# firelion9/raytracing-course-hw-public

Measured on AMD Instinct MI355X. Metric: Msamples/sec (whole node) on Sponza 1000x1000, higher is better.
Workload: dtype f32; 1 GPU; S-sponza synthetic (Sponza-sized): 262144+28 triangles, 16x3 1024^2 RGBA8 textures, 1000x1000, 64 SPP, ray_depth 8, device RNG; workload_id=sponza, width=1000, height=1000, spp=64, triangles=262172, launcher=single, ranks_formed=1, film=device (rt_render_rgb8), traversal=reference tree, reference order and pruning (parity mode), bvh=reference topology, host build

## Files before the change

### raytracing-course-hw-public_amd/csrc/rt_accum_host.cpp

```cpp
#include <algorithm>
#include <cmath>
#include <cstring>

#include "rt_scene_impl.h"

struct rt_accum {
    rt_scene *scene = nullptr;
    uint32_t width = 0, height = 0;
    WfView view{};
    WfView *d_view = nullptr;
    rt::AccumRound R{};
    std::vector<void *> owned;
    rt::PacketPolicy pkt;
    bool features = false;
    WfFeat F{};
    rt::DenoiseBufs D{};
    ~rt_accum() {
        (void)hipSetDevice(scene->device);
        (void)hipStreamSynchronize(scene->stream);
        for (void *p : owned)
            (void)hipFree(p);
        if (counted)
            --scene->live_accums;
    }
    bool counted = false;
};

template <class T> static int accum_alloc(rt_accum *a, size_t bytes, T **ptr, const char *fn) {
    void *q = nullptr;
    hipError_t e = hipMalloc(&q, bytes ? bytes : 16);
    if (e != hipSuccess)
        return rt::fail(e == hipErrorOutOfMemory ? RT_ERR_OOM : RT_ERR_HIP, std::string(fn) + ": " + hipGetErrorString(e));
    a->owned.push_back(q);
    *ptr = static_cast<T *>(q);
    return RT_OK;
}

extern "C" int rt_accum_create(rt_scene *s, uint32_t width, uint32_t height, const rt_camera *camera, uint64_t seed, rt_accum **out) {
    return rt_accum_create_ex(s, width, height, camera, seed, 0u, out);
}

extern "C" int rt_accum_create_ex(rt_scene *s, uint32_t width, uint32_t height, const rt_camera *camera, uint64_t seed, uint32_t accum_flags, rt_accum **out) {
    if (!s || !out)
        return rt::fail(RT_ERR_INVALID_ARG, "rt_accum_create: null argument");
    *out = nullptr;
    if (accum_flags & ~(uint32_t)RT_ACCUM_FEATURES)
        return rt::fail(RT_ERR_INVALID_ARG, "rt_accum_create_ex: unknown accum_flags bit");
    if (width == 0 || height == 0 || (uint64_t)width * height >= 0x7FFFFFFFull)
        return rt::fail(RT_ERR_INVALID_ARG, "rt_accum_create: image size " + std::to_string(width) + "x" + std::to_string(height));
    if (s->group)
        return rt::fail(RT_ERR_UNSUPPORTED, "rt_accum_create: accumulators run on single-GPU scenes only");
    HIP_TRY(hipSetDevice(s->device));
    auto a = std::make_unique<rt_accum>();
    a->scene = s;
    a->width = width;
    a->height = height;
    a->view = rt::make_view(camera ? *camera : s->cam, width, height, seed);
    const size_t n = (size_t)width * height;
    auto alloc = [&]<class T>(size_t bytes, T **ptr) -> int { return accum_alloc(a.get(), bytes, ptr, "rt_accum_create"); };
    rt::AccumRound &R = a->R;
    R.width = width;
    R.height = height;
    R.scan_temp_bytes = rt::accum_scan_temp_bytes((uint32_t)n);
    int rc;
    if ((rc = alloc(12 * n, &R.sum)) != RT_OK || (rc = alloc(12 * n, &R.even_sum)) != RT_OK || (rc = alloc(4 * n, &R.count)) != RT_OK ||
        (rc = alloc(4 * n, &R.err)) != RT_OK || (rc = alloc(4 * n, &R.target)) != RT_OK || (rc = alloc(8 * n, &R.scan_in)) != RT_OK ||
        (rc = alloc(8 * n, &R.scan)) != RT_OK || (rc = alloc(4 * n, &R.list_pix)) != RT_OK || (rc = alloc(4 * n, &R.list_base)) != RT_OK ||
        (rc = alloc(4 * (n + 1), &R.list_off)) != RT_OK || (rc = alloc(8, &R.totals)) != RT_OK || (rc = alloc(R.scan_temp_bytes, &R.scan_temp)) != RT_OK ||
        (rc = alloc(sizeof(WfView), &a->d_view)) != RT_OK)
        return rc;
    if (accum_flags & RT_ACCUM_FEATURES) {
        WfFeat &F = a->F;
        if ((rc = alloc(12 * n, &F.albedo_sum)) != RT_OK || (rc = alloc(12 * n, &F.normal_sum)) != RT_OK || (rc = alloc(4 * n, &F.depth_sum)) != RT_OK ||
            (rc = alloc(4 * n, &F.hits)) != RT_OK)
            return rc;
        HIP_TRY(hipMemsetAsync(F.albedo_sum, 0, 12 * n, s->stream));
        HIP_TRY(hipMemsetAsync(F.normal_sum, 0, 12 * n, s->stream));
        HIP_TRY(hipMemsetAsync(F.depth_sum, 0, 4 * n, s->stream));
        HIP_TRY(hipMemsetAsync(F.hits, 0, 4 * n, s->stream));
        a->features = true;
    }
    HIP_TRY(hipMemsetAsync(R.sum, 0, 12 * n, s->stream));
    HIP_TRY(hipMemsetAsync(R.even_sum, 0, 12 * n, s->stream));
    HIP_TRY(hipMemsetAsync(R.count, 0, 4 * n, s->stream));
    HIP_TRY(hipMemsetD32Async(R.err, 0x7F800000 , n, s->stream));
    HIP_TRY(hipMemcpyAsync(a->d_view, &a->view, sizeof(WfView), hipMemcpyHostToDevice, s->stream));
    HIP_TRY(hipStreamSynchronize(s->stream));
    a->counted = true;
    ++s->live_accums;
    *out = a.release();
    return RT_OK;
}

extern "C" void rt_accum_destroy(rt_accum *acc) { delete acc; }

static int accum_check(const rt_accum *a, const rt_params *p, const char *fn) {
    if (!a || !p)
        return rt::fail(RT_ERR_INVALID_ARG, std::string(fn) + ": null argument");
    if (p->width != a->width || p->height != a->height)
        return rt::fail(RT_ERR_INVALID_ARG, std::string(fn) + ": params size " + std::to_string(p->width) + "x" + std::to_string(p->height) +
                                                " differs from the accumulator's " + std::to_string(a->width) + "x" + std::to_string(a->height));
    if (p->shard_count > 1 || (p->flags & RT_FLAG_DEVICE_FB))
        return rt::fail(RT_ERR_INVALID_ARG, std::string(fn) + ": shard_count > 1 and RT_FLAG_DEVICE_FB do not apply to an accumulator");
    if (p->rng_mode == RT_RNG_REFERENCE)
        return rt::fail(RT_ERR_UNSUPPORTED, std::string(fn) + ": the reference RNG draws a 256-pixel span as one sequential stream; accumulators need RT_RNG_DEVICE");
    if (p->rng_mode != RT_RNG_DEVICE)
        return rt::fail(RT_ERR_INVALID_ARG, std::string(fn) + ": unknown rng_mode");
    if (p->flags & RT_FLAG_MEGAKERNEL)
        return rt::fail(RT_ERR_UNSUPPORTED, std::string(fn) + ": accumulators run on the wavefront pipeline, not the megakernel");
    return rt::check_pass_params(p, fn);
}

static int accum_run(rt_accum *a, const rt_params *p, const rt_adaptive *ad, uint32_t *rounds_out, rt_stats *stats) {
    rt_scene *s = a->scene;
    const auto wall0 = std::chrono::steady_clock::now();
    if (stats)
        std::memset(stats, 0, sizeof(*stats));
    if (rounds_out)
        *rounds_out = 0;
    if (s->dev.ray_depth == 0)
        return RT_OK;
    HIP_TRY(hipSetDevice(s->device));
    const uint32_t n_pix = a->width * a->height;
    const bool counters = stats && (p->flags & RT_FLAG_COUNTERS);
    const uint64_t max_paths = rt::wavefront_max_paths(s, p);
    const uint32_t chunk_cap = (uint32_t)std::max<uint64_t>(1, std::min<uint64_t>(max_paths, 0xFFFFFFFFull / n_pix));
    WfLaunch W{};
    W.width = a->width;
    W.height = a->height;
    W.shard_count = 1;
    W.shard_block = n_pix;
    W.ray_depth = s->dev.ray_depth;
    W.views = a->d_view;
    W.view_pixels = n_pix;
    W.global_best = (p->flags & RT_FLAG_GLOBAL_BEST) ? 1u : 0u;
    W.stats = counters ? s->d_stats : nullptr;
    s->ext_events.reset();
    uint32_t passes = 0, packet_passes = 0, rounds = 0;
    uint64_t added = 0;
    const uint32_t uni_chunk = std::min(ad ? 1u : p->samples, chunk_cap);
    const uint64_t uni_per_pass = std::max<uint64_t>(1, max_paths / uni_chunk);
    const uint32_t uni_passes = ad ? 0u : (uint32_t)(((uint64_t)p->samples + uni_chunk - 1) / uni_chunk * ((n_pix + uni_per_pass - 1) / uni_per_pass));

    auto fill = [&](uint32_t K, bool *any) -> int {
        const uint32_t C = std::min(K, chunk_cap);
        const uint32_t per_pass = (uint32_t)std::min<uint64_t>(n_pix, std::max<uint64_t>(1, max_paths / C));
        for (;;) {
            HIP_TRY(rt::launch_accum_plan(a->R, C, s->stream));
            uint32_t tot[2] = {0u, 0u};
            HIP_TRY(hipMemcpyAsync(tot, a->R.totals, sizeof(tot), hipMemcpyDeviceToHost, s->stream));
            HIP_TRY(hipStreamSynchronize(s->stream));
            if (tot[0] == 0)
                return RT_OK;
            *any = true;
            const uint64_t cap = std::min<uint64_t>((uint64_t)std::min(per_pass, tot[0]) * C, tot[1]);
            if (int rc = s->ensure_wavefront(cap, std::max<uint64_t>(s->wf_pixels_cap, 1), s->dev.ray_depth); rc != RT_OK)
                return rc;
            if (a->features) {
                if (int rc = s->ensure_features(); rc != RT_OK)
                    return rc;
                a->F.rec = s->wf_feat;
            }
            s->wf_bind(W);
            W.fb = nullptr;
            W.accum = nullptr;
            for (uint32_t e0 = 0; e0 < tot[0]; e0 += per_pass) {
                WfAccum A{a->R.sum, a->R.even_sum, a->R.count, a->R.list_pix, a->R.list_base, a->R.list_off, e0, std::min(per_pass, tot[0] - e0)};
                W.n_paths = (uint32_t)std::min<uint64_t>((uint64_t)A.n_entries * C, tot[1]);
                W.first_pixel = 0, W.pass_pixels = A.n_entries;
                W.first_sample = 0, W.pass_samples = C, W.samples = C;
                HIP_TRY(rt::launch_pass(s, p, a->pkt, W, 1, true, true, stats != nullptr, &A, a->features ? &a->F : nullptr));
                passes += 1;
                packet_passes += W.use_packet;
                if (p->progress && !ad) {
                    HIP_TRY(hipStreamSynchronize(s->stream));
                    p->progress(passes, std::max(passes, uni_passes), p->progress_user);
                }
            }
            added += tot[1];
        }
    };

    auto queue = [&]() -> int {
        if (counters)
            HIP_TRY(hipMemsetAsync(s->d_stats, 0, sizeof(DevStats), s->stream));
        HIP_TRY(hipEventRecord(s->ev0, s->stream));
        if (!ad) {
            HIP_TRY(rt::launch_accum_uniform(a->R, p->samples, s->stream));
            bool any = false;
            if (int rc = fill(p->samples, &any); rc != RT_OK)
                return rc;
        } else {
            const uint32_t mn = ad->min_samples ? ad->min_samples : 16u, st = ad->step ? ad->step : 32u, mx = ad->max_samples;
            const uint32_t bound = 1u + (mx - std::min(mn, mx) + st - 1u) / st;
            for (uint32_t r = 0;; ++r) {
                HIP_TRY(rt::launch_accum_judge(a->R, r == 0 ? 1 : 0, ad->threshold, mn, mx, st, s->stream));
                bool any = false;
                if (int rc = fill(r == 0 ? mn : st, &any); rc != RT_OK)
                    return rc;
                if (any) {
                    ++rounds;
                    if (p->progress)
                        p->progress(rounds, std::max(rounds, bound), p->progress_user);
                } else if (r > 0) {
                    break;
                }
            }
        }
        HIP_TRY(hipEventRecord(s->ev1, s->stream));
        return RT_OK;
    };
    if (int rc = rt::queue_and_wait(s, queue); rc != RT_OK)
        return rc;
    if (rounds_out)
        *rounds_out = rounds;
    if (stats) {
        float ms = 0;
        HIP_TRY(hipEventElapsedTime(&ms, s->ev0, s->ev1));
        if (int rc = rt::fill_stats(s, counters, added, ms, wall0, stats); rc != RT_OK)
            return rc;
        stats->packet_lanes_x100 = a->pkt.lanes_x100;
        stats->passes = passes;
        stats->packet_passes = packet_passes;
    }
    return RT_OK;
}

extern "C" int rt_accum_render(rt_accum *acc, const rt_params *params, rt_stats *stats) {
    if (int rc = accum_check(acc, params, "rt_accum_render"); rc != RT_OK)
        return rc;
    if (params->samples == 0)
        return rt::fail(RT_ERR_INVALID_ARG, "rt_accum_render: samples must be >= 1");
    return accum_run(acc, params, nullptr, nullptr, stats);
}

extern "C" int rt_accum_render_adaptive(rt_accum *acc, const rt_params *params, const rt_adaptive *ad, uint32_t *rounds, rt_stats *stats) {
    if (int rc = accum_check(acc, params, "rt_accum_render_adaptive"); rc != RT_OK)
        return rc;
    if (!ad)
        return rt::fail(RT_ERR_INVALID_ARG, "rt_accum_render_adaptive: null argument");
    if (!(ad->threshold >= 0.0f) || std::isinf(ad->threshold))
        return rt::fail(RT_ERR_INVALID_ARG, "rt_accum_render_adaptive: threshold must be finite and >= 0");
    const uint32_t mn = ad->min_samples ? ad->min_samples : 16u;
    if (mn == 1u || ad->max_samples < mn)
        return rt::fail(RT_ERR_INVALID_ARG, "rt_accum_render_adaptive: min_samples must be 0 or >= 2, and max_samples >= min_samples");
    for (uint32_t r : ad->reserved)
        if (r != 0)
            return rt::fail(RT_ERR_INVALID_ARG, "rt_accum_render_adaptive: reserved fields must be 0");
    return accum_run(acc, params, ad, rounds, stats);
}

extern "C" int rt_accum_resolve(rt_accum *acc, uint32_t flags, float *fb_rgb) {
    if (!acc || !fb_rgb || (flags & ~(uint32_t)RT_FLAG_DEVICE_FB))
        return rt::fail(RT_ERR_INVALID_ARG, "rt_accum_resolve: null argument or flags other than RT_FLAG_DEVICE_FB");
    rt_scene *s = acc->scene;
    HIP_TRY(hipSetDevice(s->device));
    const size_t n = (size_t)acc->width * acc->height;
    const bool device_fb = (flags & RT_FLAG_DEVICE_FB) != 0;
    if (!device_fb)
        if (int rc = s->ensure_fb(3 * n); rc != RT_OK)
            return rc;
    HIP_TRY(rt::launch_accum_image(acc->R, device_fb ? fb_rgb : s->d_fb, s->stream));
    if (!device_fb)
        HIP_TRY(hipMemcpyAsync(fb_rgb, s->d_fb, 3 * n * sizeof(float), hipMemcpyDeviceToHost, s->stream));
    HIP_TRY(hipStreamSynchronize(s->stream));
    return RT_OK;
}

extern "C" int rt_accum_resolve_rgb8(rt_accum *acc, uint32_t flags, uint8_t *rgb8) {
    if (!acc || !rgb8 || (flags & ~(uint32_t)RT_FLAG_DEVICE_FB))
        return rt::fail(RT_ERR_INVALID_ARG, "rt_accum_resolve_rgb8: null argument or flags other than RT_FLAG_DEVICE_FB");
    rt_scene *s = acc->scene;
    HIP_TRY(hipSetDevice(s->device));
    const uint32_t n = acc->width * acc->height;
    const bool device_fb = (flags & RT_FLAG_DEVICE_FB) != 0;
    int rc = s->ensure_fb(3ull * n);
    if (rc == RT_OK)
        rc = s->ensure_film(device_fb ? 0 : 3ull * n);
    if (rc != RT_OK)
        return rc;
    uint8_t *d_rgb8 = device_fb ? rgb8 : s->d_rgb8;
    HIP_TRY(rt::launch_accum_image(acc->R, s->d_fb, s->stream));
    HIP_TRY(rt::launch_film(s->d_fb, d_rgb8, n, 0, 1, n, s->d_film_table, s->stream));
    if (!device_fb)
        HIP_TRY(hipMemcpyAsync(rgb8, d_rgb8, 3ull * n, hipMemcpyDeviceToHost, s->stream));
    HIP_TRY(hipStreamSynchronize(s->stream));
    return RT_OK;
}

extern "C" int rt_accum_read(rt_accum *acc, float *sum_rgb, float *even_sum_rgb, uint32_t *samples, float *error) {
    if (!acc)
        return rt::fail(RT_ERR_INVALID_ARG, "rt_accum_read: null accumulator");
    rt_scene *s = acc->scene;
    HIP_TRY(hipSetDevice(s->device));
    const size_t n = (size_t)acc->width * acc->height;
    if (sum_rgb)
        HIP_TRY(hipMemcpyAsync(sum_rgb, acc->R.sum, 12 * n, hipMemcpyDeviceToHost, s->stream));
    if (even_sum_rgb)
        HIP_TRY(hipMemcpyAsync(even_sum_rgb, acc->R.even_sum, 12 * n, hipMemcpyDeviceToHost, s->stream));
    if (samples)
        HIP_TRY(hipMemcpyAsync(samples, acc->R.count, 4 * n, hipMemcpyDeviceToHost, s->stream));
    if (error)
        HIP_TRY(hipMemcpyAsync(error, acc->R.err, 4 * n, hipMemcpyDeviceToHost, s->stream));
    HIP_TRY(hipStreamSynchronize(s->stream));
    return RT_OK;
}

static int feature_check(const rt_accum *acc, const char *fn) {
    if (!acc)
        return rt::fail(RT_ERR_INVALID_ARG, std::string(fn) + ": null accumulator");
    if (!acc->features)
        return rt::fail(RT_ERR_INVALID_ARG, std::string(fn) + ": the accumulator was created without RT_ACCUM_FEATURES");
    return RT_OK;
}

extern "C" int rt_accum_read_features(rt_accum *acc, float *albedo_sum, float *normal_sum, float *depth_sum, uint32_t *hits) {
    if (int rc = feature_check(acc, "rt_accum_read_features"); rc != RT_OK)
        return rc;
    rt_scene *s = acc->scene;
    HIP_TRY(hipSetDevice(s->device));
    const size_t n = (size_t)acc->width * acc->height;
    if (albedo_sum)
        HIP_TRY(hipMemcpyAsync(albedo_sum, acc->F.albedo_sum, 12 * n, hipMemcpyDeviceToHost, s->stream));
    if (normal_sum)
        HIP_TRY(hipMemcpyAsync(normal_sum, acc->F.normal_sum, 12 * n, hipMemcpyDeviceToHost, s->stream));
    if (depth_sum)
        HIP_TRY(hipMemcpyAsync(depth_sum, acc->F.depth_sum, 4 * n, hipMemcpyDeviceToHost, s->stream));
    if (hits)
        HIP_TRY(hipMemcpyAsync(hits, acc->F.hits, 4 * n, hipMemcpyDeviceToHost, s->stream));
    HIP_TRY(hipStreamSynchronize(s->stream));
    return RT_OK;
}

extern "C" int rt_accum_resolve_features(rt_accum *acc, uint32_t flags, float *albedo, float *normal, float *depth) {
    if (int rc = feature_check(acc, "rt_accum_resolve_features"); rc != RT_OK)
        return rc;
    if (flags & ~(uint32_t)RT_FLAG_DEVICE_FB)
        return rt::fail(RT_ERR_INVALID_ARG, "rt_accum_resolve_features: flags other than RT_FLAG_DEVICE_FB");
    rt_scene *s = acc->scene;
    HIP_TRY(hipSetDevice(s->device));
    const size_t n = (size_t)acc->width * acc->height;
    if (flags & RT_FLAG_DEVICE_FB) {
        HIP_TRY(rt::launch_accum_feature_means(acc->R, acc->F, albedo, normal, depth, s->stream));
        HIP_TRY(hipStreamSynchronize(s->stream));
        return RT_OK;
    }
    if (int rc = s->ensure_fb(7 * n); rc != RT_OK)
        return rc;
    float *d_a = s->d_fb, *d_n = s->d_fb + 3 * n, *d_z = s->d_fb + 6 * n;
    HIP_TRY(rt::launch_accum_feature_means(acc->R, acc->F, d_a, d_n, d_z, s->stream));
    if (albedo)
        HIP_TRY(hipMemcpyAsync(albedo, d_a, 12 * n, hipMemcpyDeviceToHost, s->stream));
    if (normal)
        HIP_TRY(hipMemcpyAsync(normal, d_n, 12 * n, hipMemcpyDeviceToHost, s->stream));
    if (depth)
        HIP_TRY(hipMemcpyAsync(depth, d_z, 4 * n, hipMemcpyDeviceToHost, s->stream));
    HIP_TRY(hipStreamSynchronize(s->stream));
    return RT_OK;
}

static int denoise_options(const rt_accum *acc, const rt_denoise *opt, uint32_t flags, const void *out, const char *fn, rt::DenoiseOpt *O) {
    if (int rc = feature_check(acc, fn); rc != RT_OK)
        return rc;
    if (!out || (flags & ~(uint32_t)RT_FLAG_DEVICE_FB))
        return rt::fail(RT_ERR_INVALID_ARG, std::string(fn) + ": null buffer or flags other than RT_FLAG_DEVICE_FB");
    const rt_denoise zero{};
    const rt_denoise &o = opt ? *opt : zero;
    for (uint32_t r : o.reserved)
        if (r != 0)
            return rt::fail(RT_ERR_INVALID_ARG, std::string(fn) + ": reserved fields must be 0");
    if (o.iterations > 8u || o.normal_sharpness > 8u || (o.flags & ~(uint32_t)RT_DENOISE_NO_DEMODULATE))
        return rt::fail(RT_ERR_INVALID_ARG, std::string(fn) + ": iterations and normal_sharpness are at most 8; unknown rt_denoise.flags bit");
    if (!(o.sigma_color >= 0.0f) || std::isinf(o.sigma_color) || !(o.sigma_depth >= 0.0f) || std::isinf(o.sigma_depth))
        return rt::fail(RT_ERR_INVALID_ARG, std::string(fn) + ": sigma_color and sigma_depth must be finite and >= 0");
    O->iterations = o.iterations ? o.iterations : 5u;
    O->sigma_color = o.sigma_color != 0.0f ? o.sigma_color : 8.0f;
    O->sigma_depth = o.sigma_depth != 0.0f ? o.sigma_depth : 0.5f;
    O->sharpness = o.normal_sharpness ? o.normal_sharpness : 3u;
    O->demodulate = (o.flags & RT_DENOISE_NO_DEMODULATE) ? 0u : 1u;
    return RT_OK;
}

static int denoise_buffers(rt_accum *acc, const char *fn) {
    if (acc->D.guide)
        return RT_OK;
    const size_t n = (size_t)acc->width * acc->height;
    int rc;
    if ((rc = accum_alloc(acc, 16 * n, &acc->D.sig[0], fn)) != RT_OK || (rc = accum_alloc(acc, 16 * n, &acc->D.sig[1], fn)) != RT_OK ||
        (rc = accum_alloc(acc, 16 * n, &acc->D.den, fn)) != RT_OK)
        return rc;
    return accum_alloc(acc, 32 * n, &acc->D.guide, fn);
}

extern "C" int rt_accum_denoise(rt_accum *acc, const rt_denoise *opt, uint32_t flags, float *fb_rgb) {
    rt::DenoiseOpt O{};
    if (int rc = denoise_options(acc, opt, flags, fb_rgb, "rt_accum_denoise", &O); rc != RT_OK)
        return rc;
    rt_scene *s = acc->scene;
    HIP_TRY(hipSetDevice(s->device));
    const size_t n = (size_t)acc->width * acc->height;
    const bool device_fb = (flags & RT_FLAG_DEVICE_FB) != 0;
    if (int rc = denoise_buffers(acc, "rt_accum_denoise"); rc != RT_OK)
        return rc;
    if (!device_fb)
        if (int rc = s->ensure_fb(3 * n); rc != RT_OK)
            return rc;
    HIP_TRY(rt::launch_denoise(acc->R, acc->F, acc->D, O, device_fb ? fb_rgb : s->d_fb, s->stream));
    if (!device_fb)
        HIP_TRY(hipMemcpyAsync(fb_rgb, s->d_fb, 3 * n * sizeof(float), hipMemcpyDeviceToHost, s->stream));
    HIP_TRY(hipStreamSynchronize(s->stream));
    return RT_OK;
}

extern "C" int rt_accum_denoise_rgb8(rt_accum *acc, const rt_denoise *opt, uint32_t flags, uint8_t *rgb8) {
    rt::DenoiseOpt O{};
    if (int rc = denoise_options(acc, opt, flags, rgb8, "rt_accum_denoise_rgb8", &O); rc != RT_OK)
        return rc;
    rt_scene *s = acc->scene;
    HIP_TRY(hipSetDevice(s->device));
    const uint32_t n = acc->width * acc->height;
    const bool device_fb = (flags & RT_FLAG_DEVICE_FB) != 0;
    int rc = denoise_buffers(acc, "rt_accum_denoise_rgb8");
    if (rc == RT_OK)
        rc = s->ensure_fb(3ull * n);
    if (rc == RT_OK)
        rc = s->ensure_film(device_fb ? 0 : 3ull * n);
    if (rc != RT_OK)
        return rc;
    uint8_t *d_rgb8 = device_fb ? rgb8 : s->d_rgb8;
    HIP_TRY(rt::launch_denoise(acc->R, acc->F, acc->D, O, s->d_fb, s->stream));
    HIP_TRY(rt::launch_film(s->d_fb, d_rgb8, n, 0, 1, n, s->d_film_table, s->stream));
    if (!device_fb)
        HIP_TRY(hipMemcpyAsync(rgb8, d_rgb8, 3ull * n, hipMemcpyDeviceToHost, s->stream));
    HIP_TRY(hipStreamSynchronize(s->stream));
    return RT_OK;
}
```

### raytracing-course-hw-public_amd/csrc/rt_dev_queue.h

```cpp
#pragma once
#include "rt_dev_math.h"

namespace {

struct TicketState {
    uint32_t part, tried;
};
DEV TicketState ticket_init() { return TicketState{blockIdx.x & 7u, 0u}; }
DEV bool ticket_take(uint32_t *counters, uint32_t n_in, uint32_t chunk, TicketState &ts, uint32_t &q_lo, uint32_t &q_hi) {
    const uint32_t n_chunks = (n_in + chunk - 1u) / chunk;
    for (;;) {
        if (ts.tried >= 8u)
            return false;
        const uint32_t c0 = (uint32_t)(((unsigned long long)n_chunks * ts.part) >> 3), c1 = (uint32_t)(((unsigned long long)n_chunks * (ts.part + 1u)) >> 3);
        uint32_t t = 0;
        if ((threadIdx.x & 63u) == 0u)
            t = atomicAdd(counters + WF_CNT_XCD + ts.part * WF_CNT_XCD_STRIDE, 1u);
        t = (uint32_t)__builtin_amdgcn_readfirstlane((int)t);
        if (c0 + t < c1) {
            q_lo = (c0 + t) * chunk;
            q_hi = q_lo + chunk < n_in ? q_lo + chunk : n_in;
            return true;
        }
        ts.part = (ts.part + 1u) & 7u;
        ++ts.tried;
    }
}
template <class START>
DEV void ticket_refill(uint32_t *counters, uint32_t n_in, uint32_t chunk, int refill_min, bool idle, bool &exhausted, uint32_t &q_lo, uint32_t &q_hi, TicketState &tks, START start) {
    const unsigned long long im = __ballot(idle);
    const int n_idle = __popcll(im);
    if (!exhausted && (n_idle >= refill_min || n_idle == (int)__popcll(__ballot(1)))) {
        if (q_lo == q_hi)
            exhausted = !ticket_take(counters, n_in, chunk, tks, q_lo, q_hi);
        const uint32_t rank = lane_rank(im);
        const uint32_t avail = q_hi - q_lo;
        if (idle && rank < avail)
            start(q_lo + rank);
        q_lo += (uint32_t)n_idle < avail ? (uint32_t)n_idle : avail;
    }
}
DEV void census_flush(unsigned long long *census, unsigned long long n_trips, unsigned long long n_lanes) {
    if ((threadIdx.x & 63u) == 0u && census && n_trips != 0ull) {
        atomicAdd(census, n_trips);
        atomicAdd(census + 1, n_lanes);
    }
}

}
```

### raytracing-course-hw-public_amd/csrc/rt_dev_trav.h

```cpp
#pragma once
#include "../../include/rt_primspec.h"
#include "rt_dev_math.h"

namespace {

DEV float div_exact_fast(float a, float d, float r) {
    const float q0 = a * r;
    const float e0 = __builtin_fmaf(-d, q0, a);
    return __builtin_fmaf(e0, r, q0);
}
constexpr float RANGE_LO = 9.094947017729282e-13f;
constexpr float RANGE_HI = 1099511627776.0f;
constexpr float ORIGIN_LO = 7.275957614183426e-12f;
DEV bool coord_in_fast_range(float c) {
    const float m = __builtin_fabsf(c);
    return (c == 0.0f) | ((m >= ORIGIN_LO) & (m <= RANGE_HI));
}

DEV bool box_hit_exact(V3 bmin, V3 bmax, V3 o, V3 d, float min_dst, float &dist) {
    V3 i1 = (bmin - o) / d;
    V3 i2 = (bmax - o) / d;
    V3 mn = {rmin(i1.x, i2.x), rmin(i1.y, i2.y), rmin(i1.z, i2.z)};
    V3 mx = {rmax(i1.x, i2.x), rmax(i1.y, i2.y), rmax(i1.z, i2.z)};
    float t_min = mn.x;
    if (t_min < mn.y)
        t_min = mn.y;
    if (t_min < mn.z)
        t_min = mn.z;
    float t_max = mx.x;
    if (mx.y < t_max)
        t_max = mx.y;
    if (mx.z < t_max)
        t_max = mx.z;
    if (t_min <= t_max && t_max >= min_dst) {
        dist = rmax(t_min, min_dst);
        return true;
    }
    return false;
}

DEV bool box_hit_fast(V3 bmin, V3 bmax, V3 o, V3 d, V3 r, float min_dst, float &dist) {
    V3 a1 = bmin - o, a2 = bmax - o;
    float q1x = div_exact_fast(a1.x, d.x, r.x), q1y = div_exact_fast(a1.y, d.y, r.y), q1z = div_exact_fast(a1.z, d.z, r.z);
    float q2x = div_exact_fast(a2.x, d.x, r.x), q2y = div_exact_fast(a2.y, d.y, r.y), q2z = div_exact_fast(a2.z, d.z, r.z);
    float t_min = fmaxf(fmaxf(fminf(q1x, q2x), fminf(q1y, q2y)), fminf(q1z, q2z));
    float t_max = fminf(fminf(fmaxf(q1x, q2x), fmaxf(q1y, q2y)), fmaxf(q1z, q2z));
    dist = fmaxf(t_min, min_dst);
    return (t_min <= t_max) & (t_max >= min_dst);
}

struct NodeRec {
    V3 lmin, lmax, rmn, rmx;
    uint32_t left, right;
};
template <class P, class P3> DEV NodeRec node_rec(const P &r0, const P &r1, const P &r2, const P3 &r3) {
    return NodeRec{mk(r0.x, r0.y, r0.z), mk(r0.w, r1.x, r1.y), mk(r1.z, r1.w, r2.x), mk(r2.y, r2.z, r2.w), __float_as_uint(r3.x), __float_as_uint(r3.y)};
}
struct TriRec {
    V3 a, v, u;
    uint32_t flags, index;
};
template <class P> DEV TriRec tri_rec(const P &r0, const P &r1, const P &r2) {
    return TriRec{mk(r0.x, r0.y, r0.z), mk(r0.w, r1.x, r1.y), mk(r1.z, r1.w, r2.x), __float_as_uint(r2.z), __float_as_uint(r2.w)};
}

DEV bool tri_hit(const TriRec &tri, V3 o, V3 d, float min_dst, V3 &xs_out) {
    const V3 av = tri.v, au = tri.u;
    V3 at = -d;
    V3 y = o - tri.a;
    V3 c_ut = crs(au, at);
    float den = dot(av, c_ut);
    float nx = dot(y, c_ut), ny = dot(av, crs(y, at)), nz = dot(av, crs(au, y));
    const uint32_t sgn = __float_as_uint(den) & 0x80000000u;
    const float D = __builtin_fabsf(den);
    const float nxs = __uint_as_float(__float_as_uint(nx) ^ sgn), nys = __uint_as_float(__float_as_uint(ny) ^ sgn),
                nzs = __uint_as_float(__float_as_uint(nz) ^ sgn);
    const bool d_ok = (D >= 8.673617379884035e-19f) & (D <= 1.152921504606847e18f);
    const bool miss = (nxs < -8.673617379884035e-19f) | (nys < -8.673617379884035e-19f) | (nxs + nys > D * 1.00000095367431640625f) |
                      (nzs < D * (min_dst * 0.99999904632568359375f));
    if (d_ok & miss)
        return false;
    V3 xs = V3{nx, ny, nz} / den;
    if (xs.x >= 0 && xs.y >= 0 && xs.x + xs.y <= 1 && xs.z >= min_dst) {
        xs_out = xs;
        return true;
    }
    return false;
}

struct Hit {
    uint32_t k;
    float b, c, t;
};
DEV void hit_take(Hit &best, uint32_t k, float b, float c, float t) {
    if (best.k == RT_NONE || best.t > t) {
        best.k = k;
        best.b = b;
        best.c = c;
        best.t = t;
    }
}

DEV rt_primitive_desc load_prim(const rt_primitive_desc *prims, uint32_t i) {
    rt_primitive_desc p;
    const uint4 *src = reinterpret_cast<const uint4 *>(prims + i);
    uint4 *dst = reinterpret_cast<uint4 *>(&p);
    dst[0] = src[0];
    dst[1] = src[1];
    dst[2] = src[2];
    return p;
}
DEV void prims_closest(const DevScene &S, V3 o, V3 d, Hit &best) {
    const float oo[3] = {o.x, o.y, o.z}, dd[3] = {d.x, d.y, d.z};
    for (uint32_t i = 0; i < S.n_prims; ++i) {
        const rt_primitive_desc p = load_prim(S.prims, i);
        float t, n[3];
        if (rt_prim_intersect(&p, oo, dd, 1e-4f , &t, n))
            hit_take(best, RT_PRIM_FLAG | i, 0.0f, 0.0f, t);
    }
}

constexpr uint32_t T_DONE = 0xFFFFFFFEu, T_POP = 0xFFFFFFFDu;
struct Trav {
    V3 o, d, r;
    uint32_t cur;
    int sp;
    float t_loc;
    Hit best;
    bool fast;
    uint32_t top_ref;
    float top_d, top_loc;
};
DEV bool ray_fast_ok_ray(V3 o, V3 d) {
    const float lo = fminf(fminf(__builtin_fabsf(d.x), __builtin_fabsf(d.y)), __builtin_fabsf(d.z));
    const float hi = fmaxf(fmaxf(__builtin_fabsf(d.x), __builtin_fabsf(d.y)), __builtin_fabsf(d.z));
    return (d.x == d.x) & (d.y == d.y) & (d.z == d.z) & (lo >= RANGE_LO) & (hi <= RANGE_HI) & (int)coord_in_fast_range(o.x) & (int)coord_in_fast_range(o.y) &
           (int)coord_in_fast_range(o.z);
}
DEV bool ray_fast_ok(const DevBvh &bvh, V3 o, V3 d) {
    const bool ray_ok = ray_fast_ok_ray(o, d);
    return ray_ok & (bvh.fast_ok != 0u);
}
template <bool GB = false> DEV void trav_init_stored(Trav &T, const DevBvh &bvh, V3 o, V3 d, V3 r, bool ray_ok) {
    T.o = o;
    T.d = d;
    T.r = r;
    T.fast = ray_ok & (bvh.fast_ok != 0u);
    T.cur = (bvh.root == RT_NONE || bvh.n_tris == 0) ? T_DONE : bvh.root;
    T.sp = 0;
    T.t_loc = GB ? RT_INF : RT_NAN;
    if constexpr (GB)
        T.top_loc = 0.0f;
    T.best = Hit{RT_NONE, 0.f, 0.f, 0.f};
}
DEV void trav_init(Trav &T, const DevBvh &bvh, V3 o, V3 d) { trav_init_stored<false>(T, bvh, o, d, mk(1.0f / d.x, 1.0f / d.y, 1.0f / d.z), ray_fast_ok_ray(o, d)); }
template <bool GB = false> DEV Trav trav_idle() {
    Trav T;
    T.o = T.d = T.r = mk(0.f, 0.f, 0.f);
    T.cur = T_DONE;
    T.sp = 0;
    T.t_loc = GB ? RT_INF : RT_NAN;
    T.best = Hit{RT_NONE, 0.f, 0.f, 0.f};
    T.fast = false;
    T.top_ref = 0u;
    T.top_d = T.top_loc = 0.f;
    return T;
}

template <class STK> DEV void trav_pop(Trav &T, STK &stk) {
    while (T.cur == T_POP) {
        if (T.sp == 0) {
            T.cur = T_DONE;
            break;
        }
        --T.sp;
        const uint32_t ref = T.top_ref;
        const float dfar = T.top_d, saved = T.top_loc;
        if (T.sp > 0)
            stk.pop(T.sp - 1, T.top_ref, T.top_d, T.top_loc);
        const float t_near = T.t_loc;
        T.t_loc = fminf(saved, t_near);
        if (!(t_near <= dfar))
            T.cur = ref;
    }
}

struct TwoBox {
    bool hl, hr;
    float dl, dr;
};
template <bool KNOWN_FAST = false> DEV TwoBox two_box(const NodeRec &n, V3 o, V3 d, V3 r, bool fast, float min_dst) {
    TwoBox b;
    if (KNOWN_FAST || fast) {
        b.hl = box_hit_fast(n.lmin, n.lmax, o, d, r, min_dst, b.dl);
        b.hr = box_hit_fast(n.rmn, n.rmx, o, d, r, min_dst, b.dr);
    } else {
        b.hl = box_hit_exact(n.lmin, n.lmax, o, d, min_dst, b.dl);
        b.hr = box_hit_exact(n.rmn, n.rmx, o, d, min_dst, b.dr);
    }
    return b;
}
template <bool STATS, bool GB = false, bool KNOWN_FAST = false, class STK>
DEV void trav_inner_apply(Trav &T, STK &stk, const NodeRec &n, float min_dst, LaneStats<STATS> &st) {
    st.node();
    st.box(2);
    const TwoBox bx = two_box<KNOWN_FAST>(n, T.o, T.d, T.r, T.fast, min_dst);
    bool hl = bx.hl, hr = bx.hr;
    const float dl = bx.dl, dr = bx.dr;
    if constexpr (GB) {
        hl = hl && dl < T.t_loc;
        hr = hr && dr < T.t_loc;
    }
    const bool both = hl & hr;
    const bool swap = dl > dr;
    if (both & (T.sp > 0))
        stk.push(T.sp - 1, T.top_ref, T.top_d, T.top_loc);
    T.top_ref = both ? (swap ? n.left : n.right) : T.top_ref;
    T.top_d = both ? (swap ? dl : dr) : T.top_d;
    if constexpr (!GB) {
        T.top_loc = both ? T.t_loc : T.top_loc;
        T.t_loc = both ? RT_NAN : T.t_loc;
    }
    T.sp += both ? 1 : 0;
    T.cur = both ? (swap ? n.right : n.left) : (hl ? n.left : (hr ? n.right : T_POP));
}
template <bool STATS, bool GB = false, class STK> DEV void trav_step_core(Trav &T, const DevBvh &bvh, STK &stk, float min_dst, LaneStats<STATS> &st) {
    const bool leaf = (T.cur & RT_LEAF_FLAG) != 0;
    const float4 *p = leaf ? reinterpret_cast<const float4 *>(bvh.tris + (T.cur & RT_LEAF_BEGIN_MASK)) : reinterpret_cast<const float4 *>(bvh.nodes + T.cur);
    const float4 r0 = p[0], r1 = p[1], r2 = p[2];
    if (!leaf) {
        trav_inner_apply<STATS, GB>(T, stk, node_rec(r0, r1, r2, p[3]), min_dst, st);
    } else {
        const TriRec tri = tri_rec(r0, r1, r2);
        if (tri.flags & 2u)
            st.node();
        st.tri();
        V3 xs;
        if (tri_hit(tri, T.o, T.d, min_dst, xs)) {
            hit_take(T.best, T.cur & RT_LEAF_BEGIN_MASK, xs.x, xs.y, xs.z);
            T.t_loc = fminf(T.t_loc, xs.z);
        }
        T.cur = (tri.flags & 1u) ? T_POP : T.cur + 1;
    }
}
template <bool STATS, class STK> DEV void trav_step(Trav &T, const DevBvh &bvh, STK &stk, float min_dst, LaneStats<STATS> &st) {
    trav_step_core<STATS, false>(T, bvh, stk, min_dst, st);
    trav_pop(T, stk);
}
template <bool STATS, bool GB = false, class STK> DEV void trav_step_inner_fast(Trav &T, const DevBvh &bvh, STK &stk, float min_dst, LaneStats<STATS> &st) {
    const float4 *p = reinterpret_cast<const float4 *>(bvh.nodes + T.cur);
    const float4 r0 = p[0], r1 = p[1], r2 = p[2];
    const float2 r3 = *reinterpret_cast<const float2 *>(p + 3);
    trav_inner_apply<STATS, GB, true>(T, stk, node_rec(r0, r1, r2, r3), min_dst, st);
}
template <bool GB = false, class STK> DEV void trav_pop_once(Trav &T, STK &stk) {
    const bool pop = T.cur == T_POP;
    const bool go = pop & (T.sp != 0);
    const int nsp = T.sp - 1;
    const bool refill = go & (nsp > 0);
    uint32_t n_ref;
    float n_d, n_loc = 0.0f;
    stk.pop_masked(nsp - 1, refill, n_ref, n_d, n_loc);
    const float t_near = T.t_loc;
    const bool visit = !(t_near <= T.top_d);
    T.cur = pop ? (go ? (visit ? T.top_ref : T_POP) : T_DONE) : T.cur;
    if constexpr (!GB)
        T.t_loc = go ? fminf(T.top_loc, t_near) : t_near;
    T.sp = go ? nsp : T.sp;
    T.top_ref = refill ? n_ref : T.top_ref;
    T.top_d = refill ? n_d : T.top_d;
    if constexpr (!GB)
        T.top_loc = refill ? n_loc : T.top_loc;
}
template <bool GB = false, class STK> DEV void trav_pop_wave(Trav &T, STK &stk) {
    while (__ballot(T.cur == T_POP) != 0ull)
        trav_pop_once<GB>(T, stk);
}
template <class PAYLOAD> struct CoopLds {
    uint16_t *owner;
    unsigned long long *min;
    PAYLOAD *pay;
};
template <class PAYLOAD> DEV PAYLOAD coop_payload(V3 xs, uint32_t index) {
    if constexpr (sizeof(PAYLOAD) == sizeof(float2))
        return make_float2(xs.x, xs.y);
    else
        return make_float4(xs.x, xs.y, __uint_as_float(index), 0.0f);
}
template <int N_ENT, bool STATS, class PAYLOAD, class REC, class ENTRY, class ADDR>
DEV void coop_tri_batch(bool waiting, uint32_t n, uint32_t base, V3 ro, V3 rd, const REC *recs, const CoopLds<PAYLOAD> &lds, ENTRY entry, ADDR addr, LaneStats<STATS> &st) {
    const uint32_t lane = threadIdx.x & 63u;
    uint32_t total;
    const uint32_t off = wave_prefix_sum4(n, total);
    if (waiting) {
        uint16_t ent[N_ENT];
#pragma unroll
        for (int t = 0; t < N_ENT; ++t)
            ent[t] = (uint16_t)(lane | (entry(t) << 8));
#pragma unroll
        for (int t = N_ENT - 1; t >= 0; --t) {
            lds.owner[off + t] = ent[t];
            asm volatile("" ::: "memory");
        }
        lds.min[lane] = ~0ull;
    }
    __threadfence_block();
    for (uint32_t q0 = 0; q0 < total; q0 += 64u) {
        const uint32_t q = q0 + lane;
        const bool valid = q < total;
        const uint32_t ow = valid ? (uint32_t)lds.owner[q] : 0u;
        const int src = (int)(ow & 63u);
        const uint32_t kk = addr((uint32_t)__shfl((int)base, src), ow >> 8);
        const V3 o = mk(__shfl(ro.x, src), __shfl(ro.y, src), __shfl(ro.z, src));
        const V3 d = mk(__shfl(rd.x, src), __shfl(rd.y, src), __shfl(rd.z, src));
        if (valid) {
            const float4 *p = reinterpret_cast<const float4 *>(recs + kk);
            const float4 r0 = p[0], r1 = p[1], r2 = p[2];
            const TriRec tri = tri_rec(r0, r1, r2);
            st.tri();
            V3 xs;
            if (tri_hit(tri, o, d, EPS, xs)) {
                const unsigned long long key = ((unsigned long long)__float_as_uint(xs.z) << 32) | (unsigned long long)kk;
                atomicMin(&lds.min[src], key);
                __threadfence_block();
                if (lds.min[src] == key)
                    lds.pay[src] = coop_payload<PAYLOAD>(xs, tri.index);
            }
        }
    }
    __threadfence_block();
}
template <class PAYLOAD> DEV bool coop_result(const CoopLds<PAYLOAD> &lds, float &t, uint32_t &rec, PAYLOAD &pay) {
    const uint32_t lane = threadIdx.x & 63u;
    const unsigned long long key = lds.min[lane];
    if (key == ~0ull)
        return false;
    t = __uint_as_float((uint32_t)(key >> 32));
    rec = (uint32_t)key;
    pay = lds.pay[lane];
    return true;
}

struct LightTabs {
    const float4 *nodes, *tris, *aux;
};
DEV LightTabs light_tabs_global(const DevScene &S) {
    return LightTabs{reinterpret_cast<const float4 *>(S.lights.nodes), reinterpret_cast<const float4 *>(S.lights.tris), reinterpret_cast<const float4 *>(S.light_aux)};
}
template <bool STATS, class STK> DEV float lights_pdf(const DevScene &S, const LightTabs &LT, V3 x, V3 d, STK &stk, LaneStats<STATS> &st) {
    const DevBvh &bvh = S.lights;
    st.lq();
    float res = 0;
    if (bvh.root != RT_NONE && bvh.n_tris != 0) {
        uint32_t cur = bvh.root;
        int sp = 0;
        const bool fast = ray_fast_ok(bvh, x, d);
        const V3 r = mk(1.0f / d.x, 1.0f / d.y, 1.0f / d.z);
        while (cur != T_DONE) {
            const bool leaf = (cur & RT_LEAF_FLAG) != 0;
            const float4 *p = leaf ? LT.tris + 3u * (cur & RT_LEAF_BEGIN_MASK) : LT.nodes + 4u * cur;
            const float4 r0 = p[0], r1 = p[1], r2 = p[2];
            if (!leaf) {
                const NodeRec n = node_rec(r0, r1, r2, p[3]);
                st.lnode();
                st.lbox(2);
                const TwoBox bx = two_box(n, x, d, r, fast, EPS);
                if (bx.hl & bx.hr) {
                    stk.push_ref(sp++, n.right);
                    cur = n.left;
                } else if (bx.hl) {
                    cur = n.left;
                } else if (bx.hr) {
                    cur = n.right;
                } else {
                    cur = T_POP;
                }
            } else {
                const uint32_t k = cur & RT_LEAF_BEGIN_MASK;
                const TriRec tri = tri_rec(r0, r1, r2);
                const uint32_t flags = tri.flags;
                if (flags & 2u)
                    st.lnode();
                st.ltri();
                V3 xs;
                if (tri_hit(tri, x, d, EPS, xs)) {
                    st.lhit();
                    const float4 aux = LT.aux[k];
                    V3 y = x + d * xs.z;
                    V3 dir = norm(y - x);
                    float mult = len2(x - y) / __builtin_fabsf(dot(dir, mk(aux.x, aux.y, aux.z)));
                    res += mult / aux.w;
                }
                cur = (flags & 1u) ? T_POP : cur + 1;
            }
            if (cur == T_POP)
                cur = sp ? stk.pop_ref(--sp) : T_DONE;
        }
    }
    return res / (float)bvh.n_tris;
}

}
```

### raytracing-course-hw-public_amd/csrc/rt_device_types.h

```cpp
#pragma once
#include <stdint.h>

#include "../../include/rt_abi.h"

#define RT_NONE 0xFFFFFFFFu
#define RT_PRIM_FLAG 0x40000000u
#define RT_LEAF_FLAG 0x80000000u
#define RT_LEAF_BEGIN_MASK 0x07FFFFFFu
#define RT_LEAF_CNT(ref) (((ref) >> 27) & 15u)
#define RT_LEAF_COOP_MAX 8u
#define RT_MAX_STACK 64
#define RT_MAX_RAY_DEPTH 32u
#define RT_SPAN 256u

struct alignas(16) DevNode {
    float lmin[3], lmax[3];
    float rmin[3], rmax[3];
    uint32_t left, right;
    uint32_t pad[2];
};
static_assert(sizeof(DevNode) == 64, "DevNode must be 64 bytes");

struct alignas(16) DevTri {
    float a[3];
    float v[3];
    float u[3];
    uint32_t prim;
    uint32_t flags;
    uint32_t pad;
};
static_assert(sizeof(DevTri) == 48, "DevTri must be 48 bytes");

struct alignas(16) DevAttr {
    float n[9];
    float tg[9];
    float uv[6];
    float gn[3];
    uint32_t material;
    uint32_t pad[4];
};
static_assert(sizeof(DevAttr) == 128, "DevAttr must be 128 bytes");

struct alignas(16) uint4_pod {
    uint32_t x, y, z, w;
};

struct alignas(16) DevLightAux {
    float normal[3];
    float area;
};

struct alignas(16) DevMaterial {
    float color[4];
    float emission[3];
    float roughness;
    float metallic;
    float ior;
    int32_t color_tex, emissive_tex, mr_tex, normal_tex;
    int32_t tex_set;
    uint32_t tex_set_info;
};
static_assert(sizeof(DevMaterial) == 64, "DevMaterial must be 64 bytes");

struct alignas(16) DevTexture {
    uint32_t width, height;
    uint32_t offset;
    uint32_t count;
    uint32_t stride;
    uint32_t tiles_x;
    uint32_t tw_log, th_log;
};
static_assert(sizeof(DevTexture) == 32, "DevTexture must be 32 bytes");

struct alignas(16) WideNode {
    float p[3];
    uint8_t e[3];
    uint8_t imask;
    uint32_t child_base;
    uint32_t tri_base;
    uint32_t tri_mask;
    uint32_t pad;
    uint8_t qlo[3][8];
    uint8_t qhi[3][8];
};
static_assert(sizeof(WideNode) == 80, "WideNode must be 80 bytes");
#define RT_WIDE_MAX_LEAF_TRIS 3u

struct WideGrid {
    float base[3];
    float g;
    int32_t e_base;
    uint32_t pad_;
};
#define RT_WIDE_ORIGIN_BITS 20u
#define RT_WIDE_NODE_UNITS 4u
#define RT_WIDE_TRI_UNITS 3u

struct DevBvh {
    const DevNode *nodes;
    const DevTri *tris;
    uint32_t root;
    uint32_t n_tris;
    uint32_t fast_ok;
    uint32_t lds_inner;
    const uint4_pod *wide;
    uint32_t n_wide;
    uint32_t n_units;
    WideGrid grid;
};
#define RT_SHADE_LIGHTS_F4 384

struct DevScene {
    DevBvh scene;
    DevBvh lights;
    const DevAttr *attrs;
    const DevLightAux *light_aux;
    const DevMaterial *materials;
    const DevTexture *textures;
    const uint32_t *texels;
    const float *lut_linear;
    const float *lut_gamma;
    float cam_pos[3], cam_right[3], cam_up[3], cam_fwd[3];
    float bg[3];
    uint32_t ray_depth;
    float bounds_lo[3], bounds_inv[3];
    const rt_primitive_desc *prims;
    uint32_t n_prims;
    uint32_t n_triangles;
    int32_t bg_tex;
    uint32_t pad_bg;
};

struct DevStats {
    unsigned long long samples, casts, nodes, box_tests, tri_tests, shaded, lq, lnodes, lbox, ltri, lhits, texels;
};

struct alignas(64) WfPath {
    float o[3];
    float dx;
    float dy, dz;
    uint32_t path;
    uint32_t depth;
    float r[3];
    uint32_t fast;
    uint32_t s[4];
};
static_assert(sizeof(WfPath) == 64, "WfPath must be 64 bytes");
#define WF_ORDER_SLOT_MASK 0x3FFFFFFFu
#define WF_ORDER_CLASS_SHIFT 30
struct alignas(16) WfHit {
    uint32_t k;
    float b, c, t;
};
struct alignas(16) RtF4 {
    float x, y, z, w;
};
struct alignas(16) WfFold {
    float e[3], pad0;
    float s[3], pad1;
};
enum {
    WF_CNT_IN = 0, WF_CNT_TICKET = 2, WF_CNT_SLOTS = 3,
    WF_CNT_XCD = 32 , WF_CNT_XCD_STRIDE = 32,
    WF_CNT_WORDS = WF_CNT_XCD + 8 * WF_CNT_XCD_STRIDE,
    WF_CNT_CENSUS = WF_CNT_WORDS,
    WF_CNT_ALLOC_WORDS = WF_CNT_CENSUS + 4
};
static_assert(WF_CNT_XCD + 7 * WF_CNT_XCD_STRIDE < WF_CNT_WORDS && WF_CNT_CENSUS >= WF_CNT_WORDS && (WF_CNT_CENSUS % 2) == 0,
              "census words must not overlap the ticket lines and must be 8-byte aligned");
#define WF_STRIPES 64u
#define WF_STRIPE_WORDS 32u
#define WF_STRIPE_BUF_WORDS (WF_STRIPES * WF_STRIPE_WORDS + WF_STRIPES + 1u)
#ifdef __HIPCC__
__host__ __device__
#endif
inline uint32_t wf_stripe_base(uint32_t k, uint32_t n_slots) {
    const uint32_t q = n_slots / WF_STRIPES, r = n_slots % WF_STRIPES;
    return 64u * (k * q + (k < r ? k : r));
}

struct alignas(64) WfView {
    float pos[3], right[3], up[3], fwd[3];
    float tan_x, tan_y;
    uint64_t seed;
};
static_assert(sizeof(WfView) == 64, "WfView must be 64 bytes");

struct WfLaunch {
    uint32_t width, height, samples;
    uint32_t first_sample, pass_samples;
    uint32_t first_pixel, pass_pixels;
    uint32_t n_paths;
    uint32_t shard_index, shard_count, shard_block;
    uint32_t ray_depth;
    const WfView *views;
    uint32_t view_pixels;
    WfPath *paths_in, *paths_out;
    WfHit *hits;
    WfFold *fold;
    RtF4 *sample_out;
    RtF4 *accum;
    float *fb;
    void *stack_overflow;
    uint32_t stack_stride;
    uint32_t *counters;
    uint32_t *stripes;
    const uint32_t *order;
    uint32_t *sort_keys[2];
    uint32_t *sort_vals[2];
    void *sort_temp;
    uint32_t use_packet;
    unsigned long long *packet_census;
    uint32_t global_best;
    uint32_t order_classed;
    uint32_t sort_mode;
    size_t sort_temp_bytes;
    DevStats *stats;
};

struct WfAccum {
    float *sum, *even_sum;
    uint32_t *count;
    const uint32_t *list_pix;
    const uint32_t *list_base;
    const uint32_t *list_off;
    uint32_t first_entry, n_entries;
};

struct WfFeat {
    RtF4 *rec;
    float *albedo_sum, *normal_sum;
    float *depth_sum;
    uint32_t *hits;
};

struct WfRays {
    const uint4_pod *rays;
    uint32_t group;
    uint32_t samples;
    uint64_t seed;
};

struct RenderLaunch {
    uint32_t width, height, samples, rng_mode;
    uint64_t seed;
    uint32_t shard_index, shard_count, shard_block;
    uint32_t n_items;
    uint32_t items_per_block;
    float tan_x, tan_y;
    uint32_t item_base;
    uint32_t pix_base;
    float *fb;
    uint32_t *counter;
    DevStats *stats;
};
```

### raytracing-course-hw-public_amd/csrc/rt_kernels.h

```cpp
#pragma once
#include <hip/hip_runtime_api.h>

#include <type_traits>
#include <vector>

#include "rt_device_types.h"

#define RT_LAUNCH_CHECKED(...)               \
    ({                                       \
        (void)hipGetLastError();             \
        hipLaunchKernelGGL(__VA_ARGS__);     \
        hipGetLastError();                   \
    })

template <class F> auto with_bools(F &&f) { return f(); }
template <class F, class... Rest> auto with_bools(F &&f, bool b, Rest... rest) {
    return b ? with_bools([&](auto... c) { return f(std::true_type{}, c...); }, rest...) : with_bools([&](auto... c) { return f(std::false_type{}, c...); }, rest...);
}

namespace rt {
struct EventPool {
    std::vector<hipEvent_t> ev;
    size_t used = 0;
    hipEvent_t next() {
        if (used == ev.size()) {
            hipEvent_t e = nullptr;
            if (hipEventCreate(&e) != hipSuccess)
                return nullptr;
            ev.push_back(e);
        }
        return ev[used++];
    }
    void reset() { used = 0; }
    void destroy() {
        for (hipEvent_t e : ev)
            (void)hipEventDestroy(e);
        ev.clear();
        used = 0;
    }
};
hipError_t launch_render(const DevScene &S, const RenderLaunch &L, bool stats, int blocks, hipStream_t stream);
hipError_t launch_cast(const DevScene &S, const float *rays, uint32_t n, uint32_t *prim, float *bct, hipStream_t stream);
hipError_t launch_surface_normals(const DevScene &S, const float *rays, uint32_t n, uint32_t *prim, float *t, float *normal, float *shading, hipStream_t stream);
hipError_t launch_light_pdf(const DevScene &S, const float *rays, uint32_t n, float *pdf, hipStream_t stream);
hipError_t launch_bg_at(const DevScene &S, const float *dirs, uint32_t n, float *rgb, hipStream_t stream);
struct WfHostSync {
    uint32_t *counts;
    hipEvent_t *events;
    int n_events;
};
#define WF_HOST_CENSUS_WORD 40
hipError_t launch_wavefront_pass(const DevScene &S, WfLaunch L, bool stats, int num_cus, bool first_pass, bool last_pass, hipStream_t stream,
                                 EventPool *extend_events, unsigned long long *packet_census_out, const WfHostSync *host_sync,
                                 const WfAccum *acc = nullptr, const WfFeat *feat = nullptr, const WfRays *rays = nullptr);
hipError_t launch_wavefront_cast(const DevScene &S, WfLaunch L, const float *rays, uint32_t n, bool packet, bool stats, uint32_t *prim, float *bct,
                                 hipStream_t stream);
hipError_t launch_extend_wide(const DevScene &S, const WfLaunch &L, bool packet, bool stats, int blocks, hipStream_t stream);
size_t wavefront_sort_temp_bytes(size_t n);
struct AccumRound {
    float *sum, *even_sum;
    uint32_t *count;
    float *err;
    uint32_t *target;
    unsigned long long *scan_in, *scan;
    uint32_t *list_pix, *list_base, *list_off;
    uint32_t *totals;
    void *scan_temp;
    size_t scan_temp_bytes;
    uint32_t width, height;
};
size_t accum_scan_temp_bytes(uint32_t pixels);
hipError_t launch_accum_judge(const AccumRound &R, int round0, float threshold, uint32_t min_samples, uint32_t max_samples, uint32_t step,
                              hipStream_t stream);
hipError_t launch_accum_uniform(const AccumRound &R, uint32_t samples, hipStream_t stream);
hipError_t launch_accum_plan(const AccumRound &R, uint32_t chunk, hipStream_t stream);
hipError_t launch_accum_image(const AccumRound &R, float *fb, hipStream_t stream);
hipError_t launch_accum_feature_means(const AccumRound &R, const WfFeat &F, float *albedo, float *normal, float *depth, hipStream_t stream);
struct DenoiseBufs {
    RtF4 *sig[2];
    RtF4 *den;
    RtF4 *guide;
};
struct DenoiseOpt {
    uint32_t iterations, sharpness, demodulate;
    float sigma_color, sigma_depth;
};
hipError_t launch_denoise(const AccumRound &R, const WfFeat &F, const DenoiseBufs &D, const DenoiseOpt &O, float *fb, hipStream_t stream);
}
```

### raytracing-course-hw-public_amd/csrc/rt_render.cpp

```cpp
#include <algorithm>
#include <cmath>
#include <cstring>

#include "rt_scene_impl.h"

#ifndef RT_WIDE_PACKET_MIN_LANES
#define RT_WIDE_PACKET_MIN_LANES 20.0
#endif
static_assert(WF_STRIPES == 64u && (WF_STRIPES & (WF_STRIPES - 1u)) == 0u, "WF_STRIPES must equal the wave size (64)");

WfView rt::make_view(const rt_camera &cam, uint32_t width, uint32_t height, uint64_t seed) {
    WfView v{};
    std::memcpy(v.pos, cam.position, 12);
    std::memcpy(v.right, cam.right, 12);
    std::memcpy(v.up, cam.up, 12);
    std::memcpy(v.fwd, cam.forward, 12);
    v.tan_x = std::tan(cam.fov_x / 2);
    const float fov_y = std::atan(std::tan(cam.fov_x / 2) * height / width) * 2;
    v.tan_y = std::tan(fov_y / 2);
    v.seed = seed;
    return v;
}
void rt::set_camera(DevScene &D, const float *pos, const float *right, const float *up, const float *fwd) {
    std::memcpy(D.cam_pos, pos, 12);
    std::memcpy(D.cam_right, right, 12);
    std::memcpy(D.cam_up, up, 12);
    std::memcpy(D.cam_fwd, fwd, 12);
}

int rt::check_views(const rt_params *p, const rt_view *views, uint32_t n_views) {
    if (!p || !views || n_views == 0)
        return rt::fail(RT_ERR_INVALID_ARG, "rt_render_views: null argument or no view");
    for (uint32_t v = 0; v < n_views; ++v)
        if (views[v].reserved != 0)
            return rt::fail(RT_ERR_INVALID_ARG, "rt_render_views: reserved field of view " + std::to_string(v) + " is not 0");
    if ((uint64_t)n_views * p->width * p->height >= 0x7FFFFFFFull)
        return rt::fail(RT_ERR_INVALID_ARG, "rt_render_views: n_views x width x height must stay below 2^31");
    if (p->rng_mode == RT_RNG_REFERENCE && n_views > 1 && p->shard_count > 1)
        return rt::fail(RT_ERR_INVALID_ARG, "rt_render_views: reference RNG mode shards one view at a time (shard_count > 1 needs n_views == 1)");
    return RT_OK;
}

uint64_t rt::wavefront_max_paths(rt_scene *s, const rt_params *p) {
    uint64_t max_paths = 128ull << 20;
    {
        size_t free_b = 0, total_b = 0;
        if (hipMemGetInfo(&free_b, &total_b) == hipSuccess) {
            const uint64_t per_path = 2 * sizeof(WfPath) + sizeof(WfHit) + s->dev.ray_depth * sizeof(WfFold) + sizeof(RtF4) + 16 ;
            const uint64_t have = free_b + s->wf_paths_cap * per_path;
            const uint64_t fit = (uint64_t)(0.6 * (double)have) / per_path;
            max_paths = std::max<uint64_t>(1u << 16, std::min(max_paths, fit));
        }
    }
    if (p->max_paths)
        max_paths = std::max<uint64_t>(1024, p->max_paths);
    return std::min<uint64_t>(max_paths, 1ull << 29);
}

static rt::WfHostSync wavefront_host_sync(rt_scene *s) {
    if (!s->wf_host_count && hipHostMalloc((void **)&s->wf_host_count, 48 * sizeof(uint32_t)) != hipSuccess)
        s->wf_host_count = nullptr;
    while (s->wf_count_events.size() < RT_MAX_RAY_DEPTH + 1) {
        hipEvent_t ev = nullptr;
        if (hipEventCreateWithFlags(&ev, hipEventDisableTiming) != hipSuccess)
            break;
        s->wf_count_events.push_back(ev);
    }
    return rt::WfHostSync{s->wf_host_count, s->wf_count_events.data(), (int)s->wf_count_events.size()};
}

static uint32_t wavefront_sort_mode(const rt_scene *s, const rt_params *p) {
    const size_t bvh_bytes = (size_t)s->dev.scene.n_units * 16u;
    const bool sort_default = !(s->wide_built && bvh_bytes < ((size_t)128 << 20));
    return (p->sort_mode == RT_SORT_AUTO ? sort_default : p->sort_mode == RT_SORT_OCTANT_CELL_CONE) ? 1u : 0u;
}

static double packet_min_lanes(const rt_scene *s, const rt_params *p) {
    return p->packet_min_lanes > 0.0f ? (double)p->packet_min_lanes : (s->wide_built ? RT_WIDE_PACKET_MIN_LANES : 33.0);
}

int rt::check_pass_params(const rt_params *p, const char *fn) {
    if ((p->sort_mode != RT_SORT_AUTO && p->sort_mode != RT_SORT_OFF && p->sort_mode != RT_SORT_OCTANT_CELL_CONE) || p->packet_mode > RT_PACKET_ON || !(p->packet_min_lanes >= 0.0f && p->packet_min_lanes <= 64.0f))
        return rt::fail(RT_ERR_INVALID_ARG, std::string(fn) + ": unknown sort_mode / packet_mode, or packet_min_lanes outside [0, 64]");
    return RT_OK;
}

hipError_t rt::launch_pass(rt_scene *s, const rt_params *p, PacketPolicy &pol, WfLaunch &W, uint32_t n_views, bool first_pass, bool last_pass, bool time_extends,
                           const WfAccum *acc, const WfFeat *feat, const WfRays *rays) {
    W.sort_mode = (p->sort_mode == RT_SORT_AUTO && W.n_paths < (1u << 20)) ? 0u : wavefront_sort_mode(s, p);
    const double min_lanes = packet_min_lanes(s, p);
    uint32_t min_lanes_bits;
    { const float ml = (float)min_lanes; std::memcpy(&min_lanes_bits, &ml, 4); }
    const uint64_t key = ((uint64_t)W.width << 44) ^ ((uint64_t)W.height << 24) ^ ((uint64_t)W.pass_samples << 8) ^ (uint64_t)W.shard_count ^
                         ((uint64_t)min_lanes_bits * 0x9E3779B97F4A7C15ull) ^ ((uint64_t)(n_views - 1) * 0xC2B2AE3D27D4EB4Full);
    if (key != pol.key) {
        pol.key = key;
        pol.off = false;
    }
    const uint32_t pkt_min_spp = s->wide_built ? 4u : 16u;
    W.use_packet = p->packet_mode == RT_PACKET_OFF ? 0u : p->packet_mode == RT_PACKET_ON ? 1u : (W.pass_samples >= pkt_min_spp && !pol.off) ? 1u : 0u;
    const rt::WfHostSync hsync = wavefront_host_sync(s);
    unsigned long long census[2] = {0ull, 0ull};
    const hipError_t e = rt::launch_wavefront_pass(s->dev, W, W.stats != nullptr, s->num_cus, first_pass, last_pass, s->stream, time_extends ? &s->ext_events : nullptr, census,
                                                   s->wf_host_count ? &hsync : nullptr, acc, feat, rays);
    if (e == hipSuccess && census[0] != 0ull) {
        pol.lanes_x100 = (uint32_t)(100.0 * (double)census[1] / (double)census[0]);
        if ((double)census[1] < min_lanes * (double)census[0])
            pol.off = true;
    }
    return e;
}

int rt::fill_stats(rt_scene *s, bool counters, uint64_t samples, float kernel_ms, std::chrono::steady_clock::time_point wall0, rt_stats *stats) {
    DevStats h{};
    if (counters)
        HIP_TRY(hipMemcpy(&h, s->d_stats, sizeof(h), hipMemcpyDeviceToHost));
    stats->samples = counters ? h.samples : samples;
    stats->casts = h.casts;
    stats->nodes_visited = h.nodes;
    stats->box_tests = h.box_tests;
    stats->tri_tests = h.tri_tests;
    stats->shaded_hits = h.shaded;
    stats->light_queries = h.lq;
    stats->light_nodes = h.lnodes;
    stats->light_box_tests = h.lbox;
    stats->light_tri_tests = h.ltri;
    stats->light_hits = h.lhits;
    stats->texel_fetches = h.texels;
    stats->kernel_ms = kernel_ms;
    const std::vector<hipEvent_t> &xe = s->ext_events.ev;
    const size_t n_xe = s->ext_events.used & ~size_t(1);
    stats->dominant_launches = (uint32_t)(n_xe / 2);
    for (size_t i = 0; i + 1 < n_xe; i += 2) {
        float t = 0;
        if (hipEventElapsedTime(&t, xe[i], xe[i + 1]) == hipSuccess)
            stats->dominant_ms += t;
    }
    stats->total_ms = std::chrono::duration<double, std::milli>(std::chrono::steady_clock::now() - wall0).count();
    return RT_OK;
}

static int render_impl(rt_scene *s, const rt_params *p, const rt_view *views, uint32_t n_views, float *fb_rgb, uint8_t *rgb8_out, rt_stats *stats) {
    if (!s || !p || (!fb_rgb && !rgb8_out))
        return rt::fail(RT_ERR_INVALID_ARG, "rt_render: null argument");
    if (views)
        if (int rc = rt::check_views(p, views, n_views); rc != RT_OK)
            return rc;
    if (s->group)
        return rt::group_render(s->group, p, views, n_views, fb_rgb, rgb8_out, stats);
    if (!views)
        n_views = 1;
    if (p->width == 0 || p->height == 0 || (uint64_t)p->width * p->height >= 0x7FFFFFFFull)
        return rt::fail(RT_ERR_INVALID_ARG, "Illegal image size" + std::to_string(p->width) + "x" + std::to_string(p->height));
    if (p->rng_mode != RT_RNG_DEVICE && p->rng_mode != RT_RNG_REFERENCE)
        return rt::fail(RT_ERR_INVALID_ARG, "rt_render: unknown rng_mode");
    if (p->samples == 0)
        return rt::fail(RT_ERR_INVALID_ARG, "rt_render: samples must be >= 1");
    if (int rc = rt::check_pass_params(p, "rt_render"); rc != RT_OK)
        return rc;
    auto wall0 = std::chrono::steady_clock::now();
    if (stats)
        std::memset(stats, 0, sizeof(*stats));
    if (s->dev.ray_depth == 0)
        return RT_OK;
    HIP_TRY(hipSetDevice(s->device));

    const uint32_t view_pixels = p->width * p->height;
    const uint32_t n_pix = n_views * view_pixels;
    RenderLaunch L{};
    L.width = p->width;
    L.height = p->height;
    L.samples = p->samples;
    L.rng_mode = p->rng_mode;
    L.seed = p->seed;
    L.shard_count = p->shard_count ? p->shard_count : 1;
    L.shard_index = p->shard_index;
    if (L.shard_index >= L.shard_count)
        return rt::fail(RT_ERR_INVALID_ARG, "rt_render: shard_index >= shard_count");
    const uint32_t unit = p->rng_mode == RT_RNG_REFERENCE ? RT_SPAN : 1u;
    uint32_t block = p->shard_block ? p->shard_block : (L.shard_count > 1 ? RT_SPAN * 8u : n_pix);
    if (L.shard_count == 1)
        block = ((n_pix + unit - 1) / unit) * unit;
    if (block % unit != 0)
        return rt::fail(RT_ERR_INVALID_ARG, "rt_render: shard_block must be a multiple of 256 in reference RNG mode");
    L.shard_block = block;
    L.items_per_block = block / unit;
    const uint64_t n_blocks = ((uint64_t)n_pix + block - 1) / block;
    uint64_t items = 0, local_pixels = 0;
    for (uint64_t b = L.shard_index; b < n_blocks; b += L.shard_count) {
        uint64_t first = b * block, last = std::min<uint64_t>(first + block, n_pix);
        items += (last - first + unit - 1) / unit;
        local_pixels += last - first;
    }
    L.n_items = (uint32_t)items;
    std::vector<WfView> vt(n_views);
    for (uint32_t v = 0; v < n_views; ++v)
        vt[v] = views ? rt::make_view(views[v].camera, p->width, p->height, views[v].seed) : rt::make_view(s->cam, p->width, p->height, p->seed);
    L.tan_x = vt[0].tan_x;
    L.tan_y = vt[0].tan_y;

    const bool device_fb = (p->flags & RT_FLAG_DEVICE_FB) != 0;
    const size_t fb_floats = (size_t)n_pix * 3;
    float *d_fb = fb_rgb;
    if (!device_fb || rgb8_out) {
        int rc = s->ensure_fb(fb_floats);
        if (rc != RT_OK)
            return rc;
        d_fb = s->d_fb;
    }
    uint8_t *d_rgb8 = nullptr;
    if (rgb8_out) {
        int rc = s->ensure_film(device_fb ? 0 : fb_floats);
        if (rc != RT_OK)
            return rc;
        d_rgb8 = device_fb ? rgb8_out : s->d_rgb8;
    }
    L.fb = d_fb;
    L.counter = s->d_counter;
    const bool counters = stats && (p->flags & RT_FLAG_COUNTERS);
    L.stats = counters ? s->d_stats : nullptr;
    HIP_TRY(hipMemsetAsync(s->d_counter, 0, sizeof(uint32_t), s->stream));
    if (counters)
        HIP_TRY(hipMemsetAsync(s->d_stats, 0, sizeof(DevStats), s->stream));

    const bool wavefront = p->rng_mode == RT_RNG_DEVICE && !(p->flags & RT_FLAG_MEGAKERNEL);
    if (s->wide_built && !wavefront)
        return rt::fail(RT_ERR_UNSUPPORTED, "rt_render: a scene built with RT_BUILD_WIDE renders through the wavefront pipeline only (the megakernel and "
                                            "the reference-RNG parity mode walk the reference's binary tree: create the scene without RT_BUILD_WIDE)");
    s->ext_events.reset();
    uint32_t passes = 0, packet_passes = 0;
    auto queue_render = [&]() -> int {
    HIP_TRY(hipEventRecord(s->ev0, s->stream));
    if (L.n_items > 0 && wavefront) {
        const uint64_t max_paths = rt::wavefront_max_paths(s, p);
        const uint64_t tile_pixels = std::min<uint64_t>(local_pixels, max_paths);
        const uint32_t pass_spp = (uint32_t)std::clamp<uint64_t>(max_paths / tile_pixels, 1, p->samples);
        int rc = s->ensure_wavefront(tile_pixels * pass_spp, tile_pixels, s->dev.ray_depth);
        if (rc == RT_OK)
            rc = s->ensure_views(n_views);
        if (rc != RT_OK)
            return rc;
        HIP_TRY(hipMemcpyAsync(s->d_views, vt.data(), n_views * sizeof(WfView), hipMemcpyHostToDevice, s->stream));
        WfLaunch W{};
        W.width = p->width;
        W.height = p->height;
        W.samples = p->samples;
        W.shard_index = L.shard_index;
        W.shard_count = L.shard_count;
        W.shard_block = L.shard_block;
        W.ray_depth = s->dev.ray_depth;
        W.views = s->d_views;
        W.view_pixels = view_pixels;
        s->wf_bind(W);
        W.fb = d_fb;
        W.global_best = (p->flags & RT_FLAG_GLOBAL_BEST) ? 1u : 0u;
        W.stats = L.stats;
        uint32_t n_passes = 0, reported = 0;
        for (uint64_t p0 = 0; p0 < local_pixels; p0 += tile_pixels)
            n_passes += (p->samples + pass_spp - 1) / pass_spp;
        if (p->progress)
            while (s->pass_events.size() < n_passes) {
                hipEvent_t ev = nullptr;
                if (hipEventCreateWithFlags(&ev, hipEventDisableTiming) != hipSuccess)
                    return rt::fail(RT_ERR_HIP, "rt_render: progress event");
                s->pass_events.push_back(ev);
            }
        uint32_t pass_no = 0;
        for (uint64_t p0 = 0; p0 < local_pixels; p0 += tile_pixels) {
            W.first_pixel = (uint32_t)p0;
            W.pass_pixels = (uint32_t)std::min<uint64_t>(tile_pixels, local_pixels - p0);
            for (uint32_t s0 = 0; s0 < p->samples; s0 += pass_spp) {
                W.first_sample = s0;
                W.pass_samples = std::min<uint32_t>(pass_spp, p->samples - s0);
                W.n_paths = W.pass_pixels * W.pass_samples;
                HIP_TRY(rt::launch_pass(s, p, s->pkt, W, n_views, s0 == 0, s0 + W.pass_samples >= p->samples, stats != nullptr, nullptr));
                passes += 1;
                packet_passes += W.use_packet;
                if (p->progress) {
                    HIP_TRY(hipEventRecord(s->pass_events[pass_no], s->stream));
                    if (pass_no > 0) {
                        HIP_TRY(hipEventSynchronize(s->pass_events[pass_no - 1]));
                        p->progress(++reported, n_passes, p->progress_user);
                    }
                }
                ++pass_no;
            }
        }
        if (p->progress && pass_no > 0) {
            HIP_TRY(hipEventSynchronize(s->pass_events[pass_no - 1]));
            p->progress(++reported, n_passes, p->progress_user);
        }
    } else if (L.n_items > 0) {
        const uint64_t blk = L.shard_block;
        auto items_below = [&](uint64_t x) {
            const uint64_t full = x / blk, r = x % blk;
            return (full / L.shard_count) * blk + ((full % L.shard_count) > L.shard_index ? blk : 0) + ((full % L.shard_count) == L.shard_index ? r : 0);
        };
        uint32_t launched = 0;
        for (uint32_t v = 0; v < n_views; ++v) {
            RenderLaunch Lv = L;
            DevScene Sv = s->dev;
            rt::set_camera(Sv, vt[v].pos, vt[v].right, vt[v].up, vt[v].fwd);
            Lv.tan_x = vt[v].tan_x;
            Lv.tan_y = vt[v].tan_y;
            Lv.seed = vt[v].seed;
            Lv.fb = d_fb + (size_t)v * view_pixels * 3;
            if (n_views > 1 && p->rng_mode == RT_RNG_REFERENCE) {
                const uint32_t spans = (view_pixels + RT_SPAN - 1) / RT_SPAN;
                Lv.shard_block = spans * RT_SPAN;
                Lv.items_per_block = spans;
                Lv.n_items = spans;
            } else if (n_views > 1) {
                const uint64_t lo = items_below((uint64_t)v * view_pixels), hi = items_below((uint64_t)(v + 1) * view_pixels);
                Lv.item_base = (uint32_t)lo;
                Lv.n_items = (uint32_t)(hi - lo);
                Lv.pix_base = v * view_pixels;
            }
            if (Lv.n_items == 0)
                continue;
            if (launched > 0)
                HIP_TRY(hipMemsetAsync(s->d_counter, 0, sizeof(uint32_t), s->stream));
            const int vblocks = (int)std::max<uint64_t>(1, std::min<uint64_t>((Lv.n_items + 255) / 256, (uint64_t)s->num_cus * s->blocks_per_cu));
            HIP_TRY(rt::launch_render(Sv, Lv, counters, vblocks, s->stream));
            ++launched;
        }
        passes = launched;
        if (p->progress) {
            HIP_TRY(hipStreamSynchronize(s->stream));
            p->progress(launched, launched, p->progress_user);
        }
    }
    if (rgb8_out && L.n_items > 0)
        HIP_TRY(rt::launch_film(d_fb, d_rgb8, n_pix, L.shard_index, L.shard_count, block, s->d_film_table, s->stream));
    HIP_TRY(hipEventRecord(s->ev1, s->stream));
    return RT_OK;
    };
    if (int rc = rt::queue_and_wait(s, queue_render); rc != RT_OK)
        return rc;
    float ms = 0;
    HIP_TRY(hipEventElapsedTime(&ms, s->ev0, s->ev1));

    if (!device_fb && L.n_items > 0) {
        const size_t elem = rgb8_out ? 1 : sizeof(float);
        char *dst = rgb8_out ? reinterpret_cast<char *>(rgb8_out) : reinterpret_cast<char *>(fb_rgb);
        const char *src = rgb8_out ? reinterpret_cast<const char *>(d_rgb8) : reinterpret_cast<const char *>(d_fb);
        if (L.shard_count == 1) {
            HIP_TRY(hipMemcpy(dst, src, fb_floats * elem, hipMemcpyDeviceToHost));
        } else {
            for (uint64_t b = L.shard_index; b < n_blocks; b += L.shard_count) {
                uint64_t first = b * block, last = std::min<uint64_t>(first + block, n_pix);
                HIP_TRY(hipMemcpy(dst + 3 * first * elem, src + 3 * first * elem, (last - first) * 3 * elem, hipMemcpyDeviceToHost));
            }
        }
    }
    if (stats) {
        if (int rc = rt::fill_stats(s, counters, local_pixels * p->samples, ms, wall0, stats); rc != RT_OK)
            return rc;
        if (!wavefront) {
            stats->dominant_launches = passes;
            stats->dominant_ms = ms;
        }
        stats->packet_lanes_x100 = wavefront ? s->pkt.lanes_x100 : 0u;
        stats->passes = passes;
        stats->packet_passes = packet_passes;
    }
    return RT_OK;
}

extern "C" int rt_render(rt_scene *s, const rt_params *p, float *fb_rgb, rt_stats *stats) {
    if (!fb_rgb)
        return rt::fail(RT_ERR_INVALID_ARG, "rt_render: null argument");
    return render_impl(s, p, nullptr, 0, fb_rgb, nullptr, stats);
}

extern "C" int rt_render_rgb8(rt_scene *s, const rt_params *p, uint8_t *rgb8, rt_stats *stats) {
    if (!rgb8)
        return rt::fail(RT_ERR_INVALID_ARG, "rt_render_rgb8: null argument");
    return render_impl(s, p, nullptr, 0, nullptr, rgb8, stats);
}

extern "C" int rt_render_views(rt_scene *s, const rt_params *p, const rt_view *views, uint32_t n_views, float *fb_rgb, rt_stats *stats) {
    if (!fb_rgb || !views || n_views == 0)
        return rt::fail(RT_ERR_INVALID_ARG, "rt_render_views: null argument or no view");
    return render_impl(s, p, views, n_views, fb_rgb, nullptr, stats);
}

extern "C" int rt_render_views_rgb8(rt_scene *s, const rt_params *p, const rt_view *views, uint32_t n_views, uint8_t *rgb8, rt_stats *stats) {
    if (!rgb8 || !views || n_views == 0)
        return rt::fail(RT_ERR_INVALID_ARG, "rt_render_views_rgb8: null argument or no view");
    return render_impl(s, p, views, n_views, nullptr, rgb8, stats);
}

extern "C" int rt_film_rgb8(rt_scene *s, const float *rgb, size_t n_pixels, uint8_t *out_rgb8) {
    if (s && s->group)
        return rt_film_rgb8(rt::group_primary(s->group), rgb, n_pixels, out_rgb8);
    if (!s || (n_pixels && (!rgb || !out_rgb8)) || n_pixels >= 0x7FFFFFFFull)
        return rt::fail(RT_ERR_INVALID_ARG, "rt_film_rgb8: bad argument");
    if (n_pixels == 0)
        return RT_OK;
    HIP_TRY(hipSetDevice(s->device));
    int rc = s->ensure_fb(n_pixels * 3);
    if (rc == RT_OK)
        rc = s->ensure_film(n_pixels * 3);
    if (rc != RT_OK)
        return rc;
    HIP_TRY(hipMemcpyAsync(s->d_fb, rgb, n_pixels * 3 * sizeof(float), hipMemcpyHostToDevice, s->stream));
    HIP_TRY(rt::launch_film(s->d_fb, s->d_rgb8, (uint32_t)n_pixels, 0, 1, (uint32_t)n_pixels, s->d_film_table, s->stream));
    HIP_TRY(hipMemcpyAsync(out_rgb8, s->d_rgb8, n_pixels * 3, hipMemcpyDeviceToHost, s->stream));
    HIP_TRY(hipStreamSynchronize(s->stream));
    return RT_OK;
}
```

### raytracing-course-hw-public_amd/csrc/rt_scene.cpp

```cpp
#include <array>
#include <cmath>
#include <cstring>
#include <future>

#include "rt_bvh_device.h"
#include "rt_scene_impl.h"
#include "rt_wide_pack.h"
#include "wide_build.h"
#include "rt_build_stamp.h"

namespace {

template <class T> int upload(const std::vector<T> &v, const T **out, std::vector<void *> &owned) {
    *out = nullptr;
    if (v.empty())
        return RT_OK;
    void *p = nullptr;
    HIP_TRY(hipMalloc(&p, v.size() * sizeof(T)));
    owned.push_back(p);
    HIP_TRY(hipMemcpy(p, v.data(), v.size() * sizeof(T), hipMemcpyHostToDevice));
    *out = static_cast<const T *>(p);
    return RT_OK;
}

struct V3h {
    float x, y, z;
};
inline V3h cross_h(V3h a, V3h b) { return {a.y * b.z - a.z * b.y, a.z * b.x - a.x * b.z, a.x * b.y - a.y * b.x}; }
inline float len_h(V3h a) { return std::sqrt(a.x * a.x + a.y * a.y + a.z * a.z); }

}

extern "C" const char *rt_source_stamp(void) { return RT_SOURCE_STAMP; }

extern "C" int rt_device_count(void) {
    int n = 0;
    if (hipGetDeviceCount(&n) != hipSuccess)
        return 0;
    return n;
}

uint32_t rt::light_lds_inner(const rt::FlatBvh &f) {
    if (f.root == RT_NONE || f.tris.empty() || 4u * f.nodes.size() + 4u * f.tris.size() > (size_t)RT_SHADE_LIGHTS_F4)
        return 0u;
    return (uint32_t)f.nodes.size() + 1u;
}


static void make_attrs(const rt_scene_desc *d, const std::vector<DevTri> &tris, std::vector<DevAttr> &attrs) {
    attrs.resize(tris.size());
    for (size_t k = 0; k < attrs.size(); ++k) {
        const uint32_t t = tris[k].prim;
        DevAttr &a = attrs[k];
        std::memset(&a, 0, sizeof(a));
        std::memcpy(a.n, d->normals + 9 * (size_t)t, 36);
        std::memcpy(a.tg, d->tangents + 9 * (size_t)t, 36);
        std::memcpy(a.uv, d->texcoords + 6 * (size_t)t, 24);
        const DevTri &tr = tris[k];
        V3h c = cross_h({tr.v[0], tr.v[1], tr.v[2]}, {tr.u[0], tr.u[1], tr.u[2]});
        float l = len_h(c);
        a.gn[0] = c.x / l;
        a.gn[1] = c.y / l;
        a.gn[2] = c.z / l;
        a.material = d->material_ids[t];
    }
}
static void make_wide_tris(const rt_scene_desc *d, const rt::WideBvh &wide, std::vector<DevTri> &tris) {
    tris.resize(wide.order.size());
    for (size_t k = 0; k < tris.size(); ++k) {
        const float *p = d->positions + 9 * (size_t)wide.order[k];
        DevTri &t = tris[k];
        for (int c = 0; c < 3; ++c) {
            t.a[c] = p[c];
            t.v[c] = p[3 + c] - p[c];
            t.u[c] = p[6 + c] - p[c];
        }
        t.prim = wide.order[k];
        t.flags = 0;
        t.pad = 0;
    }
}

void rt::prepare_geometry(const rt_scene_desc *d, const std::vector<uint8_t> &emissive, float wide_cost_node, float wide_cost_tri, rt::PreparedGeometry &P,
                          bool lights_only) {
    const uint32_t n = d->n_triangles;
    std::vector<uint32_t> all(n), lights;
    for (uint32_t i = 0; i < n; ++i) {
        all[i] = i;
        if (emissive[d->material_ids[i]])
            lights.push_back(i);
    }
    P.dev_build = n > 0 && (d->build_flags & RT_BUILD_DEVICE_LBVH);
    P.wide_build = n > 0 && (d->build_flags & RT_BUILD_WIDE);
    const auto tb0 = std::chrono::steady_clock::now();
    if (!P.dev_build && !lights_only) {
        P.host_bvh[0] = rt::build_bvh(d->positions, n, all);
        if (!P.wide_build) {
            P.flat[0] = rt::flatten_bvh(P.host_bvh[0], d->positions);
            make_attrs(d, P.flat[0].tris, P.attrs);
        }
        P.build_ms = std::chrono::duration<double, std::milli>(std::chrono::steady_clock::now() - tb0).count();
        if (P.wide_build) {
            const auto tw0 = std::chrono::steady_clock::now();
            P.wide = rt::build_wide(rt::bin_from_host(P.host_bvh[0]), d->positions, wide_cost_node, wide_cost_tri);
            make_wide_tris(d, P.wide, P.wide_tris);
            make_attrs(d, P.wide_tris, P.attrs);
            P.wide_ms = std::chrono::duration<double, std::milli>(std::chrono::steady_clock::now() - tw0).count();
        }
    }
    rt::prepare_lights(d->positions, n, lights, nullptr, P);
}

void rt::prepare_lights(const float *positions, uint32_t n_total, const std::vector<uint32_t> &lights, const uint32_t *original, rt::PreparedGeometry &P) {
    P.host_bvh[1] = rt::build_bvh(positions, n_total, lights);
    P.flat[1] = rt::flatten_bvh(P.host_bvh[1], positions);
    if (original) {
        for (uint32_t &t : P.host_bvh[1].order)
            t = original[t];
        for (DevTri &tr : P.flat[1].tris)
            tr.prim = original[tr.prim];
    }
    P.laux.resize(P.flat[1].tris.size());
    for (size_t k = 0; k < P.laux.size(); ++k) {
        const DevTri &tr = P.flat[1].tris[k];
        V3h c = cross_h({tr.v[0], tr.v[1], tr.v[2]}, {tr.u[0], tr.u[1], tr.u[2]});
        float l = len_h(c);
        P.laux[k].normal[0] = c.x / l;
        P.laux[k].normal[1] = c.y / l;
        P.laux[k].normal[2] = c.z / l;
        P.laux[k].area = l / 2;
    }
}

static int prepare_scene(const rt_scene_desc *d, rt::PreparedScene &P) {
    const uint32_t n = d->n_triangles;
    for (uint32_t i = 0; i < n; ++i)
        if (d->material_ids[i] >= d->n_materials)
            return rt::fail(RT_ERR_INVALID_ARG, "rt_create: material id out of range");
    for (size_t i = 0; i < (size_t)n * 9; ++i)
        if (!std::isfinite(d->positions[i]))
            return rt::fail(RT_ERR_INVALID_ARG, "rt_create: non-finite vertex position (triangle " + std::to_string(i / 9) + ")");
    auto tex_ok = [&](int32_t t) { return t < 0 || (uint32_t)t < d->n_textures; };
    for (uint32_t i = 0; i < d->n_materials; ++i) {
        const rt_material_desc &m = d->materials[i];
        if (!tex_ok(m.color_tex) || !tex_ok(m.emissive_tex) || !tex_ok(m.metallic_roughness_tex) || !tex_ok(m.normal_tex))
            return rt::fail(RT_ERR_INVALID_ARG, "rt_create: texture index out of range");
    }
    if (!tex_ok(d->bg_texture))
        return rt::fail(RT_ERR_INVALID_ARG, "rt_create: bg_texture out of range");
    for (uint32_t i = 0; i < d->n_textures; ++i)
        if (d->textures[i].width == 0 || d->textures[i].height == 0 || !d->textures[i].rgba8)
            return rt::fail(RT_ERR_INVALID_ARG, "rt_create: empty texture");

    if (d->build.wide_cost_node > 0.0f)
        P.wide_cost_node = d->build.wide_cost_node;
    if (d->build.wide_cost_tri > 0.0f)
        P.wide_cost_tri = d->build.wide_cost_tri;
    P.build_flags = d->build_flags;
    P.build = d->build;
    std::vector<uint8_t> emissive(d->n_materials);
    for (uint32_t i = 0; i < d->n_materials; ++i) {
        const float *e = d->materials[i].emission;
        emissive[i] = !((e[0] == 0) & (e[1] == 0) & (e[2] == 0));
    }
    auto G = std::make_shared<rt::PreparedGeometry>();
    auto geometry_task = std::async(std::launch::async, [&]() { rt::prepare_geometry(d, emissive, P.wide_cost_node, P.wide_cost_tri, *G); });
    struct JoinGeometry {
        std::future<void> &f;
        ~JoinGeometry() {
            if (f.valid())
                f.wait();
        }
    } join_geometry{geometry_task};

    std::vector<DevMaterial> &mats = P.mats;
    mats.resize(d->n_materials);
    for (uint32_t i = 0; i < d->n_materials; ++i) {
        const rt_material_desc &m = d->materials[i];
        DevMaterial &o = mats[i];
        std::memset(&o, 0, sizeof(o));
        std::memcpy(o.color, m.color, 16);
        std::memcpy(o.emission, m.emission, 12);
        o.roughness = m.roughness;
        o.metallic = m.metallic;
        o.ior = m.ior;
        o.color_tex = m.color_tex;
        o.emissive_tex = m.emissive_tex;
        o.mr_tex = m.metallic_roughness_tex;
        o.normal_tex = m.normal_tex;
    }
    std::vector<DevTexture> &texs = P.texs;
    std::vector<uint32_t> &pool = P.pool;
    {
        auto store = [&](const std::vector<int32_t> &members, uint32_t stride, std::vector<int32_t> &view_of_member) {
            const rt_texture_desc *first = nullptr;
            for (int32_t t : members)
                if (t >= 0)
                    first = &d->textures[t];
            const uint32_t w = first->width, h = first->height;
            const uint32_t tw_log = stride == 1 ? 3u : 2u, th_log = stride == 1 ? 2u : 1u;
            const uint32_t tiles_x = (w + (1u << tw_log) - 1) >> tw_log, tiles_y = (h + (1u << th_log) - 1) >> th_log;
            const size_t base = (pool.size() + 31) & ~size_t(31);
            const size_t records = (size_t)tiles_x * tiles_y << (tw_log + th_log);
            pool.resize(base + records * stride, 0u);
            view_of_member.assign(members.size(), -1);
            for (size_t k = 0; k < members.size(); ++k) {
                if (members[k] < 0)
                    continue;
                const uint32_t *src = reinterpret_cast<const uint32_t *>(d->textures[members[k]].rgba8);
                for (uint32_t y = 0; y < h; ++y)
                    for (uint32_t x = 0; x < w; ++x) {
                        const size_t tile = (size_t)(y >> th_log) * tiles_x + (x >> tw_log);
                        const size_t within = ((y & ((1u << th_log) - 1)) << tw_log) | (x & ((1u << tw_log) - 1));
                        pool[base + ((tile << (tw_log + th_log)) + within) * stride + k] = src[(size_t)y * w + x];
                    }
                view_of_member[k] = (int32_t)texs.size();
                texs.push_back(DevTexture{w, h, (uint32_t)(base + k), w * h, stride, tiles_x, tw_log, th_log});
            }
        };
        std::vector<int32_t> alone(d->n_textures, -1);
        auto alone_view = [&](int32_t t) {
            if (alone[t] < 0) {
                std::vector<int32_t> v;
                store({t}, 1, v);
                alone[t] = v[0];
            }
            return alone[t];
        };
        std::vector<std::pair<std::array<int32_t, 4>, std::array<int32_t, 4>>> sets;
        const size_t budget = (size_t)1 << 30;
        for (uint32_t i = 0; i < d->n_materials; ++i) {
            DevMaterial &o = mats[i];
            std::array<int32_t, 4> ids = {o.color_tex, o.emissive_tex, o.mr_tex, o.normal_tex}, views = {-1, -1, -1, -1};
            bool found = false;
            for (const auto &e : sets)
                if (e.first == ids) {
                    views = e.second;
                    found = true;
                }
            if (!found) {
                std::array<int32_t, 4> group = {-1, -1, -1, -1};
                int best_n = 0;
                for (int a = 0; a < 4; ++a) {
                    if (ids[a] < 0 || d->textures[ids[a]].width * d->textures[ids[a]].height == 1)
                        continue;
                    std::array<int32_t, 4> g = {-1, -1, -1, -1};
                    int n = 0;
                    for (int b = 0; b < 4; ++b)
                        if (ids[b] >= 0 && d->textures[ids[b]].width == d->textures[ids[a]].width && d->textures[ids[b]].height == d->textures[ids[a]].height) {
                            g[b] = ids[b];
                            ++n;
                        }
                    if (n > best_n) {
                        best_n = n;
                        group = g;
                    }
                }
                if (best_n >= 2 && pool.size() < budget) {
                    std::vector<int32_t> v;
                    store({group[0], group[1], group[2], group[3]}, 4, v);
                    for (int a = 0; a < 4; ++a)
                        views[a] = v[a];
                }
                for (int a = 0; a < 4; ++a)
                    if (ids[a] >= 0 && views[a] < 0)
                        views[a] = alone_view(ids[a]);
                sets.push_back({ids, views});
            }
            o.color_tex = views[0];
            o.emissive_tex = views[1];
            o.mr_tex = views[2];
            o.normal_tex = views[3];
            o.tex_set = -1;
            o.tex_set_info = 0;
            uint32_t present = 0;
            int first = -1;
            bool one_set = true;
            for (int a = 0; a < 4; ++a) {
                if (views[a] < 0)
                    continue;
                present |= 1u << a;
                const DevTexture &t = texs[views[a]];
                if (t.stride != 4u)
                    one_set = false;
                else if (first < 0)
                    first = a;
                else if (t.offset - (uint32_t)a != texs[views[first]].offset - (uint32_t)first)
                    one_set = false;
            }
            if (one_set && first >= 0) {
                o.tex_set = views[first];
                o.tex_set_info = present | ((uint32_t)first << 4);
            }
        }
        if (d->bg_texture >= 0)
            P.bg_view = alone_view(d->bg_texture);
        if (pool.size() >= ((size_t)1 << 32))
            return rt::fail(RT_ERR_OOM, "rt_create: texture pool exceeds 2^32 texels");
    }
    if (d->n_primitives) {
        if (!d->primitives || d->n_primitives > RT_MAX_PRIMITIVES)
            return rt::fail(RT_ERR_INVALID_ARG, "rt_create: bad primitive list (limit " + std::to_string(RT_MAX_PRIMITIVES) + ")");
        P.prims.assign(d->primitives, d->primitives + d->n_primitives);
        for (const rt_primitive_desc &pr : P.prims)
            if ((pr.kind != RT_PRIM_ELLIPSOID && pr.kind != RT_PRIM_PLANE) || pr.material_id >= d->n_materials)
                return rt::fail(RT_ERR_INVALID_ARG, "rt_create: primitive with unknown kind or material id out of range");
    }
    P.lut_lin.resize(256);
    P.lut_gam.resize(256);
    for (int k = 0; k < 256; ++k) {
        P.lut_lin[k] = k / 255.0f;
        P.lut_gam[k] = std::pow(P.lut_lin[k], 2.2f);
    }
    geometry_task.get();
    P.geo = G;
    return RT_OK;
}

int rt::upload_geometry(rt_scene *s, const rt_scene_desc *d, const rt::PreparedScene &PS, const rt::PreparedGeometry &P, rt::GeometryOnDevice &out,
                        const rt::DeviceArrays *arrays) {
    const bool dev_build = P.dev_build, wide_build = P.wide_build;
    rt::DeviceBvh dbvh{};
    rt::WideBvh wide_local;
    std::vector<DevTri> wide_tris_local;
    std::vector<DevAttr> attrs_local;
    const rt::WideBvh *wide = &P.wide;
    const std::vector<DevTri> *wide_tris = &P.wide_tris;
    const std::vector<DevAttr> *attrs = &P.attrs;
    out.build_ms = P.build_ms;
    out.wide_ms = P.wide_ms;
    if (dev_build) {
        const char *what = "";
        const bool device_collapse = wide_build && !(d->build_flags & RT_BUILD_WIDE_HOST_COLLAPSE);
        if (arrays && wide_build && (!device_collapse || d->n_triangles <= 8u))
            return rt::fail(RT_ERR_INVALID_ARG, "upload_geometry: the host collapse reads the arrays on the host");
        hipError_t be = arrays ? rt::build_bvh_device_arrays(*arrays, d->build, s->stream, &dbvh, &what, device_collapse, PS.wide_cost_node, PS.wide_cost_tri)
                               : rt::build_bvh_device(d, s->stream, &dbvh, &what, device_collapse, PS.wide_cost_node, PS.wide_cost_tri);
        if (be != hipSuccess)
            return rt::fail(be == hipErrorOutOfMemory ? RT_ERR_OOM : RT_ERR_HIP, std::string("device BVH build: ") + what + ": " + hipGetErrorString(be));
        out.device_built = true;
        out.build_ms = dbvh.build_ms;
        out.build_upload_ms = dbvh.upload_ms;
        if (!wide_build) {
            out.owned.push_back(dbvh.nodes);
            out.owned.push_back(dbvh.tris);
            out.owned.push_back(dbvh.attrs);
        } else if (dbvh.wide) {
            out.owned.push_back(dbvh.tris);
            out.owned.push_back(dbvh.attrs);
            out.wide_ms = dbvh.wide_ms;
        } else {
            const auto tw0 = std::chrono::steady_clock::now();
            std::vector<DevNode> hn(dbvh.n_inner);
            std::vector<DevTri> ht(dbvh.n_tris);
            hipError_t ce = hipSuccess;
            if (dbvh.n_inner)
                ce = hipMemcpy(hn.data(), dbvh.nodes, sizeof(DevNode) * hn.size(), hipMemcpyDeviceToHost);
            if (ce == hipSuccess && dbvh.n_tris)
                ce = hipMemcpy(ht.data(), dbvh.tris, sizeof(DevTri) * ht.size(), hipMemcpyDeviceToHost);
            (void)hipFree(dbvh.nodes);
            (void)hipFree(dbvh.tris);
            (void)hipFree(dbvh.attrs);
            dbvh.nodes = nullptr, dbvh.tris = nullptr, dbvh.attrs = nullptr;
            if (ce != hipSuccess)
                return rt::fail(RT_ERR_HIP, std::string("wide build: reading the device BVH back: ") + hipGetErrorString(ce));
            wide_local = rt::build_wide(rt::bin_from_device(hn, ht, dbvh.root), d->positions, PS.wide_cost_node, PS.wide_cost_tri);
            make_wide_tris(d, wide_local, wide_tris_local);
            make_attrs(d, wide_tris_local, attrs_local);
            wide = &wide_local, wide_tris = &wide_tris_local, attrs = &attrs_local;
            out.wide_ms = std::chrono::duration<double, std::milli>(std::chrono::steady_clock::now() - tw0).count();
        }
    }
    const bool wide_on_device = wide_build && dbvh.wide != nullptr;
    if (wide_on_device)
        out.owned.push_back(dbvh.wide);
    if (wide_build) {
        out.wide_built = true;
        out.wide_depth = wide_on_device ? dbvh.wide_depth : wide->depth;
        out.wide_cost = wide_on_device ? 0.0 : wide->sah_cost;
        if (out.wide_depth > (uint32_t)RT_MAX_STACK)
            return rt::fail(RT_ERR_UNSUPPORTED, "rt_create: the 8-wide tree is " + std::to_string(out.wide_depth) + " levels deep, the traversal stacks hold " +
                                                    std::to_string(RT_MAX_STACK) + ": build the scene without RT_BUILD_WIDE");
    }
    int rc;
    for (int w = 0; w < 2; ++w) {
        DevBvh &b = w == 0 ? out.scene : out.lights;
        std::vector<void *> &owned = w == 0 ? out.owned : out.light_owned;
        if (w == 0 && wide_build) {
            const WideNode *d_wide80 = nullptr;
            std::vector<void *> wide80_owned;
            struct FreeWide80 {
                std::vector<void *> &v;
                ~FreeWide80() {
                    for (void *q : v)
                        (void)hipFree(q);
                }
            } free_wide80{wide80_owned};
            WideGrid grid{};
            if (wide_on_device) {
                d_wide80 = dbvh.wide;
                out.owned.pop_back();
                wide80_owned.push_back(dbvh.wide);
                b.tris = dbvh.tris;
                b.n_tris = dbvh.n_tris;
                b.n_wide = dbvh.n_wide;
                grid = dbvh.wide_grid;
            } else {
                if ((rc = upload(wide->nodes, &d_wide80, wide80_owned)) != RT_OK)
                    return rc;
                if ((rc = upload(*wide_tris, &b.tris, owned)) != RT_OK)
                    return rc;
                b.n_tris = (uint32_t)wide_tris->size();
                b.n_wide = (uint32_t)wide->nodes.size();
                grid = wide->grid;
                HIP_TRY(hipDeviceSynchronize());
            }
            if (b.n_wide != 0u && !rt::wide_grid_in_range(grid))
                return rt::fail(RT_ERR_UNSUPPORTED, "rt_create: the scene's extent is outside the 8-wide tree's exponent range (2^-52 .. 2^52): build without RT_BUILD_WIDE");
            uint4_pod *blob = nullptr;
            uint32_t n_units = 0;
            const char *what = "";
            if (hipError_t pe = rt::pack_wide_device(d_wide80, b.n_wide, b.tris, grid, s->stream, &blob, &n_units, &what); pe != hipSuccess)
                return rt::fail(pe == hipErrorOutOfMemory ? RT_ERR_OOM : RT_ERR_HIP, std::string("wide pack: ") + what + ": " + hipGetErrorString(pe));
            if (blob)
                owned.push_back(blob);
            b.wide = blob;
            b.n_units = n_units;
            b.grid = grid;
            b.nodes = nullptr;
            b.root = b.n_wide == 0u ? RT_NONE : 0u;
            b.fast_ok = 0u;
            out.dev_n_inner[0] = 0;
            continue;
        }
        if (w == 0 && dev_build) {
            b.nodes = dbvh.nodes;
            b.tris = dbvh.tris;
            b.root = dbvh.root;
            b.n_tris = dbvh.n_tris;
            b.fast_ok = dbvh.fast_ok ? 1u : 0u;
            out.dev_n_inner[0] = dbvh.n_inner;
            continue;
        }
        if ((rc = upload(P.flat[w].nodes, &b.nodes, owned)) != RT_OK)
            return rc;
        if ((rc = upload(P.flat[w].tris, &b.tris, owned)) != RT_OK)
            return rc;
        b.root = P.flat[w].root;
        b.n_tris = (uint32_t)P.flat[w].tris.size();
        b.fast_ok = P.flat[w].fast_ok ? 1u : 0u;
        b.lds_inner = w == 1 ? rt::light_lds_inner(P.flat[w]) : 0u;
        out.dev_n_inner[w] = (uint32_t)P.flat[w].nodes.size();
    }
    if (dev_build && (!wide_build || wide_on_device))
        out.attrs = dbvh.attrs;
    else if ((rc = upload(*attrs, &out.attrs, out.owned)) != RT_OK)
        return rc;
    if ((rc = upload(P.laux, &out.light_aux, out.light_owned)) != RT_OK)
        return rc;
    for (int k = 0; k < 3; ++k) {
        float lo = 0.f, hi = 1.f;
        if (dev_build) {
            lo = dbvh.lo[k];
            hi = dbvh.hi[k];
        } else if (P.host_bvh[0].root != RT_NONE && !P.host_bvh[0].nodes.empty()) {
            lo = P.host_bvh[0].nodes[P.host_bvh[0].root].lo[k];
            hi = P.host_bvh[0].nodes[P.host_bvh[0].root].hi[k];
        }
        rt::sort_bounds_axis(lo, hi, out.bounds_lo[k], out.bounds_inv[k]);
    }
    return RT_OK;
}

void rt::install_geometry(rt_scene *s, rt::GeometryOnDevice &g) {
    DevScene &D = s->dev;
    D.scene = g.scene;
    D.lights = g.lights;
    D.attrs = g.attrs;
    D.light_aux = g.light_aux;
    std::memcpy(D.bounds_lo, g.bounds_lo, 12);
    std::memcpy(D.bounds_inv, g.bounds_inv, 12);
    s->geo_owned = std::move(g.owned);
    s->light_owned = std::move(g.light_owned);
    g.owned.clear();
    g.light_owned.clear();
    s->device_built = g.device_built;
    s->wide_built = g.wide_built;
    s->wide_depth = g.wide_depth;
    s->wide_ms = g.wide_ms;
    s->wide_cost = g.wide_cost;
    s->build_ms = g.build_ms;
    s->build_upload_ms = g.build_upload_ms;
    s->dev_n_inner[0] = g.dev_n_inner[0];
    s->dev_n_inner[1] = g.dev_n_inner[1];
}

static int create_impl(const rt_scene_desc *d, const std::shared_ptr<const rt::PreparedScene> &prep, int device, rt_scene *s) {
    const rt::PreparedScene &P = *prep;
    int ndev = 0;
    if (hipGetDeviceCount(&ndev) != hipSuccess || ndev == 0)
        return rt::fail(RT_ERR_NO_DEVICE, "rt_create: no HIP device available (this library has no CPU fallback)");
    if (device < 0 || device >= ndev)
        return rt::fail(RT_ERR_INVALID_ARG, "rt_create: device ordinal out of range");
    s->device = device;
    s->prep = prep;
    s->geo = prep->geo;
    HIP_TRY(hipSetDevice(device));
    hipDeviceProp_t prop;
    HIP_TRY(hipGetDeviceProperties(&prop, device));
    s->num_cus = prop.multiProcessorCount;
    HIP_TRY(hipStreamCreateWithFlags(&s->stream, hipStreamNonBlocking));
    HIP_TRY(hipEventCreate(&s->ev0));
    HIP_TRY(hipEventCreate(&s->ev1));

    DevScene &D = s->dev;
    int rc;
    {
        rt::GeometryOnDevice g;
        rc = rt::upload_geometry(s, d, P, *prep->geo, g);
        if (rc == RT_OK)
            rt::install_geometry(s, g);
        else
            g.free_all();
        if (rc != RT_OK)
            return rc;
    }
    if ((rc = upload(P.mats, &D.materials, s->owned)) != RT_OK)
        return rc;
    if ((rc = upload(P.texs, &D.textures, s->owned)) != RT_OK)
        return rc;
    if ((rc = upload(P.pool, &D.texels, s->owned)) != RT_OK)
        return rc;
    if ((rc = upload(P.lut_lin, &D.lut_linear, s->owned)) != RT_OK)
        return rc;
    if ((rc = upload(P.lut_gam, &D.lut_gamma, s->owned)) != RT_OK)
        return rc;
    if ((rc = upload(P.prims, &D.prims, s->owned)) != RT_OK)
        return rc;
    D.n_prims = (uint32_t)P.prims.size();
    D.n_triangles = d->n_triangles;
    rt::set_camera(D, d->camera.position, d->camera.right, d->camera.up, d->camera.forward);
    std::memcpy(D.bg, d->bg_color, 12);
    D.bg_tex = P.bg_view;
    D.ray_depth = d->ray_depth;
    s->cam = d->camera;

    void *p = nullptr;
    HIP_TRY(hipMalloc(&p, sizeof(uint32_t) * 64));
    s->owned.push_back(p);
    s->d_counter = static_cast<uint32_t *>(p);
    HIP_TRY(hipMalloc(&p, sizeof(DevStats)));
    s->owned.push_back(p);
    s->d_stats = static_cast<DevStats *>(p);
    HIP_TRY(hipDeviceSynchronize());
    return RT_OK;
}

static int check_desc(const rt_scene_desc *desc, const void *out) {
    if (!desc || !out)
        return rt::fail(RT_ERR_INVALID_ARG, "rt_create: null argument");
    if (desc->abi_version != RT_ABI_VERSION)
        return rt::fail(RT_ERR_INVALID_ARG, "rt_create: ABI version mismatch");
    if (desc->ray_depth > RT_MAX_RAY_DEPTH)
        return rt::fail(RT_ERR_INVALID_ARG, "rt_create: ray_depth above RT_MAX_RAY_DEPTH (32)");
    if (desc->n_triangles && (!desc->positions || !desc->normals || !desc->texcoords || !desc->tangents || !desc->material_ids || !desc->materials))
        return rt::fail(RT_ERR_INVALID_ARG, "rt_create: null geometry array");
    if (desc->n_triangles > RT_LEAF_BEGIN_MASK)
        return rt::fail(RT_ERR_INVALID_ARG, "rt_create: too many triangles (limit 2^27 - 1)");
    if (desc->build_flags & ~(uint32_t)(RT_BUILD_DEVICE_LBVH | RT_BUILD_WIDE | RT_BUILD_WIDE_HOST_COLLAPSE | RT_BUILD_GROUP_COPY | RT_BUILD_GROUP_SELF_EXCHANGE))
        return rt::fail(RT_ERR_INVALID_ARG, "rt_create: unknown build_flags bit");
    if (desc->build.reserved0 || desc->build.reserved1 || desc->build.reserved)
        return rt::fail(RT_ERR_INVALID_ARG, "rt_create: reserved field of rt_build_options is not 0");
    return RT_OK;
}

int rt::create_replica(const rt_scene_desc *desc, const std::shared_ptr<const rt::PreparedScene> &prep, int device, rt_scene **out) {
    rt_scene *s = new rt_scene();
    int rc = create_impl(desc, prep, device, s);
    if (rc != RT_OK) {
        delete s;
        return rc;
    }
    *out = s;
    return RT_OK;
}
int rt::prepare(const rt_scene_desc *desc, std::shared_ptr<const rt::PreparedScene> *out) {
    auto P = std::make_shared<rt::PreparedScene>();
    if (int rc = prepare_scene(desc, *P); rc != RT_OK)
        return rc;
    *out = P;
    return RT_OK;
}
const rt::HostBvh &rt::prepared_host_bvh(const rt_scene *s, int which) { return s->geo->host_bvh[which]; }

extern "C" int rt_create_on(const rt_scene_desc *desc, const int *devices, int n_devices, rt_scene **out) {
    if (int rc = check_desc(desc, out); rc != RT_OK)
        return rc;
    if (!devices || n_devices < 1)
        return rt::fail(RT_ERR_INVALID_ARG, "rt_create_on: empty device list");
    rt::Group *g = nullptr;
    if (int rc = rt::group_create(desc, devices, n_devices, &g); rc != RT_OK)
        return rc;
    rt_scene *s = new rt_scene();
    s->group = g;
    s->device = devices[0];
    *out = s;
    return RT_OK;
}

extern "C" int rt_create(const rt_scene_desc *desc, int device, rt_scene **out) {
    if (int rc = check_desc(desc, out); rc != RT_OK)
        return rc;
    if (device == RT_ALL_DEVICES) {
        int ndev = 0;
        if (hipGetDeviceCount(&ndev) != hipSuccess || ndev == 0)
            return rt::fail(RT_ERR_NO_DEVICE, "rt_create: no HIP device available (this library has no CPU fallback)");
        std::vector<int> all(ndev);
        for (int i = 0; i < ndev; ++i)
            all[i] = i;
        return rt_create_on(desc, all.data(), ndev, out);
    }
    int ndev = 0;
    if (hipGetDeviceCount(&ndev) != hipSuccess || ndev == 0)
        return rt::fail(RT_ERR_NO_DEVICE, "rt_create: no HIP device available (this library has no CPU fallback)");
    std::shared_ptr<const rt::PreparedScene> prep;
    if (int rc = rt::prepare(desc, &prep); rc != RT_OK)
        return rc;
    return rt::create_replica(desc, prep, device, out);
}

extern "C" int rt_scene_device_count(const rt_scene *scene) { return !scene ? 0 : (scene->group ? rt::group_size(scene->group) : 1); }

extern "C" void rt_destroy(rt_scene *scene) { delete scene; }

extern "C" int rt_build_times(const rt_scene *s, double *build_ms, double *upload_ms) {
    if (!s)
        return rt::fail(RT_ERR_INVALID_ARG, "rt_build_times: null argument");
    if (s->group)
        return rt_build_times(rt::group_primary(s->group), build_ms, upload_ms);
    if (build_ms)
        *build_ms = s->build_ms;
    if (upload_ms)
        *upload_ms = s->build_upload_ms;
    return RT_OK;
}

extern "C" int rt_build_times_ex(const rt_scene *s, double *build_ms, double *upload_ms, double *wide_ms) {
    if (!s)
        return rt::fail(RT_ERR_INVALID_ARG, "rt_build_times_ex: null argument");
    if (s->group)
        return rt_build_times_ex(rt::group_primary(s->group), build_ms, upload_ms, wide_ms);
    if (wide_ms)
        *wide_ms = s->wide_ms;
    return rt_build_times(s, build_ms, upload_ms);
}
```

### raytracing-course-hw-public_amd/csrc/rt_scene_impl.h

```cpp
#pragma once
#include <hip/hip_runtime_api.h>

#include <chrono>
#include <memory>
#include <string>
#include <vector>

#include "../../include/rt_abi.h"
#include "bvh_build.h"
#include "rt_bvh_device.h"
#include "rt_device_types.h"
#include "rt_error.h"
#include "rt_film.h"
#include "rt_group.h"
#include "rt_kernels.h"
#include "wide_build.h"

#define HIP_TRY(expr)                                                                                     \
    do {                                                                                                  \
        hipError_t e_ = (expr);                                                                           \
        if (e_ != hipSuccess)                                                                             \
            return rt::fail(e_ == hipErrorOutOfMemory ? RT_ERR_OOM : (e_ == hipErrorNoDevice ? RT_ERR_NO_DEVICE : RT_ERR_HIP), \
                            std::string(#expr) + ": " + hipGetErrorString(e_));                           \
    } while (0)

namespace rt {
struct PacketPolicy {
    uint64_t key = 0;
    bool off = false;
    uint32_t lanes_x100 = 0;
};

struct PreparedGeometry {
    bool dev_build = false, wide_build = false;
    HostBvh host_bvh[2];
    FlatBvh flat[2];
    WideBvh wide;
    std::vector<DevTri> wide_tris;
    std::vector<DevAttr> attrs;
    std::vector<DevLightAux> laux;
    double build_ms = 0, wide_ms = 0;
};
struct PreparedScene {
    std::shared_ptr<const PreparedGeometry> geo;
    std::vector<DevMaterial> mats;
    std::vector<DevTexture> texs;
    std::vector<uint32_t> pool;
    std::vector<rt_primitive_desc> prims;
    std::vector<float> lut_lin, lut_gam;
    int32_t bg_view = -1;
    float wide_cost_node = 1.0f, wide_cost_tri = 0.3f;
    uint32_t build_flags = 0;
    rt_build_options build{};
};

struct GeometryOnDevice {
    std::vector<void *> owned;
    std::vector<void *> light_owned;
    DevBvh scene{}, lights{};
    const DevAttr *attrs = nullptr;
    const DevLightAux *light_aux = nullptr;
    float bounds_lo[3] = {0, 0, 0}, bounds_inv[3] = {0, 0, 0};
    bool device_built = false, wide_built = false;
    uint32_t wide_depth = 0;
    double wide_ms = 0, wide_cost = 0, build_ms = 0, build_upload_ms = 0;
    uint32_t dev_n_inner[2] = {0, 0};
    void free_all() {
        for (void *p : owned)
            (void)hipFree(p);
        for (void *p : light_owned)
            (void)hipFree(p);
        owned.clear();
        light_owned.clear();
    }
};

inline bool wide_grid_in_range(const WideGrid &grid) { return !(grid.e_base + 15 < -60 || grid.e_base + 15 > 44); }
inline void sort_bounds_axis(float lo, float hi, float &bounds_lo, float &bounds_inv) {
    bounds_lo = lo;
    bounds_inv = (hi > lo) ? 1.0f / (hi - lo) : 0.0f;
}
}

struct rt_scene {
    rt::Group *group = nullptr;
    int device = 0;
    hipStream_t stream = nullptr;
    hipEvent_t ev0 = nullptr, ev1 = nullptr;
    rt::EventPool ext_events;
    DevScene dev{};
    rt_camera cam{};
    std::vector<void *> owned;
    std::vector<void *> geo_owned;
    std::vector<void *> light_owned;
    std::shared_ptr<const rt::PreparedScene> prep;
    std::shared_ptr<const rt::PreparedGeometry> geo;
    uint32_t live_accums = 0;
    bool refitted = false;
    rt::HostBvh rebuilt_bvh;
    bool device_built = false;
    bool wide_built = false;
    uint32_t wide_depth = 0;
    double wide_ms = 0, wide_cost = 0;
    uint32_t dev_n_inner[2] = {0, 0};
    double build_ms = 0, build_upload_ms = 0;
    double refit_ms = 0, refit_levels_ms = 0;
    uint32_t *d_counter = nullptr;
    DevStats *d_stats = nullptr;
    float *d_fb = nullptr;
    size_t fb_capacity = 0;
    uint8_t *d_rgb8 = nullptr;
    size_t rgb8_capacity = 0;
    WfView *d_views = nullptr;
    uint32_t views_capacity = 0;
    rt::FilmTable *d_film_table = nullptr;

    int ensure_fb(size_t fb_floats) {
        if (fb_capacity >= fb_floats)
            return RT_OK;
        if (d_fb)
            (void)hipFree(d_fb);
        d_fb = nullptr;
        fb_capacity = 0;
        void *q = nullptr;
        HIP_TRY(hipMalloc(&q, fb_floats * sizeof(float)));
        d_fb = static_cast<float *>(q);
        fb_capacity = fb_floats;
        return RT_OK;
    }
    int ensure_film(size_t rgb8_bytes) {
        if (!d_film_table) {
            rt::FilmTable t{};
            if (!rt::film_table(t.thr, t.special))
                return rt::fail(RT_ERR_UNSUPPORTED, "device film: the host libm's powf failed the monotonicity check; use rt_render + rt_tonemap_rgb8");
            void *q = nullptr;
            HIP_TRY(hipMalloc(&q, sizeof(t)));
            d_film_table = static_cast<rt::FilmTable *>(q);
            HIP_TRY(hipMemcpyAsync(d_film_table, &t, sizeof(t), hipMemcpyHostToDevice, stream));
            HIP_TRY(hipStreamSynchronize(stream));
        }
        if (rgb8_capacity < rgb8_bytes) {
            if (d_rgb8)
                (void)hipFree(d_rgb8);
            d_rgb8 = nullptr;
            rgb8_capacity = 0;
            void *q = nullptr;
            HIP_TRY(hipMalloc(&q, rgb8_bytes));
            d_rgb8 = static_cast<uint8_t *>(q);
            rgb8_capacity = rgb8_bytes;
        }
        return RT_OK;
    }
    int ensure_views(uint32_t n) {
        if (views_capacity >= n)
            return RT_OK;
        if (d_views)
            (void)hipFree(d_views);
        d_views = nullptr;
        views_capacity = 0;
        void *q = nullptr;
        HIP_TRY(hipMalloc(&q, (size_t)n * sizeof(WfView)));
        d_views = static_cast<WfView *>(q);
        views_capacity = n;
        return RT_OK;
    }
    void *d_rays = nullptr;
    size_t rays_capacity = 0;
    int ensure_rays(size_t bytes) {
        if (rays_capacity >= bytes)
            return RT_OK;
        if (d_rays)
            (void)hipFree(d_rays);
        d_rays = nullptr;
        rays_capacity = 0;
        HIP_TRY(hipMalloc(&d_rays, bytes));
        rays_capacity = bytes;
        return RT_OK;
    }
    int num_cus = 0;
    int blocks_per_cu = 8;
    uint64_t wf_paths_cap = 0, wf_pixels_cap = 0;
    uint32_t wf_depth_cap = 0;
    std::vector<void *> wf_owned;
    WfPath *wf_paths[2] = {nullptr, nullptr};
    uint32_t *wf_stripes = nullptr;
    WfHit *wf_hits = nullptr;
    WfFold *wf_fold = nullptr;
    RtF4 *wf_samples = nullptr, *wf_accum = nullptr;
    uint32_t *wf_counters = nullptr;
    void *wf_stack_overflow = nullptr;
    uint32_t wf_stack_stride = 0;
    uint32_t *wf_sort_keys[2] = {nullptr, nullptr}, *wf_sort_vals[2] = {nullptr, nullptr};
    void *wf_sort_temp = nullptr;
    size_t wf_sort_temp_bytes = 0;
    uint32_t *wf_host_count = nullptr;
    std::vector<hipEvent_t> wf_count_events;
    rt::PacketPolicy pkt;
    std::vector<hipEvent_t> pass_events;

    int ensure_wavefront(uint64_t paths, uint64_t pixels, uint32_t depth) {
        if (paths <= wf_paths_cap && pixels <= wf_pixels_cap && depth <= wf_depth_cap)
            return RT_OK;
        for (void *p : wf_owned)
            (void)hipFree(p);
        wf_owned.clear();
        wf_paths_cap = wf_pixels_cap = 0;
        wf_depth_cap = 0;
        auto alloc = [&](size_t bytes, void **out) -> int {
            *out = nullptr;
            hipError_t e = hipMalloc(out, bytes ? bytes : 16);
            if (e != hipSuccess)
                return rt::fail(e == hipErrorOutOfMemory ? RT_ERR_OOM : RT_ERR_HIP, std::string("wavefront workspace: ") + hipGetErrorString(e));
            wf_owned.push_back(*out);
            return RT_OK;
        };
        int rc;
        if ((rc = alloc((paths + 64) * sizeof(WfPath), (void **)&wf_paths[0])) != RT_OK || (rc = alloc((paths + 64) * sizeof(WfPath), (void **)&wf_paths[1])) != RT_OK ||
            (rc = alloc(WF_STRIPE_BUF_WORDS * sizeof(uint32_t), (void **)&wf_stripes)) != RT_OK ||
            (rc = alloc(paths * sizeof(WfHit), (void **)&wf_hits)) != RT_OK || (rc = alloc(paths * depth * sizeof(WfFold), (void **)&wf_fold)) != RT_OK ||
            (rc = alloc(paths * sizeof(RtF4), (void **)&wf_samples)) != RT_OK || (rc = alloc(pixels * sizeof(RtF4), (void **)&wf_accum)) != RT_OK ||
            (rc = alloc(WF_CNT_ALLOC_WORDS * sizeof(uint32_t), (void **)&wf_counters)) != RT_OK)
            return rc;
        wf_stack_stride = (uint32_t)num_cus * 8u * 256u;
        if ((rc = alloc((size_t)RT_MAX_STACK * wf_stack_stride * 16, &wf_stack_overflow)) != RT_OK)
            return rc;
        wf_sort_temp_bytes = rt::wavefront_sort_temp_bytes(paths);
        if ((rc = alloc(paths * 4, (void **)&wf_sort_keys[0])) != RT_OK || (rc = alloc(paths * 4, (void **)&wf_sort_keys[1])) != RT_OK ||
            (rc = alloc(paths * 4, (void **)&wf_sort_vals[0])) != RT_OK || (rc = alloc(paths * 4, (void **)&wf_sort_vals[1])) != RT_OK ||
            (rc = alloc(wf_sort_temp_bytes, &wf_sort_temp)) != RT_OK)
            return rc;
        HIP_TRY(hipMemsetAsync(wf_counters, 0, WF_CNT_ALLOC_WORDS * sizeof(uint32_t), stream));
        wf_paths_cap = paths;
        wf_pixels_cap = pixels;
        wf_depth_cap = depth;
        return RT_OK;
    }

    RtF4 *wf_feat = nullptr;
    uint64_t wf_feat_cap = 0;
    int ensure_features() {
        if (wf_feat_cap >= wf_paths_cap)
            return RT_OK;
        if (wf_feat)
            (void)hipFree(wf_feat);
        wf_feat = nullptr;
        wf_feat_cap = 0;
        void *q = nullptr;
        hipError_t e = hipMalloc(&q, wf_paths_cap * 2 * sizeof(RtF4));
        if (e != hipSuccess)
            return rt::fail(e == hipErrorOutOfMemory ? RT_ERR_OOM : RT_ERR_HIP, std::string("feature records: ") + hipGetErrorString(e));
        wf_feat = static_cast<RtF4 *>(q);
        wf_feat_cap = wf_paths_cap;
        return RT_OK;
    }

    void wf_bind(WfLaunch &W) {
        W.paths_in = wf_paths[0];
        W.paths_out = wf_paths[1];
        W.hits = wf_hits;
        W.fold = wf_fold;
        W.sample_out = wf_samples;
        W.accum = wf_accum;
        W.counters = wf_counters;
        W.stripes = wf_stripes;
        W.stack_overflow = wf_stack_overflow;
        W.stack_stride = wf_stack_stride;
        for (int k = 0; k < 2; ++k) {
            W.sort_keys[k] = wf_sort_keys[k];
            W.sort_vals[k] = wf_sort_vals[k];
        }
        W.sort_temp = wf_sort_temp;
        W.sort_temp_bytes = wf_sort_temp_bytes;
        W.packet_census = reinterpret_cast<unsigned long long *>(wf_counters + WF_CNT_CENSUS);
    }

    ~rt_scene() {
        if (group) {
            rt::group_destroy(group);
            return;
        }
        (void)hipSetDevice(device);
        if (wf_host_count)
            (void)hipHostFree(wf_host_count);
        for (hipEvent_t ev : wf_count_events)
            (void)hipEventDestroy(ev);
        for (hipEvent_t ev : pass_events)
            (void)hipEventDestroy(ev);
        for (void *p : wf_owned)
            (void)hipFree(p);
        for (void *p : owned)
            (void)hipFree(p);
        for (void *p : geo_owned)
            (void)hipFree(p);
        for (void *p : light_owned)
            (void)hipFree(p);
        if (wf_feat)
            (void)hipFree(wf_feat);
        if (d_fb)
            (void)hipFree(d_fb);
        if (d_rgb8)
            (void)hipFree(d_rgb8);
        if (d_views)
            (void)hipFree(d_views);
        if (d_rays)
            (void)hipFree(d_rays);
        if (d_film_table)
            (void)hipFree(d_film_table);
        ext_events.destroy();
        if (ev0)
            (void)hipEventDestroy(ev0);
        if (ev1)
            (void)hipEventDestroy(ev1);
        if (stream)
            (void)hipStreamDestroy(stream);
    }
};

namespace rt {
const HostBvh &prepared_host_bvh(const rt_scene *s, int which);
void prepare_geometry(const rt_scene_desc *d, const std::vector<uint8_t> &emissive, float wide_cost_node, float wide_cost_tri, PreparedGeometry &P,
                      bool lights_only = false);
void prepare_lights(const float *positions, uint32_t n_total, const std::vector<uint32_t> &lights, const uint32_t *original, PreparedGeometry &P);
int upload_geometry(rt_scene *s, const rt_scene_desc *d, const PreparedScene &PS, const PreparedGeometry &P, GeometryOnDevice &out,
                    const DeviceArrays *arrays = nullptr);
void install_geometry(rt_scene *s, GeometryOnDevice &g);
uint32_t light_lds_inner(const FlatBvh &f);
WfView make_view(const rt_camera &cam, uint32_t width, uint32_t height, uint64_t seed);
void set_camera(DevScene &D, const float *pos, const float *right, const float *up, const float *fwd);
int check_pass_params(const rt_params *p, const char *fn);
uint64_t wavefront_max_paths(rt_scene *s, const rt_params *p);
hipError_t launch_pass(rt_scene *s, const rt_params *p, PacketPolicy &pol, WfLaunch &W, uint32_t n_views, bool first_pass, bool last_pass, bool time_extends,
                       const WfAccum *acc, const WfFeat *feat = nullptr, const WfRays *rays = nullptr);
int fill_stats(rt_scene *s, bool counters, uint64_t samples, float kernel_ms, std::chrono::steady_clock::time_point wall0, rt_stats *stats);

template <class Queue> int queue_and_wait(rt_scene *s, Queue queue) {
    if (int rc = queue(); rc != RT_OK) {
        (void)hipStreamSynchronize(s->stream);
        return rc;
    }
    HIP_TRY(hipStreamSynchronize(s->stream));
    return RT_OK;
}
}
```

### raytracing-course-hw-public_amd/csrc/rt_update.cpp

```cpp
#include <cmath>
#include <cstring>

#include "rt_scene_impl.h"
#include "rt_update_dev.h"
#include "rt_wide_refit.h"
#include "wide_grid.h"

namespace {

int check_struct(const rt_geometry_update *u, const std::string &fn, bool device) {
    if (!u)
        return rt::fail(RT_ERR_INVALID_ARG, fn + ": null argument");
    if (u->mode != RT_UPDATE_REBUILD && u->mode != RT_UPDATE_REFIT)
        return rt::fail(RT_ERR_INVALID_ARG, fn + ": unknown mode");
    for (uint32_t r : u->reserved)
        if (r)
            return rt::fail(RT_ERR_INVALID_ARG, fn + ": reserved field is not 0");
    if (u->n_triangles && (!u->positions || !u->normals || !u->texcoords || !u->tangents || !u->material_ids))
        return rt::fail(RT_ERR_INVALID_ARG, fn + ": null geometry array");
    if (device)
        for (const void *p : {(const void *)u->positions, (const void *)u->normals, (const void *)u->texcoords, (const void *)u->tangents, (const void *)u->material_ids})
            if ((uintptr_t)p & 3u)
                return rt::fail(RT_ERR_INVALID_ARG, fn + ": misaligned geometry array (device pointers must be 4-byte aligned)");
    return RT_OK;
}
int check_scene(const rt_scene *s, const rt_geometry_update *u, const std::string &fn) {
    if (!s)
        return rt::fail(RT_ERR_INVALID_ARG, fn + ": null scene");
    if (s->group)
        return rt::fail(RT_ERR_UNSUPPORTED, fn + ": multi-GPU scenes cannot be updated");
    if (u->n_triangles != s->dev.n_triangles)
        return rt::fail(RT_ERR_INVALID_ARG, fn + ": n_triangles is " + std::to_string(u->n_triangles) + ", the scene has " + std::to_string(s->dev.n_triangles));
    if (s->live_accums)
        return rt::fail(RT_ERR_INVALID_ARG, fn + ": the scene has " + std::to_string(s->live_accums) +
                                                " live accumulator(s), whose sums are of the old geometry: destroy them first");
    return RT_OK;
}
int refuse_material(const std::string &fn) { return rt::fail(RT_ERR_INVALID_ARG, fn + ": material id out of range"); }
int refuse_non_finite(const std::string &fn, size_t triangle) {
    return rt::fail(RT_ERR_INVALID_ARG, fn + ": non-finite vertex position (triangle " + std::to_string(triangle) + ")");
}
int check_data(const rt_scene *s, const rt_geometry_update *u, const std::string &fn) {
    const size_t n_mats = s->prep->mats.size();
    for (uint32_t i = 0; i < u->n_triangles; ++i)
        if (u->material_ids[i] >= n_mats)
            return refuse_material(fn);
    for (size_t i = 0; i < (size_t)u->n_triangles * 9; ++i)
        if (!std::isfinite(u->positions[i]))
            return refuse_non_finite(fn, i / 9);
    return RT_OK;
}
bool check_mode_ok(const rt_scene *s, const rt_geometry_update *u) { return !(u->mode == RT_UPDATE_REFIT && !(s->prep->build_flags & RT_BUILD_WIDE)); }
int check_mode(const rt_scene *s, const rt_geometry_update *u, const std::string &fn) {
    if (!check_mode_ok(s, u))
        return rt::fail(RT_ERR_UNSUPPORTED, fn + ": RT_UPDATE_REFIT needs a scene built with RT_BUILD_WIDE (a refitted binary tree is "
                                                 "not the reference's topology): use RT_UPDATE_REBUILD");
    return RT_OK;
}

const std::string FN_HOST = "rt_update_geometry", FN_DEVICE = "rt_update_geometry_device";

rt_scene_desc geometry_desc(const rt_scene *s, const rt_geometry_update *u) {
    rt_scene_desc d{};
    d.abi_version = RT_ABI_VERSION;
    d.n_triangles = u->n_triangles;
    d.positions = u->positions;
    d.normals = u->normals;
    d.texcoords = u->texcoords;
    d.tangents = u->tangents;
    d.material_ids = u->material_ids;
    d.n_materials = (uint32_t)s->prep->mats.size();
    d.build_flags = s->prep->build_flags;
    d.build = s->prep->build;
    return d;
}

std::vector<uint8_t> emissive_materials(const rt::PreparedScene &P) {
    std::vector<uint8_t> em(P.mats.size());
    for (size_t i = 0; i < em.size(); ++i) {
        const float *e = P.mats[i].emission;
        em[i] = !((e[0] == 0) & (e[1] == 0) & (e[2] == 0));
    }
    return em;
}

void free_list(std::vector<void *> &v) {
    for (void *p : v)
        (void)hipFree(p);
    v.clear();
}

int rebuild_from(rt_scene *s, const rt_scene_desc &d, const std::shared_ptr<rt::PreparedGeometry> &G, const rt::DeviceArrays *arrays, const std::string &fn) {
    const rt::PreparedScene &P = *s->prep;
    rt::GeometryOnDevice g;
    int rc = rt::upload_geometry(s, &d, P, *G, g, arrays);
    hipError_t se = rc == RT_OK ? hipDeviceSynchronize() : hipSuccess;
    if (rc == RT_OK && se != hipSuccess)
        rc = rt::fail(RT_ERR_HIP, fn + ": " + hipGetErrorString(se));
    if (rc != RT_OK) {
        g.free_all();
        return rc;
    }
    std::vector<void *> old_geo = std::move(s->geo_owned), old_light = std::move(s->light_owned);
    rt::install_geometry(s, g);
    free_list(old_geo);
    free_list(old_light);
    s->geo = G;
    s->refitted = false;
    return RT_OK;
}

int rebuild(rt_scene *s, const rt_scene_desc &d, const std::string &fn) {
    const rt::PreparedScene &P = *s->prep;
    auto G = std::make_shared<rt::PreparedGeometry>();
    rt::prepare_geometry(&d, emissive_materials(P), P.wide_cost_node, P.wide_cost_tri, *G);
    return rebuild_from(s, d, G, nullptr, fn);
}

int refit_from(rt_scene *s, const std::shared_ptr<rt::PreparedGeometry> &G, const rt::RefitInput &in, const std::string &fn);

int refit(rt_scene *s, const rt_geometry_update *u, const rt_scene_desc &d) {
    const rt::PreparedScene &P = *s->prep;
    if (u->n_triangles == 0)
        return RT_OK;
    auto G = std::make_shared<rt::PreparedGeometry>();
    rt::prepare_geometry(&d, emissive_materials(P), P.wide_cost_node, P.wide_cost_tri, *G, true);
    rt::RefitInput in;
    const char *what = "";
    if (hipError_t e = rt::refit_upload(u, s->stream, &in, &what); e != hipSuccess)
        return rt::fail(e == hipErrorOutOfMemory ? RT_ERR_OOM : RT_ERR_HIP, std::string("rt_update_geometry: ") + what + ": " + hipGetErrorString(e));
    struct FreeInput {
        rt::RefitInput &in;
        ~FreeInput() { in.free_all(); }
    } free_input{in};
    return refit_from(s, G, in, FN_HOST);
}

int refit_from(rt_scene *s, const std::shared_ptr<rt::PreparedGeometry> &G, const rt::RefitInput &in, const std::string &fn) {
    DevScene &D = s->dev;
    const char *what = "";
    const WideGrid grid = rt::make_wide_grid(in.lo, in.hi);
    if (D.scene.n_wide != 0u && !rt::wide_grid_in_range(grid))
        return rt::fail(RT_ERR_UNSUPPORTED, fn + ": the new extent is outside the 8-wide tree's exponent range (2^-52 .. 2^52)");
    rt::GeometryOnDevice lg;
    auto upload_lights = [&]() -> int {
        auto up = [&](const void *src, size_t bytes, const void **dst) -> int {
            *dst = nullptr;
            if (!bytes)
                return RT_OK;
            void *p = nullptr;
            HIP_TRY(hipMalloc(&p, bytes));
            lg.light_owned.push_back(p);
            HIP_TRY(hipMemcpyAsync(p, src, bytes, hipMemcpyHostToDevice, s->stream));
            *dst = p;
            return RT_OK;
        };
        const rt::FlatBvh &f = G->flat[1];
        int rc;
        if ((rc = up(f.nodes.data(), f.nodes.size() * sizeof(DevNode), (const void **)&lg.lights.nodes)) != RT_OK ||
            (rc = up(f.tris.data(), f.tris.size() * sizeof(DevTri), (const void **)&lg.lights.tris)) != RT_OK ||
            (rc = up(G->laux.data(), G->laux.size() * sizeof(DevLightAux), (const void **)&lg.light_aux)) != RT_OK)
            return rc;
        HIP_TRY(hipStreamSynchronize(s->stream));
        return RT_OK;
    };
    if (int rc = upload_lights(); rc != RT_OK) {
        (void)hipStreamSynchronize(s->stream);
        lg.free_all();
        return rc;
    }
    double levels_ms = 0;
    const auto t_refit = std::chrono::steady_clock::now();
    if (hipError_t e = rt::refit_wide_device(in, const_cast<DevTri *>(D.scene.tris), const_cast<DevAttr *>(D.attrs), D.scene.n_tris, const_cast<uint4_pod *>(D.scene.wide),
                                             D.scene.n_units, D.scene.n_wide, grid, s->stream, &what, &levels_ms);
        e != hipSuccess) {
        (void)hipStreamSynchronize(s->stream);
        lg.free_all();
        return rt::fail(e == hipErrorOutOfMemory ? RT_ERR_OOM : RT_ERR_HIP, fn + ": " + what + ": " + hipGetErrorString(e));
    }
    const rt::FlatBvh &f = G->flat[1];
    DevBvh &L = D.lights;
    const DevNode *ln = lg.lights.nodes;
    const DevTri *lt = lg.lights.tris;
    L = DevBvh{};
    L.nodes = ln;
    L.tris = lt;
    L.root = f.root;
    L.n_tris = (uint32_t)f.tris.size();
    L.fast_ok = f.fast_ok ? 1u : 0u;
    L.lds_inner = rt::light_lds_inner(f);
    D.light_aux = lg.light_aux;
    s->dev_n_inner[1] = (uint32_t)f.nodes.size();
    free_list(s->light_owned);
    s->light_owned = std::move(lg.light_owned);
    D.scene.grid = grid;
    for (int k = 0; k < 3; ++k)
        rt::sort_bounds_axis(in.lo[k], in.hi[k], D.bounds_lo[k], D.bounds_inv[k]);
    s->refit_ms = std::chrono::duration<double, std::milli>(std::chrono::steady_clock::now() - t_refit).count();
    s->refit_levels_ms = levels_ms;
    s->geo = G;
    s->refitted = true;
    return RT_OK;
}

int check_device_pointers(const rt_scene *s, const rt_geometry_update *u) {
    const size_t n = u->n_triangles;
    const struct {
        const void *p;
        size_t bytes;
    } arrays[5] = {{u->positions, 36 * n}, {u->normals, 36 * n}, {u->texcoords, 24 * n}, {u->tangents, 36 * n}, {u->material_ids, 4 * n}};
    for (const auto &a : arrays)
        for (const char *q : {(const char *)a.p, (const char *)a.p + a.bytes - 1}) {
            hipPointerAttribute_t at{};
            const hipError_t e = hipPointerGetAttributes(&at, q);
            if (e != hipSuccess)
                (void)hipGetLastError();
            if (e != hipSuccess || at.type != hipMemoryTypeDevice || at.device != s->device)
                return rt::fail(RT_ERR_INVALID_ARG, FN_DEVICE + ": a geometry array is not device memory of the scene's GPU (device " + std::to_string(s->device) + ")");
        }
    return RT_OK;
}

int lights_from_scan(const rt::UpdateScan &scan, uint32_t n, rt::PreparedGeometry &G) {
    const size_t nl = scan.light_prims.size();
    for (size_t k = 0; k < nl; ++k)
        if (scan.light_prims[k] >= n || (k && scan.light_prims[k] <= scan.light_prims[k - 1]))
            return rt::fail(RT_ERR_INVALID_ARG, FN_DEVICE + ": the arrays changed during the call (they must be idle on entry)");
    std::vector<uint32_t> all(nl);
    for (size_t k = 0; k < nl; ++k)
        all[k] = (uint32_t)k;
    rt::prepare_lights(scan.light_pos.data(), n == 0 ? 0u : (uint32_t)std::max<size_t>(nl, 1), all, scan.light_prims.data(), G);
    return RT_OK;
}

int rebuild_staged(rt_scene *s, const rt_geometry_update *u) {
    const size_t n = u->n_triangles;
    std::vector<float> pos(9 * n), nrm(9 * n), uv(6 * n), tan(9 * n);
    std::vector<uint32_t> mat(n);
    if (n) {
        HIP_TRY(hipMemcpyAsync(pos.data(), u->positions, 36 * n, hipMemcpyDeviceToHost, s->stream));
        HIP_TRY(hipMemcpyAsync(nrm.data(), u->normals, 36 * n, hipMemcpyDeviceToHost, s->stream));
        HIP_TRY(hipMemcpyAsync(uv.data(), u->texcoords, 24 * n, hipMemcpyDeviceToHost, s->stream));
        HIP_TRY(hipMemcpyAsync(tan.data(), u->tangents, 36 * n, hipMemcpyDeviceToHost, s->stream));
        HIP_TRY(hipMemcpyAsync(mat.data(), u->material_ids, 4 * n, hipMemcpyDeviceToHost, s->stream));
        HIP_TRY(hipStreamSynchronize(s->stream));
    }
    rt_geometry_update h = *u;
    h.positions = pos.data(), h.normals = nrm.data(), h.texcoords = uv.data(), h.tangents = tan.data(), h.material_ids = mat.data();
    return rebuild(s, geometry_desc(s, &h), FN_DEVICE);
}

}

extern "C" int rt_update_geometry(rt_scene *s, const rt_geometry_update *u) {
    int rc;
    if ((rc = check_struct(u, FN_HOST, false)) != RT_OK || (rc = check_scene(s, u, FN_HOST)) != RT_OK || (rc = check_data(s, u, FN_HOST)) != RT_OK ||
        (rc = check_mode(s, u, FN_HOST)) != RT_OK)
        return rc;
    HIP_TRY(hipSetDevice(s->device));
    HIP_TRY(hipStreamSynchronize(s->stream));
    const rt_scene_desc d = geometry_desc(s, u);
    rc = u->mode == RT_UPDATE_REFIT ? refit(s, u, d) : rebuild(s, d, FN_HOST);
    if (rc == RT_OK) {
        s->pkt = rt::PacketPolicy{};
        s->rebuilt_bvh = rt::HostBvh{};
    }
    return rc;
}

extern "C" int rt_refit_times(const rt_scene *s, double *refit_ms, double *levels_ms) {
    if (!s || !refit_ms || !levels_ms)
        return rt::fail(RT_ERR_INVALID_ARG, "rt_refit_times: null argument");
    if (s->group)
        return rt::fail(RT_ERR_UNSUPPORTED, "rt_refit_times: multi-GPU scenes cannot be updated");
    *refit_ms = s->refit_ms;
    *levels_ms = s->refit_levels_ms;
    return RT_OK;
}

extern "C" int rt_update_geometry_device(rt_scene *s, const rt_geometry_update *u) {
    int rc;
    if ((rc = check_struct(u, FN_DEVICE, true)) != RT_OK || (rc = check_scene(s, u, FN_DEVICE)) != RT_OK)
        return rc;
    HIP_TRY(hipSetDevice(s->device));
    const uint32_t n = u->n_triangles;
    if (n && (rc = check_device_pointers(s, u)) != RT_OK)
        return rc;
    HIP_TRY(hipStreamSynchronize(s->stream));
    const rt::PreparedScene &P = *s->prep;
    const bool dev_build = n > 0 && (P.build_flags & RT_BUILD_DEVICE_LBVH), wide_build = n > 0 && (P.build_flags & RT_BUILD_WIDE);
    const bool refit = u->mode == RT_UPDATE_REFIT;
    const bool staged = !refit && (!dev_build || (wide_build && ((P.build_flags & RT_BUILD_WIDE_HOST_COLLAPSE) || n <= 8u)));
    rt::DeviceArrays arrays;
    arrays.pos = u->positions, arrays.nrm = u->normals, arrays.uv = u->texcoords, arrays.tan = u->tangents, arrays.mat = u->material_ids, arrays.n = n;
    rt::UpdateScan scan;
    const char *what = "";
    const bool want_lights = !staged && check_mode_ok(s, u);
    if (hipError_t e = rt::scan_update_device(arrays, emissive_materials(P), want_lights, s->stream, &scan, &what); e != hipSuccess)
        return rt::fail(e == hipErrorOutOfMemory ? RT_ERR_OOM : RT_ERR_HIP, FN_DEVICE + ": " + what + ": " + hipGetErrorString(e));
    if (scan.bad_material)
        return refuse_material(FN_DEVICE);
    if (scan.first_non_finite != RT_NONE)
        return refuse_non_finite(FN_DEVICE, scan.first_non_finite);
    if ((rc = check_mode(s, u, FN_DEVICE)) != RT_OK)
        return rc;
    if (staged)
        rc = rebuild_staged(s, u);
    else if (refit && n == 0)
        rc = RT_OK;
    else {
        auto G = std::make_shared<rt::PreparedGeometry>();
        G->dev_build = dev_build, G->wide_build = wide_build;
        if ((rc = lights_from_scan(scan, n, *G)) != RT_OK)
            return rc;
        if (refit) {
            rt::RefitInput in;
            in.pos = const_cast<float *>(u->positions), in.nrm = const_cast<float *>(u->normals), in.uv = const_cast<float *>(u->texcoords);
            in.tan = const_cast<float *>(u->tangents), in.mat = const_cast<uint32_t *>(u->material_ids), in.n = n;
            std::memcpy(in.lo, scan.lo, 12);
            std::memcpy(in.hi, scan.hi, 12);
            rc = refit_from(s, G, in, FN_DEVICE);
        } else {
            rt_geometry_update none = *u;
            none.positions = none.normals = none.texcoords = none.tangents = nullptr;
            none.material_ids = nullptr;
            rc = rebuild_from(s, geometry_desc(s, &none), G, &arrays, FN_DEVICE);
        }
    }
    if (rc == RT_OK) {
        s->pkt = rt::PacketPolicy{};
        s->rebuilt_bvh = rt::HostBvh{};
    }
    return rc;
}
```

### raytracing-course-hw-public_amd/csrc/rt_wavefront.hip

```cpp
#include <cstring>
#include <vector>

#include <rocprim/rocprim.hpp>

#include "rt_dev_queue.h"
#include "rt_dev_shade.h"
#include "rt_dev_stack.h"
#include "rt_kernels.h"
#include "rt_wf_records.h"

namespace {

#ifndef RT_EXT_WAVES_PER_SIMD
#define RT_EXT_WAVES_PER_SIMD 6
#endif
#ifndef RT_EXT_LDS_DEPTH
#define RT_EXT_LDS_DEPTH 6
#endif
#ifndef RT_EXT_GB_LDS_DEPTH
#define RT_EXT_GB_LDS_DEPTH 9
#endif
#ifndef RT_SHADE_WAVES_PER_SIMD
#define RT_SHADE_WAVES_PER_SIMD 4
#endif
#ifndef RT_SHADE_BLOCKS_PER_CU
#define RT_SHADE_BLOCKS_PER_CU 8
#endif
#ifndef RT_SHADE_LDS_DEPTH
#define RT_SHADE_LDS_DEPTH 4
#endif
using ShadeStack = StackMemT<RT_SHADE_LDS_DEPTH>;
#ifndef RT_EXT_CHUNK
#define RT_EXT_CHUNK 64u
#endif
#ifndef RT_EXT_REFILL_MIN
#define RT_EXT_REFILL_MIN 16
#endif

DEV uint32_t wf_global_pixel(const WfLaunch &L, uint32_t local_pixel) {
    const uint32_t local_block = local_pixel / L.shard_block;
    const uint32_t within = local_pixel - local_block * L.shard_block;
    return (local_block * L.shard_count + L.shard_index) * L.shard_block + within;
}

DEV void wf_store_first(const DevScene &S, const WfLaunch &L, uint32_t i, V3 o, V3 d, const Rng<RT_RNG_DEVICE> &rng) {
    wf_store_path(L.paths_in + i, wf_pack(o, d, i, next_shade_class(rng, S.lights.n_tris != 0), L.ray_depth, 0u, rng.g));
}

DEV void wf_primary_ray(const DevScene &S, const WfLaunch &L, uint32_t i, uint32_t v, uint32_t pix, uint32_t s) {
    const uint32_t v0 = __builtin_amdgcn_readfirstlane(v);
    WfView view;
    if (__ballot(v != v0) == 0ull)
        view = L.views[v0];
    else
        view = L.views[v];
    const V3 cam_pos = ld3(view.pos), cam_right = ld3(view.right), cam_up = ld3(view.up), cam_fwd = ld3(view.fwd);
    Rng<RT_RNG_DEVICE> rng;
    rt_xoshiro_seed(&rng.g, view.seed, pix, s);
    const V3 rd = gen_ray_dir(rng, pix, L.width, L.height, view.tan_x, view.tan_y, cam_right, cam_up, cam_fwd);
    wf_store_first(S, L, i, cam_pos, rd, rng);
}

template <bool STATS> __global__ __launch_bounds__(256) void wf_generate(const DevScene S, const WfLaunch L) {
    LaneStats<STATS> st;
    if (blockIdx.x == 0 && threadIdx.x == 0)
        L.counters[WF_CNT_IN] = L.n_paths;
    for (uint32_t i = blockIdx.x * blockDim.x + threadIdx.x; i < L.n_paths; i += gridDim.x * blockDim.x) {
        const uint32_t lp = i / L.pass_samples;
        const uint32_t ds = i - lp * L.pass_samples;
        const uint32_t vpix = wf_global_pixel(L, L.first_pixel + lp);
        const uint32_t v = vpix / L.view_pixels;
        const uint32_t pix = vpix - v * L.view_pixels;
        const uint32_t s = L.first_sample + ds;
        wf_primary_ray(S, L, i, v, pix, s);
        st.cast();
    }
    st.flush(L.stats);
}

template <bool STATS> __global__ __launch_bounds__(256) void wf_generate_list(const DevScene S, const WfLaunch L, const WfAccum A) {
    LaneStats<STATS> st;
    const uint32_t *off = A.list_off + A.first_entry;
    const uint32_t base = off[0], n_exact = off[A.n_entries] - base;
    if (blockIdx.x == 0 && threadIdx.x == 0)
        L.counters[WF_CNT_IN] = n_exact;
    for (uint32_t i = blockIdx.x * blockDim.x + threadIdx.x; i < L.n_paths; i += gridDim.x * blockDim.x) {
        if (i >= n_exact) {
            L.sample_out[i] = RtF4{0.f, 0.f, 0.f, __uint_as_float(0u)};
            continue;
        }
        const uint32_t g = base + i;
        uint32_t lo = 0, hi = A.n_entries - 1;
        while (lo < hi) {
            const uint32_t mid = (lo + hi + 1u) >> 1;
            if (off[mid] <= g)
                lo = mid;
            else
                hi = mid - 1u;
        }
        const uint32_t e = A.first_entry + lo;
        wf_primary_ray(S, L, i, 0u, A.list_pix[e], A.list_base[e] + (g - off[lo]));
        st.cast();
    }
    st.flush(L.stats);
}

template <bool STATS> __global__ __launch_bounds__(256) void wf_generate_rays(const DevScene S, const WfLaunch L, const WfRays R) {
    LaneStats<STATS> st;
    if (blockIdx.x == 0 && threadIdx.x == 0)
        L.counters[WF_CNT_IN] = L.n_paths;
    const uint4 *recs = reinterpret_cast<const uint4 *>(R.rays);
    for (uint32_t i = blockIdx.x * blockDim.x + threadIdx.x; i < L.n_paths; i += gridDim.x * blockDim.x) {
        const uint32_t lp = i / L.pass_samples;
        const uint32_t ds = L.first_sample + (i - lp * L.pass_samples);
        const uint32_t sub = ds / R.samples;
        const size_t ray = (size_t)(L.first_pixel + lp) * R.group + sub;
        const uint4 p0 = recs[2 * ray], p1 = recs[2 * ray + 1];
        Rng<RT_RNG_DEVICE> rng;
        rt_xoshiro_seed(&rng.g, R.seed, p1.z, p1.w + (ds - sub * R.samples));
        (void)uniform_real(rng, 0.0f, 1.0f);
        (void)uniform_real(rng, 0.0f, 1.0f);
        wf_store_first(S, L, i, mk(__uint_as_float(p0.x), __uint_as_float(p0.y), __uint_as_float(p0.z)),
                       mk(__uint_as_float(p0.w), __uint_as_float(p1.x), __uint_as_float(p1.y)), rng);
        st.cast();
    }
    st.flush(L.stats);
}

template <bool STATS> DEV void leaf_batch(Trav &T, const DevBvh &bvh, bool at_leaf, const CoopLds<float2> &lds, LaneStats<STATS> &st) {
    coop_tri_batch<RT_LEAF_COOP_MAX>(
        at_leaf, at_leaf ? RT_LEAF_CNT(T.cur) : 0u, T.cur & RT_LEAF_BEGIN_MASK, T.o, T.d, bvh.tris, lds, [](int t) { return (uint32_t)t; },
        [](uint32_t k0, uint32_t e) { return k0 + e; }, st);
    if (at_leaf) {
        st.node();
        float t;
        uint32_t k;
        float2 bc;
        if (coop_result(lds, t, k, bc)) {
            hit_take(T.best, k, bc.x, bc.y, t);
            T.t_loc = fminf(T.t_loc, t);
        }
        T.cur = T_POP;
    }
}

#ifndef RT_EXT_LEAF_MIN
#define RT_EXT_LEAF_MIN 20
#endif

template <bool STATS, bool GB> __global__ __launch_bounds__(256, RT_EXT_WAVES_PER_SIMD) void wf_extend(const DevScene S, const WfLaunch L) {
    constexpr int DEPTH = GB ? RT_EXT_GB_LDS_DEPTH : RT_EXT_LDS_DEPTH, WORDS = GB ? 2 : 3;
    __shared__ uint32_t s_stack[STACK_LDS_DWORDS(DEPTH, WORDS)];
    __shared__ uint16_t s_owner_all[4][64 * RT_LEAF_COOP_MAX + RT_LEAF_COOP_MAX];
    __shared__ unsigned long long s_min_all[4][64];
    __shared__ float2 s_bc_all[4][64];
    const uint32_t wave = threadIdx.x >> 6;
    const CoopLds<float2> s_coop{s_owner_all[wave], s_min_all[wave], s_bc_all[wave]};
    LaneStats<STATS> st;
    RT_DECLARE_RING_STACK_W(stk, DEPTH, WORDS, s_stack, L.stack_overflow, L.stack_stride);
    const uint32_t n_in = L.counters[WF_CNT_IN];
    Trav T;
    T.cur = T_DONE;
    T.sp = 0;
    uint32_t slot = RT_NONE;
    bool exhausted = n_in == 0;
    uint32_t q_lo = 0, q_hi = 0;
    TicketState tks = ticket_init();
    for (;;) {
        ticket_refill(L.counters, n_in, (uint32_t)RT_EXT_CHUNK, RT_EXT_REFILL_MIN, T.cur == T_DONE, exhausted, q_lo, q_hi, tks, [&](uint32_t jq) {
            const WfRay ray = wf_load_ray(L.paths_in + wf_order_slot(L, jq));
            slot = jq;
            trav_init_stored<GB>(T, S.scene, ray.o, ray.d, ray.r, ray.fast);
            stk.reset();
            if (T.cur == T_DONE)
                wf_store_hit(L.hits + jq, wf_miss());
        });
        const bool was_live = T.cur != T_DONE;
        trav_pop_once<GB>(T, stk);
        if (was_live && T.cur == T_DONE)
            wf_store_hit(L.hits + slot, T.best);
        const bool active = T.cur != T_DONE;
        const bool popping = T.cur == T_POP;
        const bool at_leaf = active && !popping && (T.cur & RT_LEAF_FLAG) != 0 && RT_LEAF_CNT(T.cur) != 0;
        const bool stepper = active && !popping && !at_leaf;
        const unsigned long long lm = __ballot(at_leaf), sm = __ballot(stepper);
        if ((lm | sm) == 0ull) {
            if (__ballot(popping) != 0ull)
                continue;
            if (exhausted)
                break;
            continue;
        }
        if (sm == 0ull || __popcll(lm) >= RT_EXT_LEAF_MIN) {
            leaf_batch<STATS>(T, S.scene, at_leaf, s_coop, st);
        } else {
            const bool plain = (T.cur & RT_LEAF_FLAG) == 0 && T.fast;
            if (__ballot(stepper && !plain) == 0ull) {
                if (stepper) {
                    trav_step_inner_fast<STATS, GB>(T, S.scene, stk, EPS, st);
                }
            } else if (stepper) {
                trav_step_core<STATS, GB>(T, S.scene, stk, EPS, st);
            }
        }
    }
    st.flush(L.stats);
}

#ifndef RT_PKT_CHUNK
#define RT_PKT_CHUNK 256u
#endif
template <bool STATS, bool GB> __global__ __launch_bounds__(256, RT_EXT_WAVES_PER_SIMD) void wf_extend_packet(const DevScene S, const WfLaunch L) {
    constexpr int DEPTH = GB ? RT_EXT_GB_LDS_DEPTH : RT_EXT_LDS_DEPTH, WORDS = GB ? 2 : 3;
    __shared__ uint32_t s_stack[STACK_LDS_DWORDS(DEPTH, WORDS)];
    LaneStats<STATS> st;
    RT_DECLARE_RING_STACK_W(stk, DEPTH, WORDS, s_stack, L.stack_overflow, L.stack_stride);
    const uint32_t n_in = L.counters[WF_CNT_IN];
    const uint32_t lane = threadIdx.x & 63u;
    Trav T = trav_idle<GB>();
    unsigned long long n_trips = 0ull, n_lanes = 0ull;
    for (;;) {
        uint32_t base = 0;
        if (lane == 0u)
            base = atomicAdd(L.counters + WF_CNT_TICKET, (uint32_t)RT_PKT_CHUNK);
        base = (uint32_t)__builtin_amdgcn_readfirstlane((int)base);
        if (base >= n_in)
            break;
        for (uint32_t q0 = base; q0 < base + RT_PKT_CHUNK && q0 < n_in; q0 += 64u) {
            const uint32_t jq = q0 + lane;
            const bool have = jq < n_in;
            T.cur = T_DONE;
            if (have) {
                const WfRay ray = wf_load_ray(L.paths_in + wf_order_slot(L, jq));
                trav_init_stored<GB>(T, S.scene, ray.o, ray.d, ray.r, ray.fast);
                stk.reset();
            }
            for (;;) {
                trav_pop_wave<GB>(T, stk);
                const uint32_t target = wave_min_u32(T.cur);
                if (target == T_DONE)
                    break;
                const bool mine = T.cur == target;
                const unsigned long long mm = __ballot(mine);
                if (mm == 0ull)
                    break;
                ++n_trips;
                n_lanes += (uint32_t)__popcll(mm);
                if ((target & RT_LEAF_FLAG) == 0u) {
                    uint32_t node_index = target;
                    asm volatile("" : "+s"(node_index));
                    ConstF4 p = as_const_f4(S.scene.nodes + node_index);
                    const F4v r0 = p[0], r1 = p[1], r2 = p[2], r3 = p[3];
                    if (mine)
                        trav_inner_apply<STATS, GB>(T, stk, node_rec(r0, r1, r2, r3), EPS, st);
                } else {
                    const uint32_t cnt = RT_LEAF_CNT(target);
                    uint32_t k = target & RT_LEAF_BEGIN_MASK;
                    for (uint32_t i = 0;; ++i, ++k) {
                        ConstF4 p = as_const_f4(S.scene.tris + k);
                        const F4v r0 = p[0], r1 = p[1], r2 = p[2];
                        const TriRec tri = tri_rec(r0, r1, r2);
                        if (mine) {
                            if (tri.flags & 2u)
                                st.node();
                            st.tri();
                            V3 xs;
                            if (tri_hit(tri, T.o, T.d, EPS, xs)) {
                                hit_take(T.best, k, xs.x, xs.y, xs.z);
                                T.t_loc = fminf(T.t_loc, xs.z);
                            }
                        }
                        if (cnt != 0u ? i + 1u == cnt : (tri.flags & 1u) != 0u)
                            break;
                    }
                    if (mine)
                        T.cur = T_POP;
                }
            }
            if (have)
                wf_store_hit(L.hits + jq, T.best);
        }
    }
    census_flush(L.packet_census, n_trips, n_lanes);
    st.flush(L.stats);
}

__global__ __launch_bounds__(256) void wf_extend_prims(const DevScene S, const WfLaunch L) {
    const uint32_t n_in = L.counters[WF_CNT_IN];
    for (uint32_t jq = blockIdx.x * blockDim.x + threadIdx.x; jq < n_in; jq += gridDim.x * blockDim.x) {
        const WfHead ray = wf_load_head(L.paths_in + wf_order_slot(L, jq));
        Hit h = wf_load_hit(L.hits + jq);
        const uint32_t k0 = h.k;
        prims_closest(S, ray.o, ray.d, h);
        if (h.k != k0)
            wf_store_hit(L.hits + jq, h);
    }
}

__global__ __launch_bounds__(256) void wf_features(const DevScene S, const WfLaunch L, const WfFeat F) {
    __shared__ float s_lin[256];
    __shared__ float s_gam[256];
    s_lin[threadIdx.x] = S.lut_linear[threadIdx.x];
    s_gam[threadIdx.x] = S.lut_gamma[threadIdx.x];
    __syncthreads();
    LaneStats<false> st;
    const uint32_t n_in = L.counters[WF_CNT_IN];
    for (uint32_t i = blockIdx.x * blockDim.x + threadIdx.x; i < n_in; i += gridDim.x * blockDim.x) {
        const WfHead in = wf_load_head(L.paths_in + i);
        const Hit h = wf_load_hit(L.hits + i);
        RtF4 r0{0.f, 0.f, 0.f, 0.f}, r1{0.f, 0.f, 0.f, __uint_as_float(0u)};
        if (h.k != RT_NONE) {
            const Surf sf = make_surf<false>(S, h, in.o, in.d, s_lin, s_gam, st);
            r0 = RtF4{sf.color.r, sf.color.g, sf.color.b, h.t};
            r1 = RtF4{sf.shading_normal.x, sf.shading_normal.y, sf.shading_normal.z, __uint_as_float(1u)};
        }
        F.rec[2ull * in.id] = r0;
        F.rec[2ull * in.id + 1] = r1;
    }
}

template <bool STATS, bool LIGHTS_LDS, bool ENV> __global__ __launch_bounds__(256, RT_SHADE_WAVES_PER_SIMD) void wf_shade(const DevScene S, const WfLaunch L) {
    __shared__ float s_lin[256];
    __shared__ float s_gam[256];
    __shared__ uint32_t s_stack[STACK_LDS_DWORDS(RT_SHADE_LDS_DEPTH, 3)];
    __shared__ float4 s_lights[LIGHTS_LDS ? RT_SHADE_LIGHTS_F4 : 1];
    __shared__ uint2 s_perm[4][256];
    LightTabs LT = light_tabs_global(S);
    if (LIGHTS_LDS) {
        const uint32_t n_node_f4 = 4u * (S.lights.lds_inner - 1u), n_tri_f4 = 3u * S.lights.n_tris;
        for (uint32_t i = threadIdx.x; i < n_node_f4; i += blockDim.x)
            s_lights[i] = LT.nodes[i];
        for (uint32_t i = threadIdx.x; i < n_tri_f4; i += blockDim.x)
            s_lights[n_node_f4 + i] = LT.tris[i];
        for (uint32_t i = threadIdx.x; i < S.lights.n_tris; i += blockDim.x)
            s_lights[n_node_f4 + n_tri_f4 + i] = LT.aux[i];
        LT = LightTabs{s_lights, s_lights + n_node_f4, s_lights + n_node_f4 + n_tri_f4};
    }
    s_lin[threadIdx.x] = S.lut_linear[threadIdx.x];
    s_gam[threadIdx.x] = S.lut_gamma[threadIdx.x];
    __syncthreads();
    LaneStats<STATS> st;
    RT_DECLARE_STACK(stk, RT_SHADE_LDS_DEPTH, s_stack);
    const bool has_lights = S.lights.n_tris != 0;
    const uint32_t n_in = L.counters[WF_CNT_IN];
    const uint32_t n_slots = (n_in + 63u) >> 6;
    auto shade_wave = [&](const uint32_t jq, const uint32_t j, const uint32_t wave_slot) {
        const bool active = jq < n_in;
        bool survive = false;
        WfPacked next;
        if (active) {
            const WfHead in = wf_load_head(L.paths_in + j);
            Rng<RT_RNG_DEVICE> rng = wf_load_rng(L.paths_in + j);
            const Hit h = wf_load_hit(L.hits + jq);
            const uint32_t path = in.id;
            uint32_t depth_left = in.depth_left, nb = in.nb;
            if (h.k != RT_NONE)
                depth_left -= 1;
            const ShadeResult sr = shade_hit<Rng<RT_RNG_DEVICE>, STATS, ENV>(S, LT, h, in.o, in.d, rng, has_lights, stk, s_lin, s_gam, st);
            bool terminal = sr.terminal;
            V3 term = sr.term;
            if (sr.push)
                wf_store_fold(wf_fold_at(L.fold, L.n_paths, nb++, path), sr.emission, sr.scl);
            if (!terminal && depth_left == 0) {
                terminal = true;
                term = mk(0, 0, 0);
            }
            if (terminal) {
                L.sample_out[path] = RtF4{term.x, term.y, term.z, __uint_as_float(nb)};
                st.sample();
            } else {
                survive = true;
                st.cast();
                next = wf_pack(sr.nro, sr.nrd, path, next_shade_class(rng, has_lights), depth_left, nb, rng.g);
            }
        }
        const unsigned long long m = __ballot(survive);
        if (m != 0ull) {
            const uint32_t rank = lane_rank(m);
            uint32_t obase = 0;
            const int leader = __ffsll((long long)m) - 1;
            const uint32_t stripe =  (uint32_t)__builtin_amdgcn_readfirstlane((int)wave_slot) % WF_STRIPES;
            if ((int)(threadIdx.x & 63u) == leader)
                obase = wf_stripe_base(stripe, n_slots) + atomicAdd(L.stripes + stripe * WF_STRIPE_WORDS, (uint32_t)__popcll(m));
            obase = __shfl(obase, leader);
            if (survive)
                wf_store_path(L.paths_out + obase + rank, next);
        }
    };
    const uint32_t lane = threadIdx.x & 63u, wv = threadIdx.x >> 6;
    const uint32_t win = (L.order_classed && n_in >= gridDim.x * 1024u) ? 256u : 64u;
    for (uint32_t wbase = (blockIdx.x * 4u + wv) * win; wbase < n_in; wbase += gridDim.x * 4u * win) {
        uint32_t slot_of[4], cls[4], before[3] = {0u, 0u, 0u}, within[4];
#pragma unroll
        for (uint32_t q = 0; q < 4u; ++q) {
            const uint32_t jq = wbase + 64u * q + lane;
            slot_of[q] = jq, cls[q] = 3u;
            if (64u * q < win && jq < n_in) {
                const uint32_t v = wf_order_word(L, jq);
                slot_of[q] = wf_word_slot(v), cls[q] = wf_word_class(v);
            }
        }
#pragma unroll
        for (uint32_t q = 0; q < 4u; ++q) {
            const unsigned long long b0 = __ballot(cls[q] == 0u), b1 = __ballot(cls[q] == 1u), b2 = __ballot(cls[q] == 2u);
            const unsigned long long mine = cls[q] == 0u ? b0 : cls[q] == 1u ? b1 : cls[q] == 2u ? b2 : ~(b0 | b1 | b2);
            const uint32_t seen = cls[q] == 0u ? before[0] : cls[q] == 1u ? before[1] : cls[q] == 2u ? before[2] : 64u * q - before[0] - before[1] - before[2];
            within[q] = seen + lane_rank(mine);
            before[0] += (uint32_t)__popcll(b0), before[1] += (uint32_t)__popcll(b1), before[2] += (uint32_t)__popcll(b2);
        }
#pragma unroll
        for (uint32_t q = 0; q < 4u; ++q) {
            const uint32_t start = cls[q] == 0u ? 0u : cls[q] == 1u ? before[0] : cls[q] == 2u ? before[0] + before[1] : before[0] + before[1] + before[2];
            s_perm[wv][start + within[q]] = make_uint2(wbase + 64u * q + lane, slot_of[q]);
        }
        __builtin_amdgcn_wave_barrier();
        const uint32_t n_here = n_in - wbase < win ? n_in - wbase : win;
        for (uint32_t sub = 0; 64u * sub < n_here; ++sub) {
            const uint2 pj = s_perm[wv][64u * sub + lane];
            shade_wave(pj.x, pj.y, (wbase >> 6) + sub);
        }
        __builtin_amdgcn_wave_barrier();
    }
    st.flush(L.stats);
}

DEV uint32_t spread3(uint32_t v) {
    v &= 63u;
    v = (v | (v << 8)) & 0x0300Fu;
    v = (v | (v << 4)) & 0x030C3u;
    v = (v | (v << 2)) & 0x09249u;
    return v;
}
__global__ __launch_bounds__(256) void wf_sort_keys(const DevScene S, const WfLaunch L, int direct, uint32_t bound) {
    __shared__ uint32_t s_run[WF_STRIPES + 1u];
    const uint32_t n = L.counters[WF_CNT_IN], n_slots = L.counters[WF_CNT_SLOTS];
    if (threadIdx.x <= WF_STRIPES)
        s_run[threadIdx.x] = L.stripes[WF_STRIPES * WF_STRIPE_WORDS + threadIdx.x];
    __syncthreads();
    if (!direct)
        for (uint32_t j = n + blockIdx.x * blockDim.x + threadIdx.x; j < bound; j += gridDim.x * blockDim.x) {
            L.sort_keys[0][j] = 0xFFFFFFFFu;
            L.sort_vals[0][j] = 0u;
        }
    for (uint32_t j = blockIdx.x * blockDim.x + threadIdx.x; j < n; j += gridDim.x * blockDim.x) {
        uint32_t pos = j;
        if (n_slots != 0u) {
            uint32_t k = 0;
#pragma unroll
            for (uint32_t step = WF_STRIPES / 2u; step != 0u; step >>= 1)
                if (s_run[k + step] <= j)
                    k += step;
            pos = wf_stripe_base(k, n_slots) + (j - s_run[k]);
        }
        if (direct) {
            L.sort_vals[1][j] = pos;
            continue;
        }
        const WfHead ray = wf_load_head(L.paths_in + pos);
        const V3 o = ray.o, d = ray.d;
        const float fx = (o.x - S.bounds_lo[0]) * S.bounds_inv[0], fy = (o.y - S.bounds_lo[1]) * S.bounds_inv[1], fz = (o.z - S.bounds_lo[2]) * S.bounds_inv[2];
        const uint32_t cx = (uint32_t)fminf(fmaxf(fx * 64.0f, 0.0f), 63.0f), cy = (uint32_t)fminf(fmaxf(fy * 64.0f, 0.0f), 63.0f), cz = (uint32_t)fminf(fmaxf(fz * 64.0f, 0.0f), 63.0f);
        const uint32_t morton = spread3(cx) | (spread3(cy) << 1) | (spread3(cz) << 2);
        const uint32_t oct = (d.x < 0.0f ? 1u : 0u) | (d.y < 0.0f ? 2u : 0u) | (d.z < 0.0f ? 4u : 0u);
        const float ax = __builtin_fabsf(d.x), ay = __builtin_fabsf(d.y), az = __builtin_fabsf(d.z);
        const uint32_t sub = (ax > ay ? 1u : 0u) | (ay > az ? 2u : 0u) | (ax > az ? 4u : 0u);
        L.sort_keys[0][j] = (oct << 21) | (morton << 3) | sub;
        L.sort_vals[0][j] = wf_word(pos, ray.cls);
    }
}

__global__ __launch_bounds__(64) void wf_advance(uint32_t *counters, uint32_t *stripes) {
    const uint32_t k = threadIdx.x;
    const uint32_t c = stripes[k * WF_STRIPE_WORDS];
    uint32_t incl = c;
#pragma unroll
    for (uint32_t d = 1; d < WF_STRIPES; d <<= 1) {
        const uint32_t up = __shfl_up(incl, d);
        if (k >= d)
            incl += up;
    }
    uint32_t *run_start = stripes + WF_STRIPES * WF_STRIPE_WORDS;
    run_start[k] = incl - c;
    stripes[k * WF_STRIPE_WORDS] = 0u;
    if (k == WF_STRIPES - 1u) {
        run_start[WF_STRIPES] = incl;
        counters[WF_CNT_SLOTS] = (counters[WF_CNT_IN] + 63u) >> 6;
        counters[WF_CNT_IN] = incl;
        counters[WF_CNT_TICKET] = 0;
    }
    if (k < 8u)
        counters[WF_CNT_XCD + k * WF_CNT_XCD_STRIDE] = 0u;
}

__global__ __launch_bounds__(256) void wf_fold(const WfLaunch L) {
    for (uint32_t path = blockIdx.x * blockDim.x + threadIdx.x; path < L.n_paths; path += gridDim.x * blockDim.x) {
        const RtF4 v = L.sample_out[path];
        V3 res = mk(v.x, v.y, v.z);
        uint32_t nb = __float_as_uint(v.w);
        while (nb > 0) {
            --nb;
            V3 emission, scl;
            wf_load_fold(wf_fold_at(L.fold, L.n_paths, nb, path), emission, scl);
            const V3 clr = res * scl;
            res = emission + clr;
        }
        if (isnan_f(res.x))
            res.x = 0;
        if (isnan_f(res.y))
            res.y = 0;
        if (isnan_f(res.z))
            res.z = 0;
        L.sample_out[path] = RtF4{res.x, res.y, res.z, 0.f};
    }
}

__global__ __launch_bounds__(256) void wf_resolve(const WfLaunch L, int first_pass, int last_pass) {
    for (uint32_t lp = blockIdx.x * blockDim.x + threadIdx.x; lp < L.pass_pixels; lp += gridDim.x * blockDim.x) {
        V3 acc = mk(0, 0, 0);
        if (!first_pass) {
            const RtF4 a = L.accum[lp];
            acc = mk(a.x, a.y, a.z);
        }
        const RtF4 *src = L.sample_out + (size_t)lp * L.pass_samples;
        for (uint32_t ds = 0; ds < L.pass_samples; ++ds) {
            const RtF4 v = src[ds];
            acc = acc + mk(v.x, v.y, v.z);
        }
        if (last_pass) {
            const V3 out = acc / (float)L.samples;
            float *dst = L.fb + 3ull * wf_global_pixel(L, L.first_pixel + lp);
            dst[0] = out.x;
            dst[1] = out.y;
            dst[2] = out.z;
        } else {
            L.accum[lp] = RtF4{acc.x, acc.y, acc.z, 0.f};
        }
    }
}

__global__ __launch_bounds__(256) void wf_resolve_list(const WfLaunch L, const WfAccum A) {
    const uint32_t *off = A.list_off + A.first_entry;
    for (uint32_t le = blockIdx.x * blockDim.x + threadIdx.x; le < A.n_entries; le += gridDim.x * blockDim.x) {
        const uint32_t e = A.first_entry + le, p = A.list_pix[e], s0 = A.list_base[e];
        const uint32_t k = off[le + 1] - off[le];
        V3 acc = ld3(A.sum + 3ull * p), ev = ld3(A.even_sum + 3ull * p);
        const RtF4 *src = L.sample_out + (off[le] - off[0]);
        for (uint32_t j = 0; j < k; ++j) {
            const RtF4 v = src[j];
            acc = acc + mk(v.x, v.y, v.z);
            if (((s0 + j) & 1u) == 0u)
                ev = ev + mk(v.x, v.y, v.z);
        }
        A.sum[3ull * p] = acc.x, A.sum[3ull * p + 1] = acc.y, A.sum[3ull * p + 2] = acc.z;
        A.even_sum[3ull * p] = ev.x, A.even_sum[3ull * p + 1] = ev.y, A.even_sum[3ull * p + 2] = ev.z;
        A.count[p] = s0 + k;
    }
}

__global__ __launch_bounds__(256) void wf_resolve_features(const WfAccum A, const WfFeat F) {
    const uint32_t *off = A.list_off + A.first_entry;
    for (uint32_t le = blockIdx.x * blockDim.x + threadIdx.x; le < A.n_entries; le += gridDim.x * blockDim.x) {
        const uint32_t p = A.list_pix[A.first_entry + le];
        const uint32_t k = off[le + 1] - off[le];
        V3 al = ld3(F.albedo_sum + 3ull * p), nr = ld3(F.normal_sum + 3ull * p);
        float z = F.depth_sum[p];
        uint32_t hits = F.hits[p];
        const RtF4 *src = F.rec + 2ull * (off[le] - off[0]);
        for (uint32_t j = 0; j < k; ++j) {
            const RtF4 r0 = src[2u * j], r1 = src[2u * j + 1u];
            al = al + mk(r0.x, r0.y, r0.z);
            nr = nr + mk(r1.x, r1.y, r1.z);
            z = z + r0.w;
            hits += __float_as_uint(r1.w);
        }
        F.albedo_sum[3ull * p] = al.x, F.albedo_sum[3ull * p + 1] = al.y, F.albedo_sum[3ull * p + 2] = al.z;
        F.normal_sum[3ull * p] = nr.x, F.normal_sum[3ull * p + 1] = nr.y, F.normal_sum[3ull * p + 2] = nr.z;
        F.depth_sum[p] = z;
        F.hits[p] = hits;
    }
}

__global__ __launch_bounds__(256) void wf_from_rays(const WfLaunch L, const float *rays, uint32_t n) {
    const uint32_t i = blockIdx.x * blockDim.x + threadIdx.x;
    if (i == 0)
        L.counters[WF_CNT_IN] = n;
    if (i >= n)
        return;
    wf_store_path(L.paths_in + i, wf_pack(ld3(rays + 6ull * i), ld3(rays + 6ull * i + 3), i, 0u, 1u, 0u, rt_xoshiro{{0u, 0u, 0u, 0u}}));
}
__global__ __launch_bounds__(256) void wf_hits_out(const DevScene S, const WfLaunch L, uint32_t n, uint32_t *prim_out, float *bct_out) {
    const uint32_t i = blockIdx.x * blockDim.x + threadIdx.x;
    if (i >= n)
        return;
    const Hit h = wf_load_hit(L.hits + i);
    const uint32_t k = h.k;
    if (k == RT_NONE) {
        prim_out[i] = RT_NONE;
        bct_out[3ull * i] = bct_out[3ull * i + 1] = bct_out[3ull * i + 2] = 0.0f;
    } else {
        prim_out[i] = (k & RT_PRIM_FLAG) ? S.n_triangles + (k & ~RT_PRIM_FLAG) : S.scene.tris[k].prim;
        bct_out[3ull * i] = h.b;
        bct_out[3ull * i + 1] = h.c;
        bct_out[3ull * i + 2] = h.t;
    }
}

}

namespace rt {

#define WF_LAUNCH(...)                                  \
    do {                                                \
        if (hipError_t le_ = RT_LAUNCH_CHECKED(__VA_ARGS__); le_ != hipSuccess) \
            return le_;                                 \
    } while (0)

static hipError_t launch_extend(const DevScene &S, const WfLaunch &L, bool packet, bool stats, int ext_blocks, hipStream_t stream) {
    if (S.scene.wide)
        return launch_extend_wide(S, L, packet, stats, ext_blocks, stream);
    return with_bools([&](auto P, auto ST, auto G) {
        if constexpr (P)
            return RT_LAUNCH_CHECKED((wf_extend_packet<ST, G>), dim3(ext_blocks), dim3(256), 0, stream, S, L);
        else
            return RT_LAUNCH_CHECKED((wf_extend<ST, G>), dim3(ext_blocks), dim3(256), 0, stream, S, L);
    }, packet, stats, L.global_best != 0u);
}

hipError_t launch_wavefront_cast(const DevScene &S, WfLaunch L, const float *rays, uint32_t n, bool packet, bool stats, uint32_t *prim, float *bct,
                                 hipStream_t stream) {
    const dim3 block(256);
    hipError_t e = hipMemsetAsync(L.counters, 0, sizeof(uint32_t) * WF_CNT_WORDS, stream);
    if (e != hipSuccess)
        return e;
    L.n_paths = n;
    L.order = nullptr, L.order_classed = 0u;
    L.packet_census = nullptr;
    const int blocks = (int)((n + 255u) / 256u);
    WF_LAUNCH(wf_from_rays, dim3(blocks), block, 0, stream, L, rays, n);
    if ((e = launch_extend(S, L, packet, stats, (int)(L.stack_stride / 256u), stream)) != hipSuccess)
        return e;
    if (S.n_prims)
        WF_LAUNCH(wf_extend_prims, dim3(blocks), block, 0, stream, S, L);
    WF_LAUNCH(wf_hits_out, dim3(blocks), block, 0, stream, S, L, n, prim, bct);
    return hipSuccess;
}

hipError_t launch_wavefront_pass(const DevScene &S, WfLaunch L, bool stats, int num_cus, bool first_pass, bool last_pass, hipStream_t stream,
                                 EventPool *extend_events, unsigned long long *packet_census_out, const WfHostSync *host_sync, const WfAccum *acc,
                                 const WfFeat *feat, const WfRays *rays) {
    const int gen_blocks = (int)((L.n_paths + 255u) / 256u < (uint32_t)num_cus * 16u ? (L.n_paths + 255u) / 256u : (uint32_t)num_cus * 16u);
    const dim3 block(256);
    hipError_t e = hipMemsetAsync(L.counters, 0, sizeof(uint32_t) * WF_CNT_WORDS, stream);
    if (e != hipSuccess)
        return e;
    if ((e = hipMemsetAsync(L.stripes, 0, sizeof(uint32_t) * WF_STRIPE_BUF_WORDS, stream)) != hipSuccess)
        return e;
    const bool packet = L.use_packet != 0u && L.packet_census != nullptr;
    if (packet && (e = hipMemsetAsync(L.packet_census, 0, 2 * sizeof(unsigned long long), stream)) != hipSuccess)
        return e;
    if (packet_census_out)
        packet_census_out[0] = packet_census_out[1] = 0ull;
    e = with_bools([&](auto ST) {
        if (acc)
            return RT_LAUNCH_CHECKED((wf_generate_list<ST>), dim3(gen_blocks > 0 ? gen_blocks : 1), block, 0, stream, S, L, *acc);
        if (rays)
            return RT_LAUNCH_CHECKED((wf_generate_rays<ST>), dim3(gen_blocks > 0 ? gen_blocks : 1), block, 0, stream, S, L, *rays);
        return RT_LAUNCH_CHECKED((wf_generate<ST>), dim3(gen_blocks > 0 ? gen_blocks : 1), block, 0, stream, S, L);
    }, stats);
    if (e != hipSuccess)
        return e;
    const int ext_blocks = (int)(L.stack_stride / 256u);
    const int shade_blocks = num_cus * RT_SHADE_BLOCKS_PER_CU;
    const WfHostSync *hs = L.sort_mode != 0u || (packet && packet_census_out) ? host_sync : nullptr;
    if (hs && (!hs->counts || !hs->events || hs->n_events < (int)L.ray_depth + 1))
        hs = nullptr;
    const bool want_bound = hs && L.sort_mode != 0u;
    uint32_t bound = L.n_paths;
    bool census_pending = false;
    for (uint32_t b = 0; b < L.ray_depth; ++b) {
        L.order = nullptr, L.order_classed = 0u;
        if (b > 0) {
            if (census_pending && b == 2) {
                if ((e = hipEventSynchronize(hs->events[0])) != hipSuccess)
                    return e;
                std::memcpy(packet_census_out, hs->counts + WF_HOST_CENSUS_WORD, 2 * sizeof(unsigned long long));
                census_pending = false;
            }
            if (want_bound && b >= 2) {
                if ((e = hipEventSynchronize(hs->events[b - 1])) != hipSuccess)
                    return e;
                bound = hs->counts[b - 1];
                if (bound == 0)
                    break;
            }
            const bool sort = want_bound && bound >= 4096u;
            const uint32_t kb = (bound + 255u) / 256u < (uint32_t)num_cus * 16u ? (bound + 255u) / 256u : (uint32_t)num_cus * 16u;
            WF_LAUNCH(wf_sort_keys, dim3(kb > 0 ? kb : 1), block, 0, stream, S, L, sort ? 0 : 1, bound);
            if (sort) {
                size_t tmp = L.sort_temp_bytes;
                hipError_t se = rocprim::radix_sort_pairs(L.sort_temp, tmp, L.sort_keys[0], L.sort_keys[1], L.sort_vals[0], L.sort_vals[1], (size_t)bound, 0u, 24u , stream);
                if (se != hipSuccess)
                    return se;
            }
            L.order = L.sort_vals[1];
            L.order_classed = sort ? 1u : 0u;
        }
        hipEvent_t e0 = extend_events ? extend_events->next() : nullptr;
        hipEvent_t e1 = e0 ? extend_events->next() : nullptr;
        if (e0 && e1)
            (void)hipEventRecord(e0, stream);
        if (hipError_t xe = launch_extend(S, L, b == 0 && packet, stats, ext_blocks, stream); xe != hipSuccess)
            return xe;
        if (e0 && e1)
            (void)hipEventRecord(e1, stream);
        if (S.n_prims)
            WF_LAUNCH(wf_extend_prims, dim3(shade_blocks), block, 0, stream, S, L);
        if (b == 0 && acc && feat)
            WF_LAUNCH(wf_features, dim3(shade_blocks), block, 0, stream, S, L, *feat);
        const bool env = S.bg_tex >= 0;
        const bool lights_lds = S.lights.lds_inner != 0u && !env;
        e = with_bools([&](auto ST, auto LDS, auto ENV) {
            if constexpr (LDS && ENV)
                return hipErrorInvalidValue;
            else
                return RT_LAUNCH_CHECKED((wf_shade<ST, LDS, ENV>), dim3(shade_blocks), block, 0, stream, S, L);
        }, stats, lights_lds, env);
        if (e != hipSuccess)
            return e;
        WF_LAUNCH(wf_advance, dim3(1), dim3(64), 0, stream, L.counters, L.stripes);
        if (hs && b == 0 && packet && packet_census_out) {
            if ((e = hipMemcpyAsync(hs->counts + WF_HOST_CENSUS_WORD, L.packet_census, 2 * sizeof(unsigned long long), hipMemcpyDeviceToHost, stream)) != hipSuccess)
                return e;
            if ((e = hipEventRecord(hs->events[0], stream)) != hipSuccess)
                return e;
            census_pending = true;
        }
        if (want_bound && b + 1 < L.ray_depth) {
            if ((e = hipMemcpyAsync(hs->counts + b + 1, L.counters + WF_CNT_IN, sizeof(uint32_t), hipMemcpyDeviceToHost, stream)) != hipSuccess)
                return e;
            if ((e = hipEventRecord(hs->events[b + 1], stream)) != hipSuccess)
                return e;
        }
        WfPath *t = L.paths_in;
        L.paths_in = L.paths_out;
        L.paths_out = t;
    }
    WF_LAUNCH(wf_fold, dim3(gen_blocks > 0 ? gen_blocks : 1), block, 0, stream, L);
    if (census_pending) {
        if ((e = hipEventSynchronize(hs->events[0])) != hipSuccess)
            return e;
        std::memcpy(packet_census_out, hs->counts + WF_HOST_CENSUS_WORD, 2 * sizeof(unsigned long long));
    }
    if (acc) {
        const int res_blocks = (int)((acc->n_entries + 255u) / 256u);
        if (feat)
            WF_LAUNCH(wf_resolve_features, dim3(res_blocks > 0 ? res_blocks : 1), block, 0, stream, *acc, *feat);
        WF_LAUNCH(wf_resolve_list, dim3(res_blocks > 0 ? res_blocks : 1), block, 0, stream, L, *acc);
        return hipSuccess;
    }
    const int res_blocks = (int)((L.pass_pixels + 255u) / 256u);
    WF_LAUNCH(wf_resolve, dim3(res_blocks > 0 ? res_blocks : 1), block, 0, stream, L, first_pass ? 1 : 0, last_pass ? 1 : 0);
    return hipSuccess;
}

size_t wavefront_sort_temp_bytes(size_t n) {
    size_t tmp = 0;
    uint32_t *k = nullptr;
    (void)rocprim::radix_sort_pairs(nullptr, tmp, k, k, k, k, n, 0u, 27u, (hipStream_t) nullptr);
    return tmp;
}

}
```

Before: 286.9 Msamples/s.

## Precompute camera-relative BVH and triangle records for packet traversal; add sparse-wave drain tail

When packet traversal runs for a single view, a new kernel writes a copy of the BVH nodes and triangles with the camera position already subtracted, and the packet kernel reads these. This folds the per-box origin subtractions and one triangle cross-product term into the copy. The cost is an extra buffer, capped by a size limit, plus a rebuild whenever the camera or geometry generation changes. Separately, the non-packet extend kernel now leaves its ticket loop once the queue is exhausted and most lanes are idle. It then finishes the remaining live lanes in a dedicated unwind loop, to cut per-iteration refill overhead in sparse waves.

```diff
diff --git a/raytracing-course-hw-public_amd/csrc/rt_accum_host.cpp b/raytracing-course-hw-public_amd/csrc/rt_accum_host.cpp
--- a/raytracing-course-hw-public_amd/csrc/rt_accum_host.cpp
+++ b/raytracing-course-hw-public_amd/csrc/rt_accum_host.cpp
@@ -169,7 +169,7 @@
                 W.n_paths = (uint32_t)std::min<uint64_t>((uint64_t)A.n_entries * C, tot[1]);
                 W.first_pixel = 0, W.pass_pixels = A.n_entries;
                 W.first_sample = 0, W.pass_samples = C, W.samples = C;
-                HIP_TRY(rt::launch_pass(s, p, a->pkt, W, 1, true, true, stats != nullptr, &A, a->features ? &a->F : nullptr));
+                HIP_TRY(rt::launch_pass(s, p, a->pkt, W, 1, true, true, stats != nullptr, &A, a->features ? &a->F : nullptr, nullptr, a->view.pos));
                 passes += 1;
                 packet_passes += W.use_packet;
                 if (p->progress && !ad) {
diff --git a/raytracing-course-hw-public_amd/csrc/rt_dev_queue.h b/raytracing-course-hw-public_amd/csrc/rt_dev_queue.h
--- a/raytracing-course-hw-public_amd/csrc/rt_dev_queue.h
+++ b/raytracing-course-hw-public_amd/csrc/rt_dev_queue.h
@@ -27,7 +27,7 @@
     }
 }
 template <class START>
-DEV void ticket_refill(uint32_t *counters, uint32_t n_in, uint32_t chunk, int refill_min, bool idle, bool &exhausted, uint32_t &q_lo, uint32_t &q_hi, TicketState &tks, START start) {
+DEV int ticket_refill(uint32_t *counters, uint32_t n_in, uint32_t chunk, int refill_min, bool idle, bool &exhausted, uint32_t &q_lo, uint32_t &q_hi, TicketState &tks, START start) {
     const unsigned long long im = __ballot(idle);
     const int n_idle = __popcll(im);
     if (!exhausted && (n_idle >= refill_min || n_idle == (int)__popcll(__ballot(1)))) {
@@ -39,6 +39,7 @@
             start(q_lo + rank);
         q_lo += (uint32_t)n_idle < avail ? (uint32_t)n_idle : avail;
     }
+    return n_idle;
 }
 DEV void census_flush(unsigned long long *census, unsigned long long n_trips, unsigned long long n_lanes) {
     if ((threadIdx.x & 63u) == 0u && census && n_trips != 0ull) {
diff --git a/raytracing-course-hw-public_amd/csrc/rt_dev_trav.h b/raytracing-course-hw-public_amd/csrc/rt_dev_trav.h
--- a/raytracing-course-hw-public_amd/csrc/rt_dev_trav.h
+++ b/raytracing-course-hw-public_amd/csrc/rt_dev_trav.h
@@ -17,9 +17,9 @@
     return (c == 0.0f) | ((m >= ORIGIN_LO) & (m <= RANGE_HI));
 }
 
-DEV bool box_hit_exact(V3 bmin, V3 bmax, V3 o, V3 d, float min_dst, float &dist) {
-    V3 i1 = (bmin - o) / d;
-    V3 i2 = (bmax - o) / d;
+DEV bool box_hit_exact_rel(V3 a1, V3 a2, V3 d, float min_dst, float &dist) {
+    V3 i1 = a1 / d;
+    V3 i2 = a2 / d;
     V3 mn = {rmin(i1.x, i2.x), rmin(i1.y, i2.y), rmin(i1.z, i2.z)};
     V3 mx = {rmax(i1.x, i2.x), rmax(i1.y, i2.y), rmax(i1.z, i2.z)};
     float t_min = mn.x;
@@ -39,8 +39,7 @@
     return false;
 }
 
-DEV bool box_hit_fast(V3 bmin, V3 bmax, V3 o, V3 d, V3 r, float min_dst, float &dist) {
-    V3 a1 = bmin - o, a2 = bmax - o;
+DEV bool box_hit_fast_rel(V3 a1, V3 a2, V3 d, V3 r, float min_dst, float &dist) {
     float q1x = div_exact_fast(a1.x, d.x, r.x), q1y = div_exact_fast(a1.y, d.y, r.y), q1z = div_exact_fast(a1.z, d.z, r.z);
     float q2x = div_exact_fast(a2.x, d.x, r.x), q2y = div_exact_fast(a2.y, d.y, r.y), q2z = div_exact_fast(a2.z, d.z, r.z);
     float t_min = fmaxf(fmaxf(fminf(q1x, q2x), fminf(q1y, q2y)), fminf(q1z, q2z));
@@ -64,13 +63,11 @@
     return TriRec{mk(r0.x, r0.y, r0.z), mk(r0.w, r1.x, r1.y), mk(r1.z, r1.w, r2.x), __float_as_uint(r2.z), __float_as_uint(r2.w)};
 }
 
-DEV bool tri_hit(const TriRec &tri, V3 o, V3 d, float min_dst, V3 &xs_out) {
-    const V3 av = tri.v, au = tri.u;
+DEV bool tri_hit_rel(V3 av, V3 au, V3 y, float nz, V3 d, float min_dst, V3 &xs_out) {
     V3 at = -d;
-    V3 y = o - tri.a;
     V3 c_ut = crs(au, at);
     float den = dot(av, c_ut);
-    float nx = dot(y, c_ut), ny = dot(av, crs(y, at)), nz = dot(av, crs(au, y));
+    float nx = dot(y, c_ut), ny = dot(av, crs(y, at));
     const uint32_t sgn = __float_as_uint(den) & 0x80000000u;
     const float D = __builtin_fabsf(den);
     const float nxs = __uint_as_float(__float_as_uint(nx) ^ sgn), nys = __uint_as_float(__float_as_uint(ny) ^ sgn),
@@ -87,6 +84,13 @@
     }
     return false;
 }
+DEV V3 tri_rel_y(V3 a, V3 o) { return o - a; }
+DEV float tri_rel_nz(V3 av, V3 au, V3 y) { return dot(av, crs(au, y)); }
+DEV bool tri_hit(const TriRec &tri, V3 o, V3 d, float min_dst, V3 &xs_out) {
+    const V3 y = tri_rel_y(tri.a, o);
+    return tri_hit_rel(tri.v, tri.u, y, tri_rel_nz(tri.v, tri.u, y), d, min_dst, xs_out);
+}
+DEV bool tri_hit_folded(const TriRec &tri, V3 d, float min_dst, V3 &xs_out) { return tri_hit_rel(tri.v, tri.u, tri.a, __uint_as_float(tri.index), d, min_dst, xs_out); }
 
 struct Hit {
     uint32_t k;
@@ -189,22 +193,23 @@
     bool hl, hr;
     float dl, dr;
 };
-template <bool KNOWN_FAST = false> DEV TwoBox two_box(const NodeRec &n, V3 o, V3 d, V3 r, bool fast, float min_dst) {
+template <bool KNOWN_FAST = false, bool REL = false> DEV TwoBox two_box(const NodeRec &n, V3 o, V3 d, V3 r, bool fast, float min_dst) {
+    const V3 l1 = REL ? n.lmin : n.lmin - o, l2 = REL ? n.lmax : n.lmax - o, r1 = REL ? n.rmn : n.rmn - o, r2 = REL ? n.rmx : n.rmx - o;
     TwoBox b;
     if (KNOWN_FAST || fast) {
-        b.hl = box_hit_fast(n.lmin, n.lmax, o, d, r, min_dst, b.dl);
-        b.hr = box_hit_fast(n.rmn, n.rmx, o, d, r, min_dst, b.dr);
+        b.hl = box_hit_fast_rel(l1, l2, d, r, min_dst, b.dl);
+        b.hr = box_hit_fast_rel(r1, r2, d, r, min_dst, b.dr);
     } else {
-        b.hl = box_hit_exact(n.lmin, n.lmax, o, d, min_dst, b.dl);
-        b.hr = box_hit_exact(n.rmn, n.rmx, o, d, min_dst, b.dr);
+        b.hl = box_hit_exact_rel(l1, l2, d, min_dst, b.dl);
+        b.hr = box_hit_exact_rel(r1, r2, d, min_dst, b.dr);
     }
     return b;
 }
-template <bool STATS, bool GB = false, bool KNOWN_FAST = false, class STK>
+template <bool STATS, bool GB = false, bool KNOWN_FAST = false, bool REL = false, class STK>
 DEV void trav_inner_apply(Trav &T, STK &stk, const NodeRec &n, float min_dst, LaneStats<STATS> &st) {
     st.node();
     st.box(2);
-    const TwoBox bx = two_box<KNOWN_FAST>(n, T.o, T.d, T.r, T.fast, min_dst);
+    const TwoBox bx = two_box<KNOWN_FAST, REL>(n, T.o, T.d, T.r, T.fast, min_dst);
     bool hl = bx.hl, hr = bx.hr;
     const float dl = bx.dl, dr = bx.dr;
     if constexpr (GB) {
diff --git a/raytracing-course-hw-public_amd/csrc/rt_device_types.h b/raytracing-course-hw-public_amd/csrc/rt_device_types.h
--- a/raytracing-course-hw-public_amd/csrc/rt_device_types.h
+++ b/raytracing-course-hw-public_amd/csrc/rt_device_types.h
@@ -211,6 +211,8 @@
     void *sort_temp;
     uint32_t use_packet;
     unsigned long long *packet_census;
+    const DevNode *rel_nodes;
+    const DevTri *rel_tris;
     uint32_t global_best;
     uint32_t order_classed;
     uint32_t sort_mode;
diff --git a/raytracing-course-hw-public_amd/csrc/rt_kernels.h b/raytracing-course-hw-public_amd/csrc/rt_kernels.h
--- a/raytracing-course-hw-public_amd/csrc/rt_kernels.h
+++ b/raytracing-course-hw-public_amd/csrc/rt_kernels.h
@@ -55,6 +55,7 @@
                                  const WfAccum *acc = nullptr, const WfFeat *feat = nullptr, const WfRays *rays = nullptr);
 hipError_t launch_wavefront_cast(const DevScene &S, WfLaunch L, const float *rays, uint32_t n, bool packet, bool stats, uint32_t *prim, float *bct,
                                  hipStream_t stream);
+hipError_t launch_camera_relative(const DevBvh &bvh, uint32_t n_nodes, const float *o, DevNode *rel_nodes, DevTri *rel_tris, int num_cus, hipStream_t stream);
 hipError_t launch_extend_wide(const DevScene &S, const WfLaunch &L, bool packet, bool stats, int blocks, hipStream_t stream);
 size_t wavefront_sort_temp_bytes(size_t n);
 struct AccumRound {
diff --git a/raytracing-course-hw-public_amd/csrc/rt_render.cpp b/raytracing-course-hw-public_amd/csrc/rt_render.cpp
--- a/raytracing-course-hw-public_amd/csrc/rt_render.cpp
+++ b/raytracing-course-hw-public_amd/csrc/rt_render.cpp
@@ -85,8 +85,50 @@
     return RT_OK;
 }
 
+#ifndef RT_REL_MAX_BYTES
+#define RT_REL_MAX_BYTES (1ull << 30)
+#endif
+#ifndef RT_REL_BYTES_PER_PATH
+#define RT_REL_BYTES_PER_PATH 16ull
+#endif
+static hipError_t camera_relative_records(rt_scene *s, WfLaunch &W, const float *cam_pos) {
+    const DevBvh &B = s->dev.scene;
+    const uint32_t n_nodes = s->dev_n_inner[0];
+    if (s->wide_built || B.wide || !B.nodes || !B.tris || B.root == RT_NONE || n_nodes == 0 || B.n_tris == 0)
+        return hipSuccess;
+    const size_t node_bytes = (size_t)n_nodes * sizeof(DevNode), bytes = node_bytes + (size_t)B.n_tris * sizeof(DevTri);
+    if (bytes > RT_REL_MAX_BYTES || bytes > RT_REL_BYTES_PER_PATH * W.n_paths)
+        return hipSuccess;
+    uint32_t pos[3];
+    std::memcpy(pos, cam_pos, 12);
+    const bool same = s->wf_rel_gen == s->geo_generation && std::memcmp(pos, s->wf_rel_pos, 12) == 0;
+    if (!same) {
+        s->wf_rel_gen = 0;
+        if (s->wf_rel_bytes < bytes) {
+            if (s->wf_rel_nodes)
+                (void)hipFree(s->wf_rel_nodes);
+            s->wf_rel_nodes = nullptr, s->wf_rel_tris = nullptr, s->wf_rel_bytes = 0;
+            void *q = nullptr;
+            if (hipMalloc(&q, bytes) != hipSuccess) {
+                (void)hipGetLastError();
+                return hipSuccess;
+            }
+            s->wf_rel_nodes = static_cast<DevNode *>(q);
+            s->wf_rel_bytes = bytes;
+        }
+        s->wf_rel_tris = reinterpret_cast<DevTri *>(reinterpret_cast<char *>(s->wf_rel_nodes) + node_bytes);
+        if (hipError_t e = rt::launch_camera_relative(B, n_nodes, cam_pos, s->wf_rel_nodes, s->wf_rel_tris, s->num_cus, s->stream); e != hipSuccess)
+            return e;
+        std::memcpy(s->wf_rel_pos, pos, 12);
+        s->wf_rel_gen = s->geo_generation;
+    }
+    W.rel_nodes = s->wf_rel_nodes;
+    W.rel_tris = s->wf_rel_tris;
+    return hipSuccess;
+}
+
 hipError_t rt::launch_pass(rt_scene *s, const rt_params *p, PacketPolicy &pol, WfLaunch &W, uint32_t n_views, bool first_pass, bool last_pass, bool time_extends,
-                           const WfAccum *acc, const WfFeat *feat, const WfRays *rays) {
+                           const WfAccum *acc, const WfFeat *feat, const WfRays *rays, const float *cam_pos) {
     W.sort_mode = (p->sort_mode == RT_SORT_AUTO && W.n_paths < (1u << 20)) ? 0u : wavefront_sort_mode(s, p);
     const double min_lanes = packet_min_lanes(s, p);
     uint32_t min_lanes_bits;
@@ -99,6 +141,10 @@
     }
     const uint32_t pkt_min_spp = s->wide_built ? 4u : 16u;
     W.use_packet = p->packet_mode == RT_PACKET_OFF ? 0u : p->packet_mode == RT_PACKET_ON ? 1u : (W.pass_samples >= pkt_min_spp && !pol.off) ? 1u : 0u;
+    W.rel_nodes = nullptr, W.rel_tris = nullptr;
+    if (W.use_packet && cam_pos && n_views == 1 && !rays)
+        if (hipError_t e = camera_relative_records(s, W, cam_pos); e != hipSuccess)
+            return e;
     const rt::WfHostSync hsync = wavefront_host_sync(s);
     unsigned long long census[2] = {0ull, 0ull};
     const hipError_t e = rt::launch_wavefront_pass(s->dev, W, W.stats != nullptr, s->num_cus, first_pass, last_pass, s->stream, time_extends ? &s->ext_events : nullptr, census,
@@ -273,7 +319,8 @@
                 W.first_sample = s0;
                 W.pass_samples = std::min<uint32_t>(pass_spp, p->samples - s0);
                 W.n_paths = W.pass_pixels * W.pass_samples;
-                HIP_TRY(rt::launch_pass(s, p, s->pkt, W, n_views, s0 == 0, s0 + W.pass_samples >= p->samples, stats != nullptr, nullptr));
+                HIP_TRY(rt::launch_pass(s, p, s->pkt, W, n_views, s0 == 0, s0 + W.pass_samples >= p->samples, stats != nullptr, nullptr, nullptr, nullptr,
+                                        n_views == 1 ? vt[0].pos : nullptr));
                 passes += 1;
                 packet_passes += W.use_packet;
                 if (p->progress) {
diff --git a/raytracing-course-hw-public_amd/csrc/rt_scene.cpp b/raytracing-course-hw-public_amd/csrc/rt_scene.cpp
--- a/raytracing-course-hw-public_amd/csrc/rt_scene.cpp
+++ b/raytracing-course-hw-public_amd/csrc/rt_scene.cpp
@@ -493,6 +493,7 @@
     s->build_upload_ms = g.build_upload_ms;
     s->dev_n_inner[0] = g.dev_n_inner[0];
     s->dev_n_inner[1] = g.dev_n_inner[1];
+    ++s->geo_generation;
 }
 
 static int create_impl(const rt_scene_desc *d, const std::shared_ptr<const rt::PreparedScene> &prep, int device, rt_scene *s) {
diff --git a/raytracing-course-hw-public_amd/csrc/rt_scene_impl.h b/raytracing-course-hw-public_amd/csrc/rt_scene_impl.h
--- a/raytracing-course-hw-public_amd/csrc/rt_scene_impl.h
+++ b/raytracing-course-hw-public_amd/csrc/rt_scene_impl.h
@@ -198,6 +198,12 @@
     rt::PacketPolicy pkt;
     std::vector<hipEvent_t> pass_events;
 
+    DevNode *wf_rel_nodes = nullptr;
+    DevTri *wf_rel_tris = nullptr;
+    size_t wf_rel_bytes = 0;
+    uint64_t geo_generation = 1, wf_rel_gen = 0;
+    uint32_t wf_rel_pos[3] = {0, 0, 0};
+
     int ensure_wavefront(uint64_t paths, uint64_t pixels, uint32_t depth) {
         if (paths <= wf_paths_cap && pixels <= wf_pixels_cap && depth <= wf_depth_cap)
             return RT_OK;
@@ -296,6 +302,8 @@
             (void)hipFree(p);
         if (wf_feat)
             (void)hipFree(wf_feat);
+        if (wf_rel_nodes)
+            (void)hipFree(wf_rel_nodes);
         if (d_fb)
             (void)hipFree(d_fb);
         if (d_rgb8)
@@ -330,7 +338,7 @@
 int check_pass_params(const rt_params *p, const char *fn);
 uint64_t wavefront_max_paths(rt_scene *s, const rt_params *p);
 hipError_t launch_pass(rt_scene *s, const rt_params *p, PacketPolicy &pol, WfLaunch &W, uint32_t n_views, bool first_pass, bool last_pass, bool time_extends,
-                       const WfAccum *acc, const WfFeat *feat = nullptr, const WfRays *rays = nullptr);
+                       const WfAccum *acc, const WfFeat *feat = nullptr, const WfRays *rays = nullptr, const float *cam_pos = nullptr);
 int fill_stats(rt_scene *s, bool counters, uint64_t samples, float kernel_ms, std::chrono::steady_clock::time_point wall0, rt_stats *stats);
 
 template <class Queue> int queue_and_wait(rt_scene *s, Queue queue) {
diff --git a/raytracing-course-hw-public_amd/csrc/rt_update.cpp b/raytracing-course-hw-public_amd/csrc/rt_update.cpp
--- a/raytracing-course-hw-public_amd/csrc/rt_update.cpp
+++ b/raytracing-course-hw-public_amd/csrc/rt_update.cpp
@@ -200,6 +200,7 @@
     s->refit_levels_ms = levels_ms;
     s->geo = G;
     s->refitted = true;
+    ++s->geo_generation;
     return RT_OK;
 }
 
diff --git a/raytracing-course-hw-public_amd/csrc/rt_wavefront.hip b/raytracing-course-hw-public_amd/csrc/rt_wavefront.hip
--- a/raytracing-course-hw-public_amd/csrc/rt_wavefront.hip
+++ b/raytracing-course-hw-public_amd/csrc/rt_wavefront.hip
@@ -1,3 +1,4 @@
+#include <algorithm>
 #include <cstring>
 #include <vector>
 
@@ -147,6 +148,20 @@
 #ifndef RT_EXT_LEAF_MIN
 #define RT_EXT_LEAF_MIN 20
 #endif
+#ifndef RT_EXT_SPARSE_MAX
+#define RT_EXT_SPARSE_MAX 32
+#endif
+
+template <bool STATS, bool GB, class STK> DEV void node_step(Trav &T, const DevBvh &bvh, STK &stk, bool stepper, LaneStats<STATS> &st) {
+    const bool plain = (T.cur & RT_LEAF_FLAG) == 0 && T.fast;
+    if (__ballot(stepper && !plain) == 0ull) {
+        if (stepper) {
+            trav_step_inner_fast<STATS, GB>(T, bvh, stk, EPS, st);
+        }
+    } else if (stepper) {
+        trav_step_core<STATS, GB>(T, bvh, stk, EPS, st);
+    }
+}
 
 template <bool STATS, bool GB> __global__ __launch_bounds__(256, RT_EXT_WAVES_PER_SIMD) void wf_extend(const DevScene S, const WfLaunch L) {
     constexpr int DEPTH = GB ? RT_EXT_GB_LDS_DEPTH : RT_EXT_LDS_DEPTH, WORDS = GB ? 2 : 3;
@@ -167,7 +182,7 @@
     uint32_t q_lo = 0, q_hi = 0;
     TicketState tks = ticket_init();
     for (;;) {
-        ticket_refill(L.counters, n_in, (uint32_t)RT_EXT_CHUNK, RT_EXT_REFILL_MIN, T.cur == T_DONE, exhausted, q_lo, q_hi, tks, [&](uint32_t jq) {
+        const int n_idle = ticket_refill(L.counters, n_in, (uint32_t)RT_EXT_CHUNK, RT_EXT_REFILL_MIN, T.cur == T_DONE, exhausted, q_lo, q_hi, tks, [&](uint32_t jq) {
             const WfRay ray = wf_load_ray(L.paths_in + wf_order_slot(L, jq));
             slot = jq;
             trav_init_stored<GB>(T, S.scene, ray.o, ray.d, ray.r, ray.fast);
@@ -193,16 +208,32 @@
         }
         if (sm == 0ull || __popcll(lm) >= RT_EXT_LEAF_MIN) {
             leaf_batch<STATS>(T, S.scene, at_leaf, s_coop, st);
+            if (exhausted && n_idle >= 64 - RT_EXT_SPARSE_MAX)
+                break;
         } else {
-            const bool plain = (T.cur & RT_LEAF_FLAG) == 0 && T.fast;
-            if (__ballot(stepper && !plain) == 0ull) {
-                if (stepper) {
-                    trav_step_inner_fast<STATS, GB>(T, S.scene, stk, EPS, st);
-                }
-            } else if (stepper) {
-                trav_step_core<STATS, GB>(T, S.scene, stk, EPS, st);
-            }
-        }
+            node_step<STATS, GB>(T, S.scene, stk, stepper, st);
+        }
+    }
+    bool live = T.cur != T_DONE;
+    auto unwind = [&]() {
+        trav_pop_wave<GB>(T, stk);
+        if (live && T.cur == T_DONE) {
+            wf_store_hit(L.hits + slot, T.best);
+            live = false;
+        }
+    };
+    for (;;) {
+        unwind();
+        if (__ballot(live) == 0ull)
+            break;
+        const bool at_leaf = live && (T.cur & RT_LEAF_FLAG) != 0 && RT_LEAF_CNT(T.cur) != 0;
+        if (__ballot(at_leaf) != 0ull) {
+            leaf_batch<STATS>(T, S.scene, at_leaf, s_coop, st);
+            unwind();
+        }
+        const bool stepper = live && !((T.cur & RT_LEAF_FLAG) != 0 && RT_LEAF_CNT(T.cur) != 0);
+        if (__ballot(stepper) != 0ull)
+            node_step<STATS, GB>(T, S.scene, stk, stepper, st);
     }
     st.flush(L.stats);
 }
@@ -210,13 +241,15 @@
 #ifndef RT_PKT_CHUNK
 #define RT_PKT_CHUNK 256u
 #endif
-template <bool STATS, bool GB> __global__ __launch_bounds__(256, RT_EXT_WAVES_PER_SIMD) void wf_extend_packet(const DevScene S, const WfLaunch L) {
+template <bool STATS, bool GB, bool REL> __global__ __launch_bounds__(256, RT_EXT_WAVES_PER_SIMD) void wf_extend_packet(const DevScene S, const WfLaunch L) {
     constexpr int DEPTH = GB ? RT_EXT_GB_LDS_DEPTH : RT_EXT_LDS_DEPTH, WORDS = GB ? 2 : 3;
     __shared__ uint32_t s_stack[STACK_LDS_DWORDS(DEPTH, WORDS)];
     LaneStats<STATS> st;
     RT_DECLARE_RING_STACK_W(stk, DEPTH, WORDS, s_stack, L.stack_overflow, L.stack_stride);
     const uint32_t n_in = L.counters[WF_CNT_IN];
     const uint32_t lane = threadIdx.x & 63u;
+    const DevNode *const nodes = REL ? L.rel_nodes : S.scene.nodes;
+    const DevTri *const tris = REL ? L.rel_tris : S.scene.tris;
     Trav T = trav_idle<GB>();
     unsigned long long n_trips = 0ull, n_lanes = 0ull;
     for (;;) {
@@ -249,15 +282,15 @@
                 if ((target & RT_LEAF_FLAG) == 0u) {
                     uint32_t node_index = target;
                     asm volatile("" : "+s"(node_index));
-                    ConstF4 p = as_const_f4(S.scene.nodes + node_index);
+                    ConstF4 p = as_const_f4(nodes + node_index);
                     const F4v r0 = p[0], r1 = p[1], r2 = p[2], r3 = p[3];
                     if (mine)
-                        trav_inner_apply<STATS, GB>(T, stk, node_rec(r0, r1, r2, r3), EPS, st);
+                        trav_inner_apply<STATS, GB, false, REL>(T, stk, node_rec(r0, r1, r2, r3), EPS, st);
                 } else {
                     const uint32_t cnt = RT_LEAF_CNT(target);
                     uint32_t k = target & RT_LEAF_BEGIN_MASK;
                     for (uint32_t i = 0;; ++i, ++k) {
-                        ConstF4 p = as_const_f4(S.scene.tris + k);
+                        ConstF4 p = as_const_f4(tris + k);
                         const F4v r0 = p[0], r1 = p[1], r2 = p[2];
                         const TriRec tri = tri_rec(r0, r1, r2);
                         if (mine) {
@@ -265,7 +298,7 @@
                                 st.node();
                             st.tri();
                             V3 xs;
-                            if (tri_hit(tri, T.o, T.d, EPS, xs)) {
+                            if (REL ? tri_hit_folded(tri, T.d, EPS, xs) : tri_hit(tri, T.o, T.d, EPS, xs)) {
                                 hit_take(T.best, k, xs.x, xs.y, xs.z);
                                 T.t_loc = fminf(T.t_loc, xs.z);
                             }
@@ -283,6 +316,34 @@
     }
     census_flush(L.packet_census, n_trips, n_lanes);
     st.flush(L.stats);
+}
+
+__global__ __launch_bounds__(256) void wf_camera_relative(const DevNode *nodes, uint32_t n_nodes, const DevTri *tris, uint32_t n_tris, V3 o, DevNode *rel_nodes, DevTri *rel_tris) {
+    const uint32_t n = n_nodes + n_tris;
+    for (uint32_t i = blockIdx.x * blockDim.x + threadIdx.x; i < n; i += gridDim.x * blockDim.x) {
+        if (i < n_nodes) {
+            const float4 *p = reinterpret_cast<const float4 *>(nodes + i);
+            const float4 r0 = p[0], r1 = p[1], r2 = p[2], r3 = p[3];
+            const NodeRec r = node_rec(r0, r1, r2, r3);
+            const V3 a = r.lmin - o, b = r.lmax - o, c = r.rmn - o, d = r.rmx - o;
+            float4 *q = reinterpret_cast<float4 *>(rel_nodes + i);
+            q[0] = make_float4(a.x, a.y, a.z, b.x);
+            q[1] = make_float4(b.y, b.z, c.x, c.y);
+            q[2] = make_float4(c.z, d.x, d.y, d.z);
+            q[3] = r3;
+        } else {
+            const uint32_t k = i - n_nodes;
+            const float4 *p = reinterpret_cast<const float4 *>(tris + k);
+            const float4 r0 = p[0], r1 = p[1], r2 = p[2];
+            const TriRec t = tri_rec(r0, r1, r2);
+            const V3 y = tri_rel_y(t.a, o);
+            const float nz = tri_rel_nz(t.v, t.u, y);
+            float4 *q = reinterpret_cast<float4 *>(rel_tris + k);
+            q[0] = make_float4(y.x, y.y, y.z, r0.w);
+            q[1] = r1;
+            q[2] = make_float4(r2.x, r2.y, r2.z, nz);
+        }
+    }
 }
 
 __global__ __launch_bounds__(256) void wf_extend_prims(const DevScene S, const WfLaunch L) {
@@ -618,12 +679,18 @@
 static hipError_t launch_extend(const DevScene &S, const WfLaunch &L, bool packet, bool stats, int ext_blocks, hipStream_t stream) {
     if (S.scene.wide)
         return launch_extend_wide(S, L, packet, stats, ext_blocks, stream);
-    return with_bools([&](auto P, auto ST, auto G) {
+    return with_bools([&](auto P, auto ST, auto G, auto R) {
         if constexpr (P)
-            return RT_LAUNCH_CHECKED((wf_extend_packet<ST, G>), dim3(ext_blocks), dim3(256), 0, stream, S, L);
+            return RT_LAUNCH_CHECKED((wf_extend_packet<ST, G, R>), dim3(ext_blocks), dim3(256), 0, stream, S, L);
         else
             return RT_LAUNCH_CHECKED((wf_extend<ST, G>), dim3(ext_blocks), dim3(256), 0, stream, S, L);
-    }, packet, stats, L.global_best != 0u);
+    }, packet, stats, L.global_best != 0u, packet && L.rel_nodes != nullptr && L.rel_tris != nullptr);
+}
+
+hipError_t launch_camera_relative(const DevBvh &bvh, uint32_t n_nodes, const float *o, DevNode *rel_nodes, DevTri *rel_tris, int num_cus, hipStream_t stream) {
+    const uint32_t n = n_nodes + bvh.n_tris;
+    const uint32_t blocks = std::min<uint32_t>((n + 255u) / 256u, (uint32_t)num_cus * 16u);
+    return RT_LAUNCH_CHECKED(wf_camera_relative, dim3(blocks > 0 ? blocks : 1), dim3(256), 0, stream, bvh.nodes, n_nodes, bvh.tris, bvh.n_tris, V3{o[0], o[1], o[2]}, rel_nodes, rel_tris);
 }
 
 hipError_t launch_wavefront_cast(const DevScene &S, WfLaunch L, const float *rays, uint32_t n, bool packet, bool stats, uint32_t *prim, float *bct,
@@ -635,6 +702,7 @@
     L.n_paths = n;
     L.order = nullptr, L.order_classed = 0u;
     L.packet_census = nullptr;
+    L.rel_nodes = nullptr, L.rel_tris = nullptr;
     const int blocks = (int)((n + 255u) / 256u);
     WF_LAUNCH(wf_from_rays, dim3(blocks), block, 0, stream, L, rays, n);
     if ((e = launch_extend(S, L, packet, stats, (int)(L.stack_stride / 256u), stream)) != hipSuccess)
```

Measured after the change: 291.0 Msamples/s, median of 6. 1.4% higher.
